# una-dinosauria/local-search-quantization

Hardware: AMD Instinct MI355X
Metric: vectors encoded/sec (ICM, m=8 h=256) (higher is better)
Workload: dtype f32

## Files before the change

local-search-quantization_amd/csrc/lsq_api.hip:

```cpp
#include <stdarg.h>
#include <stddef.h>
#include <stdio.h>
#include <string.h>

#include <algorithm>
#include <atomic>
#include <chrono>
#include <string>
#include <thread>
#include <vector>

#include "lsq_internal.h"

static thread_local char g_err[512] = "";

void lsq_set_error(const char *fmt, ...) {
    va_list ap;
    va_start(ap, fmt);
    vsnprintf(g_err, sizeof(g_err), fmt, ap);
    va_end(ap);
}

extern "C" const char *lsq_last_error(void) { return g_err; }
extern "C" int lsq_version(void) { return LSQ_VERSION; }

extern "C" int lsq_device_count(int *count) {
    if (!count) { lsq_set_error("lsq_device_count: null pointer"); return LSQ_EINVAL; }
    int c = 0;
    hipError_t e = hipGetDeviceCount(&c);
    if (e != hipSuccess) { *count = 0; lsq_set_error("hipGetDeviceCount: %s", hipGetErrorString(e)); return LSQ_ENODEV; }
    *count = c;
    return LSQ_OK;
}


enum { CAT_TABLES = 0, CAT_UNARIES, CAT_PERTURB, CAT_ICM, CAT_COST, CAT_OTHER, CAT_COUNT };

enum : size_t { SMALL_COUNTERS = 0, SMALL_OBJ = 8192, SMALL_BAD = 8704, SMALL_QP = 8832, SMALL_ACTIVE = 10240, SMALL_ROAD = 11008,
                SMALL_READ_END = 11072, SMALL_PROBE = 11264, SMALL_BYTES = 12288 };
static_assert(sizeof(lsq_q16_params) <= SMALL_ACTIVE - SMALL_QP && sizeof(unsigned long long) * LSQ_WALK_COUNTERS <= SMALL_ROAD - SMALL_ACTIVE &&
              sizeof(unsigned long long) * LSQ_WALK_COUNTERS <= SMALL_BYTES - SMALL_PROBE, "the per-call block's windows");

struct ChunkRoad {
    bool filtered = false;
    bool on_device = false;
    bool resident = false;
    int64_t cn = 0, row0 = 0;
    int m = 0;
};

struct lsq_ctx {
    int device = 0;
    hipStream_t own_stream = nullptr;
    hipStream_t stream = nullptr;
    int64_t chunk = 256 * 3968;
    int profile = 0;
    int schedule = 6;
    int64_t q16_min = 65536;
    int tables_changed = 1;
    std::vector<float> hostK;
    int hostK_d = 0, hostK_m = 0;
    bool tables_valid = false;
    int64_t table_reuses = 0;
    int per_node = 0;
    int ablation = 0;
    int light = -1;
    int wave_max = 64;
    int fallback = 1;
    int skip = 1;
    uint32_t auto_it = 0;
    DevBuf sci, T, Ts, U, vCur, vNew, active, recCur, recNew, prev, counters, obj, bad;
    DevBuf probe;
    int64_t probe_div = 8;
    DevBuf small;
    char *small_host = nullptr;
    bool small_packed = false;
    DevBuf Uq, Tq, qp, qscratch, qflag, qsigma;
    lsq_q16_work qw;
    ChunkRoad chunk_road;
    int64_t call_row0 = 0;
    int async_mode = 0;
    bool pending_fold = false;
    DevBuf road;
    int64_t fallback_div = 64;
    int64_t filter_fallback_chunks = 0;
    lsq_lsqr_state *lsqr = nullptr;
    lsq_kmeans_state *kmeans = nullptr;
    lsq_spgl1_state *spgl1 = nullptr;
    lsq_adc_state *adc = nullptr;
    lsq_linscan_stats adc_stats{};
    lsq_search_opts search;
    int knn_u8_int = 1;
    int64_t rerank_batch = 0;
    DevBuf sX, sX2, sK, sB16, sOut16, sTight, sF32;
    DevBuf sSample, sSigmaS;
    std::vector<float> sample_host;
    std::vector<hipEvent_t> panel_ev;
    int64_t panel_bytes = 48ll << 20;
    int64_t pipeline_min_bytes = 64ll << 20;
    hipStream_t copy_stream = nullptr;
    hipEvent_t copy_done = nullptr;
    double cat_ms[CAT_COUNT] = {0, 0, 0, 0, 0, 0};
    int64_t icm_launches = 0, icm_node_updates = 0, staged_blocks = 0, light_blocks = 0, filtered_blocks = 0, filter_refined = 0, filter_exact = 0, filter_f32 = 0;
    int64_t trace[LSQ_WALK_TRACE] = {0};
    struct Pending { hipEvent_t a, b; int cat; };
    std::vector<Pending> pending;
    std::vector<hipEvent_t> pool;
};

static int fold_pending(lsq_ctx *c);
struct AsyncOff {
    lsq_ctx *c; int saved;
    explicit AsyncOff(lsq_ctx *ctx) : c(ctx), saved(ctx ? ctx->async_mode : 0) { if (c) c->async_mode = 0; }
    ~AsyncOff() { if (c) c->async_mode = saved; }
};

static int use_device(lsq_ctx *ctx) {
    if (!ctx) { lsq_set_error("null lsq_ctx"); return LSQ_EINVAL; }
    LSQ_HIP(hipSetDevice(ctx->device));
    return LSQ_OK;
}

struct Timer {
    lsq_ctx *c; int cat; hipEvent_t a = nullptr, b = nullptr; bool on;
    Timer(lsq_ctx *ctx, int category) : c(ctx), cat(category), on(ctx->profile != 0) {
        if (!on) return;
        a = grab(); b = grab();
        if (!a || !b) { on = false; return; }
        (void)hipEventRecord(a, c->stream);
    }
    hipEvent_t grab() {
        if (!c->pool.empty()) { hipEvent_t e = c->pool.back(); c->pool.pop_back(); return e; }
        hipEvent_t e = nullptr;
        if (hipEventCreate(&e) != hipSuccess) return nullptr;
        return e;
    }
    ~Timer() {
        if (!on) return;
        (void)hipEventRecord(b, c->stream);
        c->pending.push_back({a, b, cat});
    }
};

static int resolve_timings(lsq_ctx *ctx) {
    for (auto &p : ctx->pending) {
        LSQ_HIP(hipEventSynchronize(p.b));
        float ms = 0.f;
        LSQ_HIP(hipEventElapsedTime(&ms, p.a, p.b));
        ctx->cat_ms[p.cat] += (double)ms;
        ctx->pool.push_back(p.a);
        ctx->pool.push_back(p.b);
    }
    ctx->pending.clear();
    return LSQ_OK;
}

extern "C" int lsq_create(lsq_ctx **out, int device) {
    if (!out) { lsq_set_error("lsq_create: null out pointer"); return LSQ_EINVAL; }
    *out = nullptr;
    int count = 0;
    LSQ_TRY(lsq_device_count(&count));
    if (count <= 0) { lsq_set_error("no HIP device visible (this library has no CPU fallback)"); return LSQ_ENODEV; }
    if (device < 0 || device >= count) { lsq_set_error("device %d out of range (0..%d)", device, count - 1); return LSQ_EINVAL; }
    LSQ_HIP(hipSetDevice(device));
    hipDeviceProp_t prop;
    LSQ_HIP(hipGetDeviceProperties(&prop, device));
    if (strncmp(prop.gcnArchName, "gfx950", 6) != 0) {
        lsq_set_error("device %d is %s; this library carries gfx950 (MI355X) code objects only", device, prop.gcnArchName);
        return LSQ_ENODEV;
    }
    lsq_ctx *c = new lsq_ctx();
    c->device = device;
    hipError_t e = hipStreamCreateWithFlags(&c->own_stream, hipStreamNonBlocking);
    if (e != hipSuccess) { delete c; lsq_set_error("hipStreamCreate: %s", hipGetErrorString(e)); return LSQ_EHIP; }
    c->stream = c->own_stream;
    if (hipMalloc(&c->small.p, SMALL_BYTES) != hipSuccess || hipHostMalloc(reinterpret_cast<void **>(&c->small_host), SMALL_BYTES, hipHostMallocDefault) != hipSuccess) {
        if (c->small.p) (void)hipFree(c->small.p);
        (void)hipStreamDestroy(c->own_stream);
        delete c;
        lsq_set_error("lsq_create: no memory for the per-call block");
        return LSQ_ENOMEM;
    }
    c->small.cap = SMALL_BYTES;
    {
        hipFuncAttributes fa;
        (void)hipFuncGetAttributes(&fa, lsq_probe_kernel_gemm());
        (void)hipFuncGetAttributes(&fa, lsq_probe_kernel_icm());
        (void)hipFuncGetAttributes(&fa, lsq_probe_kernel_icmq());
        (void)hipStreamCreateWithFlags(&c->copy_stream, hipStreamNonBlocking);
        (void)hipEventCreateWithFlags(&c->copy_done, hipEventDisableTiming);
        char warm[256] = {0};
        (void)hipMemcpyAsync(c->small.p, warm, sizeof(warm), hipMemcpyHostToDevice, c->own_stream);
        (void)hipMemcpyAsync(warm, c->small.p, sizeof(warm), hipMemcpyDeviceToHost, c->own_stream);
        (void)hipStreamSynchronize(c->own_stream);
        (void)hipGetLastError();
    }
    c->counters.window(c->small.p, SMALL_COUNTERS, SMALL_OBJ - SMALL_COUNTERS);
    c->obj.window(c->small.p, SMALL_OBJ, SMALL_BAD - SMALL_OBJ);
    c->bad.window(c->small.p, SMALL_BAD, 64);
    c->qp.window(c->small.p, SMALL_QP, SMALL_ACTIVE - SMALL_QP);
    c->active.window(c->small.p, SMALL_ACTIVE, SMALL_ROAD - SMALL_ACTIVE);
    c->road.window(c->small.p, SMALL_ROAD, SMALL_READ_END - SMALL_ROAD);
    c->probe.window(c->small.p, SMALL_PROBE, SMALL_BYTES - SMALL_PROBE);
    *out = c;
    return LSQ_OK;
}

extern "C" int lsq_destroy(lsq_ctx *c) {
    if (!c) return LSQ_OK;
    (void)hipSetDevice(c->device);
    (void)hipStreamSynchronize(c->stream);
    for (auto &p : c->pending) { (void)hipEventDestroy(p.a); (void)hipEventDestroy(p.b); }
    for (auto e : c->pool) (void)hipEventDestroy(e);
    DevBuf *bufs[] = {&c->road, &c->probe, &c->Uq, &c->Tq, &c->qp, &c->qscratch, &c->qflag, &c->qsigma, &c->sci, &c->T, &c->Ts, &c->U, &c->vCur, &c->vNew, &c->active, &c->recCur, &c->recNew, &c->prev, &c->counters, &c->obj, &c->bad,
                      &c->sX, &c->sX2, &c->sK, &c->sB16, &c->sOut16, &c->sTight, &c->sF32, &c->sSample, &c->sSigmaS};
    for (DevBuf *b : bufs) b->release();
    c->small.release();
    if (c->small_host) (void)hipHostFree(c->small_host);
    for (auto e : c->panel_ev) (void)hipEventDestroy(e);
    lsq_adc_free(c->adc);
    lsq_lsqr_free(c->lsqr);
    lsq_spgl1_free(c->spgl1);
    lsq_kmeans_free(c->kmeans);
    if (c->own_stream) (void)hipStreamDestroy(c->own_stream);
    if (c->copy_stream) (void)hipStreamDestroy(c->copy_stream);
    if (c->copy_done) (void)hipEventDestroy(c->copy_done);
    delete c;
    return LSQ_OK;
}

extern "C" int lsq_set_stream(lsq_ctx *c, void *hip_stream) {
    LSQ_TRY(use_device(c));
    if (c->stream != reinterpret_cast<hipStream_t>(hip_stream)) c->tables_valid = false;
    c->stream = reinterpret_cast<hipStream_t>(hip_stream);
    return LSQ_OK;
}

extern "C" int lsq_set_option(lsq_ctx *c, const char *key, int64_t value) {
    if (!c || !key) { lsq_set_error("lsq_set_option: null argument"); return LSQ_EINVAL; }
    if (!strcmp(key, "chunk")) {
        if (value < 1) { lsq_set_error("chunk must be >= 1"); return LSQ_EINVAL; }
        c->chunk = value;
    } else if (!strcmp(key, "profile")) c->profile = value != 0;
    else if (!strcmp(key, "own_stream")) { if (c->stream != c->own_stream) c->tables_valid = false; c->stream = c->own_stream; }
    else if (!strcmp(key, "skip")) c->skip = value != 0;
#ifdef LSQ_TUNING
    else if (!strcmp(key, "ablation")) c->ablation = (int)value;
#endif
    else if (!strcmp(key, "light")) c->light = (int)value;
    else if (!strcmp(key, "wave_max")) c->wave_max = (int)value;
    else if (!strcmp(key, "fallback")) c->fallback = (int)value;
    else if (!strcmp(key, "q16_min")) c->q16_min = value;
    else if (!strcmp(key, "async")) c->async_mode = value != 0;
    else if (!strcmp(key, "per_node")) c->per_node = value != 0;
    else if (!strcmp(key, "upload_panel_bytes")) {
        if (value < 1) { lsq_set_error("upload_panel_bytes must be >= 1"); return LSQ_EINVAL; }
        c->panel_bytes = value;
    }
    else if (!strcmp(key, "upload_pipeline_min_bytes")) {
        if (value < 0) { lsq_set_error("upload_pipeline_min_bytes must be >= 0"); return LSQ_EINVAL; }
        c->pipeline_min_bytes = value;
    }
    else if (!strcmp(key, "filter_probe_div")) {
        if (value < 0) { lsq_set_error("filter_probe_div must be >= 0"); return LSQ_EINVAL; }
        c->probe_div = value;
    }
    else if (!strcmp(key, "filter_fallback_div")) {
        if (value < 0) { lsq_set_error("filter_fallback_div must be >= 0"); return LSQ_EINVAL; }
        c->fallback_div = value;
    }
    else if (!strcmp(key, "linscan_exhaustive")) c->search.force_exhaustive = value != 0;
    else if (!strcmp(key, "linscan_rank")) {
        if (value < 0) { lsq_set_error("linscan_rank must be >= 0"); return LSQ_EINVAL; }
        c->search.rank_override = (int)value;
    }
    else if (!strcmp(key, "knn_u8_int")) c->knn_u8_int = value != 0;
    else if (!strcmp(key, "rerank_batch")) {
        if (value < 0) { lsq_set_error("rerank_batch must be >= 0"); return LSQ_EINVAL; }
        c->rerank_batch = value;
    }
    else if (!strcmp(key, "ils_counter")) {
        if (value < 0 || value >= (int64_t)LSQ_IT_AUTO) { lsq_set_error("ils_counter must lie in 0..2^32-2"); return LSQ_EINVAL; }
        c->auto_it = (uint32_t)value;
    }
    else if (!strcmp(key, "schedule")) {
        if (value != 3 && value != 4 && value != 6) { lsq_set_error("schedule must be 3, 4 or 6"); return LSQ_EINVAL; }
        c->schedule = (int)value;
    } else { lsq_set_error("unknown option '%s'", key); return LSQ_EINVAL; }
    return LSQ_OK;
}

static int fill_timings(lsq_ctx *c, lsq_timings *out);

extern "C" int lsq_get_timings(lsq_ctx *c, lsq_timings *out) {
    if (!out) { lsq_set_error("lsq_get_timings: null out"); return LSQ_EINVAL; }
    lsq_timings t;
    LSQ_TRY(fill_timings(c, &t));
    memcpy(out, &t, offsetof(lsq_timings, table_reuses));
    return LSQ_OK;
}

extern "C" int lsq_get_timings_sized(lsq_ctx *c, void *out, size_t bytes) {
    if (!out) { lsq_set_error("lsq_get_timings_sized: null out"); return LSQ_EINVAL; }
    lsq_timings t;
    LSQ_TRY(fill_timings(c, &t));
    memcpy(out, &t, bytes < sizeof(t) ? bytes : sizeof(t));
    return LSQ_OK;
}

static int fill_timings(lsq_ctx *c, lsq_timings *out) {
    LSQ_TRY(use_device(c));
    LSQ_TRY(fold_pending(c));
    LSQ_TRY(resolve_timings(c));
    out->tables_ms = c->cat_ms[CAT_TABLES];
    out->unaries_ms = c->cat_ms[CAT_UNARIES];
    out->perturb_ms = c->cat_ms[CAT_PERTURB];
    out->icm_ms = c->cat_ms[CAT_ICM];
    out->cost_ms = c->cat_ms[CAT_COST];
    out->other_ms = c->cat_ms[CAT_OTHER];
    out->icm_launches = c->icm_launches;
    out->icm_node_updates = c->icm_node_updates;
    out->staged_blocks = c->staged_blocks;
    out->light_blocks = c->light_blocks;
    out->filtered_blocks = c->filtered_blocks;
    out->filter_refined = c->filter_refined;
    out->filter_exact = c->filter_exact;
    out->filter_f32 = c->filter_f32;
    out->filter_fallback_chunks = c->filter_fallback_chunks;
    out->xs_launches = 0;
    out->xs_fallback_launches = 0;
    out->table_reuses = c->table_reuses;
    return LSQ_OK;
}

extern "C" int lsq_get_walk_trace(lsq_ctx *c, int64_t *out, int count) {
    if (!c || !out || count < 0) { lsq_set_error("lsq_get_walk_trace: bad arguments"); return LSQ_EINVAL; }
    for (int q = 0; q < count; ++q) out[q] = q < LSQ_WALK_TRACE ? c->trace[q] : 0;
    return LSQ_OK;
}

static_assert(sizeof(lsq_q16_snapshot_params) == sizeof(lsq_q16_params) && sizeof(lsq_q16_snapshot_node) == sizeof(lsq_q16_node) &&
              offsetof(lsq_q16_snapshot_params, node) == offsetof(lsq_q16_params, node) && offsetof(lsq_q16_snapshot_node, window) == offsetof(lsq_q16_node, window) &&
              offsetof(lsq_q16_snapshot_node, slack) == offsetof(lsq_q16_node, slack) && offsetof(lsq_q16_snapshot_node, hiq) == offsetof(lsq_q16_node, hiq),
              "the public snapshot structure restates lsq_q16_params");
extern "C" int lsq_get_q16_snapshot(lsq_ctx *c, int what, void *dst, size_t bytes, int64_t *info) {
    LSQ_TRY(use_device(c));
    if (!c->chunk_road.resident) {
        lsq_set_error("lsq_get_q16_snapshot: no filtered chunk is resident (the last chunk whose unaries were built did not take the 16-bit filtered walk)");
        return LSQ_EINVAL;
    }
    const size_t cn = (size_t)c->chunk_road.cn, m = (size_t)c->chunk_road.m;
    const DevBuf *src = nullptr;
    size_t need = 0;
    switch (what) {
    case LSQ_SNAP_PARAMS: src = &c->qp; need = sizeof(lsq_q16_params); break;
    case LSQ_SNAP_UQ: src = &c->Uq; need = sizeof(uint16_t) * m * cn * LSQ_H; break;
    case LSQ_SNAP_TQ: src = &c->Tq; need = sizeof(uint16_t) * m * (m - 1) * LSQ_H * LSQ_H; break;
    case LSQ_SNAP_QFLAG: src = &c->qflag; need = sizeof(unsigned short) * cn; break;
    case LSQ_SNAP_U: src = &c->U; need = sizeof(float) * m * cn * LSQ_H; break;
    case LSQ_SNAP_T: src = &c->T; need = sizeof(float) * m * m * LSQ_H * LSQ_H; break;
    default: lsq_set_error("lsq_get_q16_snapshot: unknown item %d", what); return LSQ_EINVAL;
    }
    if (need > 0 && (!dst || bytes < need || src->cap < need)) {
        lsq_set_error("lsq_get_q16_snapshot: item %d takes %zu bytes, the buffer has %zu", what, need, dst ? bytes : (size_t)0);
        return LSQ_EINVAL;
    }
    if (info) {
        info[0] = c->chunk_road.cn; info[1] = c->chunk_road.row0; info[2] = c->chunk_road.m;
        info[3] = lsq_q16_slice_width(c->chunk_road.m); info[4] = lsq_walk_slice_width(c->chunk_road.m); info[5] = c->chunk_road.filtered ? 1 : 0;
    }
    if (need > 0) LSQ_HIP(hipMemcpyAsync(dst, src->p, need, hipMemcpyDefault, c->stream));
    return LSQ_OK;
}

extern "C" int lsq_reset_timings(lsq_ctx *c) {
    LSQ_TRY(use_device(c));
    LSQ_TRY(fold_pending(c));
    LSQ_TRY(resolve_timings(c));
    for (double &v : c->cat_ms) v = 0.0;
    c->icm_launches = c->icm_node_updates = c->staged_blocks = c->light_blocks = c->filtered_blocks = c->filter_refined = c->filter_exact = c->filter_f32 = 0;
    c->filter_fallback_chunks = 0;
    c->table_reuses = 0;
    for (int64_t &v : c->trace) v = 0;
    c->adc_stats = lsq_linscan_stats{};
    return LSQ_OK;
}

static int linscan_check(const char *fn, const void *a, const void *b, const void *c0, const void *d0, const void *e, const void *f, int nq, int n,
                         int m, int h, int d, int nn) {
    if (nq < 0 || n < 0 || d < 1 || nn < 1) { lsq_set_error("%s: bad shape nq=%d n=%d d=%d nn=%d", fn, nq, n, d, nn); return LSQ_EINVAL; }
    if (h != LSQ_H || m < 1 || m > LSQ_MAX_M) { lsq_set_error("%s: needs h == 256 and 1 <= m <= 16 (got h=%d m=%d)", fn, h, m); return LSQ_EINVAL; }
    if (nn > n) { lsq_set_error("%s: nn=%d exceeds the database size %d", fn, nn, n); return LSQ_EINVAL; }
    if (nq > 0 && (!a || !b || !c0 || !d0 || !e || !f)) { lsq_set_error("%s: null pointer", fn); return LSQ_EINVAL; }
    return LSQ_OK;
}

static lsq_search_opts search_opts(const lsq_ctx *c, lsq_linscan_stats *stats) {
    lsq_search_opts o = c->search;
    o.stats = stats;
    o.timed = c->profile;
    return o;
}

static lsq_search_input lsq_input(const uint8_t *codes, const float *Q, const float *K, const float *dbnorms, int n, int m, int d) {
    lsq_search_input in{};
    in.kind = LSQ_SEARCH_LSQ; in.codes = codes; in.cstride = m; in.Q = Q; in.qstride = d; in.K = K; in.dbnorms = dbnorms; in.n = n; in.m = m; in.d = d;
    return in;
}
static lsq_search_input pq_input(const uint8_t *codes, int cstride, const float *centers, const float *Q, int qstride, int n, int m, int subdim) {
    lsq_search_input in{};
    in.kind = LSQ_SEARCH_PQ; in.codes = codes; in.cstride = cstride; in.Q = Q; in.qstride = qstride; in.K = centers; in.n = n; in.m = m; in.d = subdim;
    return in;
}
static lsq_search_input exact_input(const void *base, int base_u8, int ldb, const void *Q, int q_u8, int ldq, int n, int d) {
    lsq_search_input in{};
    in.kind = LSQ_SEARCH_EXACT; in.Q = Q; in.qstride = ldq; in.n = n; in.d = d; in.base = base; in.bstride = ldb; in.base_u8 = base_u8; in.q_u8 = q_u8;
    return in;
}

extern "C" int lsq_linscan_dev(lsq_ctx *c, float *d_dists, int *d_idx, const uint8_t *d_codes, const float *d_queries, const float *d_codebooks,
                               const float *d_dbnorms, int nqueries, int ncodes, int m, int h, int d, int nn) {
    if (!c) { lsq_set_error("lsq_linscan_dev: null context"); return LSQ_EINVAL; }
    LSQ_TRY(linscan_check("lsq_linscan_dev", d_dists, d_idx, d_codes, d_queries, d_codebooks, d_dbnorms, nqueries, ncodes, m, h, d, nn));
    if (nqueries == 0) return LSQ_OK;
    LSQ_TRY(use_device(c));
    return lsq_adc_search(c->stream, &c->adc, d_dists, d_idx, lsq_input(d_codes, d_queries, d_codebooks, d_dbnorms, ncodes, m, d), nqueries, nn,
                          search_opts(c, &c->adc_stats));
}

extern "C" int lsq_linscan(lsq_ctx *c, float *dists, int *idx, const unsigned char *codes, const float *queries, const float *codebooks,
                           const float *dbnorms, int nqueries, int ncodes, int m, int h, int d, int nn) {
    if (!c) { lsq_set_error("lsq_linscan: null context"); return LSQ_EINVAL; }
    LSQ_TRY(linscan_check("lsq_linscan", dists, idx, codes, queries, codebooks, dbnorms, nqueries, ncodes, m, h, d, nn));
    if (nqueries == 0) return LSQ_OK;
    LSQ_TRY(use_device(c));
    return lsq_adc_search_host(c->stream, &c->adc, dists, idx, lsq_input(codes, queries, codebooks, dbnorms, ncodes, m, d), nqueries, nn,
                               search_opts(c, &c->adc_stats));
}

static int linscan_pq_check(const char *fn, const void *a, const void *b, const void *c0, const void *d0, const void *e, int N, uint32_t NQ, int B,
                            int K, int dim1codes, int dim1queries, int subdim) {
    LSQ_TRY(lsq_linscan_pq_check(fn, a, b, c0, d0, e, N, NQ, B, K, dim1codes, dim1queries, subdim));
    if (B / 8 > LSQ_MAX_M) { lsq_set_error("%s: the device scan needs B/8 <= 16 (got B=%d: %d sub-spaces)", fn, B, B / 8); return LSQ_EINVAL; }
    if (NQ > (uint32_t)INT32_MAX) { lsq_set_error("%s: NQ=%u exceeds the device scan's limit of 2^31 - 1 queries", fn, NQ); return LSQ_EINVAL; }
    return LSQ_OK;
}

extern "C" int lsq_linscan_pq_dev(lsq_ctx *c, float *d_dists, uint32_t *d_res, const uint8_t *d_codes, const float *d_centers, const float *d_queries,
                                  int N, uint32_t NQ, int B, int K, int dim1codes, int dim1queries, int subdim) {
    if (!c) { lsq_set_error("lsq_linscan_pq_dev: null context"); return LSQ_EINVAL; }
    LSQ_TRY(linscan_pq_check("lsq_linscan_pq_dev", d_dists, d_res, d_codes, d_centers, d_queries, N, NQ, B, K, dim1codes, dim1queries, subdim));
    if (NQ == 0) return LSQ_OK;
    LSQ_TRY(use_device(c));
    return lsq_adc_search(c->stream, &c->adc, d_dists, reinterpret_cast<int *>(d_res),
                          pq_input(d_codes, dim1codes, d_centers, d_queries, dim1queries, N, B / 8, subdim), (int)NQ, K, search_opts(c, &c->adc_stats));
}

extern "C" int lsq_linscan_pq(lsq_ctx *c, float *dists, uint32_t *res, const uint8_t *codes, const float *centers, const float *queries, int N,
                              uint32_t NQ, int B, int K, int dim1codes, int dim1queries, int subdim) {
    if (!c) { lsq_set_error("lsq_linscan_pq: null context"); return LSQ_EINVAL; }
    LSQ_TRY(linscan_pq_check("lsq_linscan_pq", dists, res, codes, centers, queries, N, NQ, B, K, dim1codes, dim1queries, subdim));
    if (NQ == 0) return LSQ_OK;
    LSQ_TRY(use_device(c));
    return lsq_adc_search_host(c->stream, &c->adc, dists, reinterpret_cast<int *>(res), pq_input(codes, dim1codes, centers, queries, dim1queries, N, B / 8, subdim),
                               (int)NQ, K, search_opts(c, &c->adc_stats));
}

extern "C" int lsq_knn_exact_dev(lsq_ctx *c, float *d_dists, uint32_t *d_ids, const float *d_base, const float *d_queries, int n, int nq, int d, int ldb,
                                 int ldq, int nn) {
    if (!c) { lsq_set_error("lsq_knn_exact_dev: null context"); return LSQ_EINVAL; }
    LSQ_TRY(lsq_knn_exact_check("lsq_knn_exact_dev", d_dists, d_ids, d_base, d_queries, n, nq, d, ldb, ldq, nn));
    LSQ_TRY(use_device(c));
    return lsq_adc_search(c->stream, &c->adc, d_dists, reinterpret_cast<int *>(d_ids), exact_input(d_base, 0, ldb, d_queries, 0, ldq, n, d), nq, nn,
                          search_opts(c, &c->adc_stats));
}

extern "C" int lsq_knn_exact(lsq_ctx *c, float *dists, uint32_t *ids, const float *base, const float *queries, int n, int nq, int d, int ldb, int ldq,
                             int nn) {
    if (!c) { lsq_set_error("lsq_knn_exact: null context"); return LSQ_EINVAL; }
    LSQ_TRY(lsq_knn_exact_check("lsq_knn_exact", dists, ids, base, queries, n, nq, d, ldb, ldq, nn));
    LSQ_TRY(use_device(c));
    return lsq_adc_search_host(c->stream, &c->adc, dists, reinterpret_cast<int *>(ids), exact_input(base, 0, ldb, queries, 0, ldq, n, d), nq, nn,
                               search_opts(c, &c->adc_stats));
}

extern "C" int lsq_get_linscan_stats(lsq_ctx *c, lsq_linscan_stats *out) {
    if (!c || !out) { lsq_set_error("lsq_get_linscan_stats: null argument"); return LSQ_EINVAL; }
    *out = c->adc_stats;
    return LSQ_OK;
}

struct lsq_index {
    lsq_ctx *ctx = nullptr;
    int64_t n = 0;
    int d = 0, m = 0, base_u8 = 0;
    int64_t ldb = 0;
    const uint8_t *codes = nullptr;
    const float *K = nullptr, *norms = nullptr;
    const void *base = nullptr;
    DevBuf own_codes, own_K, own_norms, own_base;
    lsq_adc_state *adc = nullptr;
    DevBuf rec_a, rec_b, seg, counter;
    DevBuf short_d, short_i;
    DevBuf s_qscan, s_qexact, s_cand, s_dists, s_ids;
    DevBuf nrm_x, nrm_q;
    hipEvent_t ev[3] = {nullptr, nullptr, nullptr};
    lsq_index_stats stats{};
    lsq_index_knn_info knn{};
};

extern "C" int lsq_index_destroy(lsq_index *ix) {
    if (!ix) return LSQ_OK;
    (void)hipSetDevice(ix->ctx->device);
    (void)hipStreamSynchronize(ix->ctx->stream);
    DevBuf *bufs[] = {&ix->own_codes, &ix->own_K, &ix->own_norms, &ix->own_base, &ix->rec_a, &ix->rec_b, &ix->seg, &ix->counter, &ix->short_d, &ix->short_i,
                      &ix->s_qscan, &ix->s_qexact, &ix->s_cand, &ix->s_dists, &ix->s_ids, &ix->nrm_x, &ix->nrm_q};
    for (DevBuf *b : bufs) b->release();
    lsq_adc_free(ix->adc);
    for (hipEvent_t e : ix->ev) if (e) (void)hipEventDestroy(e);
    delete ix;
    return LSQ_OK;
}

static int index_adopt(lsq_index *ix, DevBuf &own, const void *src, size_t bytes, int on_device, const void **dst) {
    if (on_device) { *dst = src; return LSQ_OK; }
    LSQ_TRY(own.ensure(bytes));
    LSQ_HIP(hipMemcpyAsync(own.p, src, bytes, hipMemcpyHostToDevice, ix->ctx->stream));
    *dst = own.p;
    return LSQ_OK;
}

extern "C" int lsq_index_create(lsq_index **out, lsq_ctx *c, const lsq_index_desc *desc) {
    if (!out) { lsq_set_error("lsq_index_create: null out pointer"); return LSQ_EINVAL; }
    *out = nullptr;
    if (!c || !desc) { lsq_set_error("lsq_index_create: null %s", c ? "description" : "context"); return LSQ_EINVAL; }
    if (!desc->codes && !desc->base) { lsq_set_error("lsq_index_create: neither codes nor base rows"); return LSQ_EINVAL; }
    if (desc->n < 1 || desc->n > (int64_t)INT32_MAX - 1 || desc->d < 1) {
        lsq_set_error("lsq_index_create: needs 1 <= n <= 2^31 - 2 and d >= 1 (got n=%lld d=%d)", (long long)desc->n, desc->d);
        return LSQ_EINVAL;
    }
    if (desc->codes) {
        if (desc->h != LSQ_H || desc->m < 1 || desc->m > LSQ_MAX_M) {
            lsq_set_error("lsq_index_create: needs h == 256 and 1 <= m <= 16 (got h=%d m=%d)", desc->h, desc->m);
            return LSQ_EINVAL;
        }
        if (!desc->codebooks || !desc->dbnorms) { lsq_set_error("lsq_index_create: codes without codebooks or dbnorms"); return LSQ_EINVAL; }
    }
    if (desc->base && desc->ldb < desc->d) { lsq_set_error("lsq_index_create: needs ldb >= d (got ldb=%d d=%d)", desc->ldb, desc->d); return LSQ_EINVAL; }
    if (desc->base && !desc->base_u8 && ((uintptr_t)desc->base & 3) != 0) { lsq_set_error("lsq_index_create: the f32 base is not 4-byte aligned"); return LSQ_EINVAL; }
    LSQ_TRY(use_device(c));
    lsq_index *ix = new lsq_index();
    ix->ctx = c;
    ix->n = desc->n; ix->d = desc->d; ix->m = desc->codes ? desc->m : 0; ix->base_u8 = desc->base_u8 != 0; ix->ldb = desc->ldb;
    const size_t n = (size_t)desc->n, d = (size_t)desc->d;
    int rc = LSQ_OK;
    if (desc->codes) {
        rc = index_adopt(ix, ix->own_codes, desc->codes, n * (size_t)desc->m, desc->on_device, reinterpret_cast<const void **>(&ix->codes));
        if (rc == LSQ_OK) rc = index_adopt(ix, ix->own_K, desc->codebooks, sizeof(float) * (size_t)desc->m * LSQ_H * d, desc->on_device, reinterpret_cast<const void **>(&ix->K));
        if (rc == LSQ_OK) rc = index_adopt(ix, ix->own_norms, desc->dbnorms, sizeof(float) * n, desc->on_device, reinterpret_cast<const void **>(&ix->norms));
    }
    if (rc == LSQ_OK && desc->base)
        rc = index_adopt(ix, ix->own_base, desc->base, ((n - 1) * (size_t)desc->ldb + d) * (desc->base_u8 ? 1 : sizeof(float)), desc->on_device, &ix->base);
    if (rc == LSQ_OK) rc = ix->counter.ensure(sizeof(unsigned long long));
    if (rc == LSQ_OK && hipStreamSynchronize(c->stream) != hipSuccess) { lsq_set_error("lsq_index_create: the upload failed"); rc = LSQ_EHIP; }
    if (rc != LSQ_OK) { (void)lsq_index_destroy(ix); return rc; }
    *out = ix;
    return LSQ_OK;
}

static int index_rerank_dev(lsq_index *ix, float *d_dists, int *d_ids, const float *d_q, int64_t ldq, const int *d_cand, int nq, int L, int nn, int id_base) {
    lsq_ctx *c = ix->ctx;
    hipStream_t s = c->stream;
    const bool timed = c->profile != 0;
    if (timed) for (hipEvent_t &e : ix->ev) if (!e) LSQ_HIP(hipEventCreate(&e));
    int64_t qb = c->rerank_batch > 0 ? c->rerank_batch : (int64_t)(1u << 28) / L;
    if (qb > (int64_t)(1u << 28) / L) qb = (int64_t)(1u << 28) / L;
    if (qb > 16384) qb = 16384;
    if (qb < 1) qb = 1;
    if (qb > nq) qb = nq;
    LSQ_TRY(ix->rec_a.ensure(sizeof(uint64_t) * (size_t)qb * L));
    LSQ_TRY(ix->rec_b.ensure(sizeof(uint64_t) * (size_t)qb * L));
    LSQ_TRY(ix->seg.ensure(sizeof(int) * 2 * (size_t)qb));
    LSQ_HIP(hipMemsetAsync(ix->counter.p, 0, sizeof(unsigned long long), s));
    const int idbits = lsq_adc_idbits(ix->n);
    for (int q0 = 0; q0 < nq; q0 += (int)qb) {
        const int nqb = (int)std::min<int64_t>(qb, nq - q0);
        if (timed) LSQ_HIP(hipEventRecord(ix->ev[0], s));
        LSQ_TRY(lsq_rerank_launch(s, ix->base, ix->base_u8, ix->ldb, ix->n, d_q, ldq, d_cand, q0, nqb, L, ix->d, id_base, ix->rec_a.as<uint64_t>(), idbits,
                                  ix->counter.as<unsigned long long>()));
        if (timed) LSQ_HIP(hipEventRecord(ix->ev[1], s));
        LSQ_TRY(lsq_adc_select(&ix->adc, s, ix->rec_a.as<uint64_t>(), ix->rec_b.as<uint64_t>(), ix->seg.as<int>(), nullptr, nullptr, nullptr, q0, nqb, L, nn,
                               d_dists, d_ids, idbits, 33 + idbits, 1 - id_base));
        if (timed) {
            LSQ_HIP(hipEventRecord(ix->ev[2], s));
            LSQ_HIP(hipEventSynchronize(ix->ev[2]));
            float a = 0, b = 0;
            LSQ_HIP(hipEventElapsedTime(&a, ix->ev[0], ix->ev[1]));
            LSQ_HIP(hipEventElapsedTime(&b, ix->ev[1], ix->ev[2]));
            ix->stats.gather_ms += a; ix->stats.select_ms += b;
        }
        ix->stats.batches += 1;
    }
    unsigned long long bad = 0;
    LSQ_HIP(hipMemcpyAsync(&bad, ix->counter.p, sizeof(bad), hipMemcpyDeviceToHost, s));
    LSQ_HIP(hipStreamSynchronize(s));
    ix->stats.invalid += (int64_t)bad;
    ix->stats.rows += (int64_t)nq * L - (int64_t)bad;
    return LSQ_OK;
}

static int index_stage_rows(lsq_index *ix, DevBuf &buf, const float *src, int rows, int64_t ld, int width, bool pack, const float **dst, int64_t *ld_out) {
    hipStream_t s = ix->ctx->stream;
    if (pack && ld != width) {
        LSQ_TRY(buf.ensure(sizeof(float) * (size_t)rows * width));
        LSQ_HIP(hipMemcpy2DAsync(buf.p, sizeof(float) * (size_t)width, src, sizeof(float) * (size_t)ld, sizeof(float) * (size_t)width, (size_t)rows,
                                 hipMemcpyDefault, s));
        *ld_out = width;
    } else {
        const size_t floats = (size_t)(rows - 1) * (size_t)ld + (size_t)width;
        LSQ_TRY(buf.ensure(sizeof(float) * floats));
        LSQ_HIP(hipMemcpyAsync(buf.p, src, sizeof(float) * floats, hipMemcpyDefault, s));
        *ld_out = ld;
    }
    *dst = buf.as<float>();
    return LSQ_OK;
}

static int index_call_check(const char *fn, lsq_index *ix, const void *dists, const void *ids, int nq, int64_t ldq, int nn) {
    if (!ix) { lsq_set_error("%s: null index", fn); return LSQ_EINVAL; }
    if (nq < 0 || nn < 1 || ldq < ix->d) { lsq_set_error("%s: needs nq >= 0, nn >= 1, ldq >= d (got nq=%d nn=%d ldq=%lld d=%d)", fn, nq, nn, (long long)ldq, ix->d); return LSQ_EINVAL; }
    if (!dists || !ids) { lsq_set_error("%s: null pointer", fn); return LSQ_EINVAL; }
    return LSQ_OK;
}

extern "C" int lsq_index_rerank(lsq_index *ix, float *dists, int *ids, const float *queries, const int *cand, int nq, int ldq, int L, int nn, int id_base,
                                int on_device) {
    LSQ_TRY(index_call_check("lsq_index_rerank", ix, dists, ids, nq, ldq, nn));
    if (!ix->base) { lsq_set_error("lsq_index_rerank: the index holds no base rows"); return LSQ_EINVAL; }
    LSQ_TRY(lsq_rerank_check("lsq_index_rerank", dists, ids, ix->base, queries, cand, ix->n, nq, ix->d, ix->ldb, ldq, L, nn, id_base));
    if (L > (1 << 28)) { lsq_set_error("lsq_index_rerank: needs L <= 2^28 candidates per query (got %d)", L); return LSQ_EINVAL; }
    if (nq == 0) return LSQ_OK;
    LSQ_TRY(use_device(ix->ctx));
    hipStream_t s = ix->ctx->stream;
    if (on_device) {
        LSQ_TRY(index_rerank_dev(ix, dists, ids, queries, ldq, cand, nq, L, nn, id_base));
    } else {
        const float *dq = nullptr;
        int64_t ld = 0;
        LSQ_TRY(index_stage_rows(ix, ix->s_qexact, queries, nq, ldq, ix->d, false, &dq, &ld));
        LSQ_TRY(ix->s_cand.ensure(sizeof(int) * (size_t)nq * L));
        LSQ_TRY(ix->s_dists.ensure(sizeof(float) * (size_t)nq * nn));
        LSQ_TRY(ix->s_ids.ensure(sizeof(int) * (size_t)nq * nn));
        LSQ_HIP(hipMemcpyAsync(ix->s_cand.p, cand, sizeof(int) * (size_t)nq * L, hipMemcpyHostToDevice, s));
        LSQ_TRY(index_rerank_dev(ix, ix->s_dists.as<float>(), ix->s_ids.as<int>(), dq, ld, ix->s_cand.as<int>(), nq, L, nn, id_base));
        LSQ_HIP(hipMemcpyAsync(dists, ix->s_dists.p, sizeof(float) * (size_t)nq * nn, hipMemcpyDeviceToHost, s));
        LSQ_HIP(hipMemcpyAsync(ids, ix->s_ids.p, sizeof(int) * (size_t)nq * nn, hipMemcpyDeviceToHost, s));
        LSQ_HIP(hipStreamSynchronize(s));
    }
    ix->stats.queries += nq;
    return LSQ_OK;
}

extern "C" int lsq_index_search(lsq_index *ix, float *dists, int *ids, const float *q_scan, const float *q_exact, int nq, int ldq, int shortlist, int nn,
                                int on_device) {
    LSQ_TRY(index_call_check("lsq_index_search", ix, dists, ids, nq, ldq, nn));
    if (!ix->codes) { lsq_set_error("lsq_index_search: the index holds no codes"); return LSQ_EINVAL; }
    if (shortlist < 0 || (shortlist > 0 && shortlist < nn)) { lsq_set_error("lsq_index_search: needs shortlist == 0 or shortlist >= nn (got shortlist=%d nn=%d)", shortlist, nn); return LSQ_EINVAL; }
    const int L = shortlist > 0 ? shortlist : nn;
    if (L > ix->n) { lsq_set_error("lsq_index_search: %s=%d exceeds the database size %lld", shortlist > 0 ? "shortlist" : "nn", L, (long long)ix->n); return LSQ_EINVAL; }
    if (shortlist > (1 << 28)) { lsq_set_error("lsq_index_search: needs shortlist <= 2^28 (got %d)", shortlist); return LSQ_EINVAL; }
    if (shortlist > 0 && !ix->base) { lsq_set_error("lsq_index_search: a shortlist needs base rows, the index holds none"); return LSQ_EINVAL; }
    if (!q_scan || (shortlist > 0 && !q_exact)) { lsq_set_error("lsq_index_search: null pointer"); return LSQ_EINVAL; }
    if (nq == 0) return LSQ_OK;
    lsq_ctx *c = ix->ctx;
    LSQ_TRY(use_device(c));
    hipStream_t s = c->stream;
    const int d = ix->d;
    const float *dqs = q_scan;
    int64_t ld = ldq;
    if (!on_device || ldq != d) LSQ_TRY(index_stage_rows(ix, ix->s_qscan, q_scan, nq, ldq, d, true, &dqs, &ld));
    const float *dqe = q_exact;
    int64_t lde = ldq;
    if (shortlist > 0 && !on_device) LSQ_TRY(index_stage_rows(ix, ix->s_qexact, q_exact, nq, ldq, d, false, &dqe, &lde));
    float *out_d = dists;
    int *out_i = ids;
    if (!on_device) {
        LSQ_TRY(ix->s_dists.ensure(sizeof(float) * (size_t)nq * nn));
        LSQ_TRY(ix->s_ids.ensure(sizeof(int) * (size_t)nq * nn));
        out_d = ix->s_dists.as<float>();
        out_i = ix->s_ids.as<int>();
    }
    float *scan_d = out_d;
    int *scan_i = out_i;
    if (shortlist > 0) {
        LSQ_TRY(ix->short_d.ensure(sizeof(float) * (size_t)nq * L));
        LSQ_TRY(ix->short_i.ensure(sizeof(int) * (size_t)nq * L));
        scan_d = ix->short_d.as<float>();
        scan_i = ix->short_i.as<int>();
    }
    lsq_linscan_stats st{};
    LSQ_TRY(lsq_adc_search(s, &ix->adc, scan_d, scan_i, lsq_input(ix->codes, dqs, ix->K, ix->norms, (int)ix->n, ix->m, d), nq, L, search_opts(c, &st)));
    ix->stats.scan_ms += st.lut_ms + st.sample_ms + st.scan_ms + st.select_ms;
    if (shortlist > 0) LSQ_TRY(index_rerank_dev(ix, out_d, out_i, dqe, lde, scan_i, nq, L, nn, 1));
    if (!on_device) {
        LSQ_HIP(hipMemcpyAsync(dists, out_d, sizeof(float) * (size_t)nq * nn, hipMemcpyDeviceToHost, s));
        LSQ_HIP(hipMemcpyAsync(ids, out_i, sizeof(int) * (size_t)nq * nn, hipMemcpyDeviceToHost, s));
        LSQ_HIP(hipStreamSynchronize(s));
    }
    ix->stats.queries += nq;
    return LSQ_OK;
}

extern "C" int lsq_index_knn(lsq_index *ix, float *dists, int *ids, const void *queries, int queries_u8, int nq, int ldq, int nn, int id_base,
                             int on_device) {
    if (!ix) { lsq_set_error("lsq_index_knn: null index"); return LSQ_EINVAL; }
    if (!ix->base) { lsq_set_error("lsq_index_knn: the index holds no base rows"); return LSQ_EINVAL; }
    if (!dists || !ids || !queries) { lsq_set_error("lsq_index_knn: null pointer"); return LSQ_EINVAL; }
    if (nq < 1 || ldq < ix->d) { lsq_set_error("lsq_index_knn: needs nq >= 1 and ldq >= d (got nq=%d ldq=%d d=%d)", nq, ldq, ix->d); return LSQ_EINVAL; }
    if (nn < 1 || nn > ix->n) { lsq_set_error("lsq_index_knn: needs 1 <= nn <= n (got nn=%d n=%lld)", nn, (long long)ix->n); return LSQ_EINVAL; }
    if (id_base != 0 && id_base != 1) { lsq_set_error("lsq_index_knn: id_base must be 0 or 1 (got %d)", id_base); return LSQ_EINVAL; }
    const int q_u8 = queries_u8 != 0;
    if (!q_u8 && ((uintptr_t)queries & 3) != 0) { lsq_set_error("lsq_index_knn: the f32 queries are not 4-byte aligned"); return LSQ_EINVAL; }
    if (ix->ldb > (int64_t)INT32_MAX) { lsq_set_error("lsq_index_knn: needs ldb <= 2^31 - 1"); return LSQ_EINVAL; }
    lsq_ctx *c = ix->ctx;
    LSQ_TRY(use_device(c));
    hipStream_t s = c->stream;
    const int n = (int)ix->n, d = ix->d;
    const size_t qe = q_u8 ? 1 : sizeof(float), out_items = (size_t)nq * (size_t)nn;
    const void *dq = queries;
    float *out_d = dists;
    int *out_i = ids;
    if (!on_device) {
        const size_t q_bytes = qe * ((size_t)(nq - 1) * (size_t)ldq + (size_t)d);
        LSQ_TRY(ix->s_qexact.ensure(q_bytes));
        LSQ_TRY(ix->s_dists.ensure(sizeof(float) * out_items));
        LSQ_TRY(ix->s_ids.ensure(sizeof(int) * out_items));
        LSQ_HIP(hipMemcpyAsync(ix->s_qexact.p, queries, q_bytes, hipMemcpyHostToDevice, s));
        dq = ix->s_qexact.p;
        out_d = ix->s_dists.as<float>();
        out_i = ix->s_ids.as<int>();
    }
    lsq_search_input in = exact_input(ix->base, ix->base_u8, (int)ix->ldb, dq, q_u8, ldq, n, d);
    in.id_base = id_base;
    const bool int_road = ix->base_u8 && q_u8 && d <= 258 && c->knn_u8_int;
    lsq_index_knn_info info{};
    if (int_road) {
        const bool timed = c->profile != 0;
        if (timed) for (hipEvent_t &e : ix->ev) if (!e) LSQ_HIP(hipEventCreate(&e));
        LSQ_TRY(ix->nrm_x.ensure(sizeof(uint32_t) * (size_t)n));
        LSQ_TRY(ix->nrm_q.ensure(sizeof(uint32_t) * (size_t)nq));
        if (timed) LSQ_HIP(hipEventRecord(ix->ev[0], s));
        LSQ_TRY(lsq_knn_launch_norms_u8(s, static_cast<const uint8_t *>(ix->base), ix->ldb, n, d, ix->nrm_x.as<uint32_t>()));
        LSQ_TRY(lsq_knn_launch_norms_u8(s, static_cast<const uint8_t *>(dq), ldq, nq, d, ix->nrm_q.as<uint32_t>()));
        if (timed) {
            LSQ_HIP(hipEventRecord(ix->ev[1], s));
            LSQ_HIP(hipEventSynchronize(ix->ev[1]));
            float ms = 0;
            LSQ_HIP(hipEventElapsedTime(&ms, ix->ev[0], ix->ev[1]));
            info.norms_ms = ms;
        }
        in.xnorms = ix->nrm_x.as<uint32_t>();
        in.qnorms = ix->nrm_q.as<uint32_t>();
    }
    lsq_linscan_stats st{};
    LSQ_TRY(lsq_adc_search(s, &ix->adc, out_d, out_i, in, nq, nn, search_opts(c, &st)));
    if (!on_device) {
        LSQ_HIP(hipMemcpyAsync(dists, out_d, sizeof(float) * out_items, hipMemcpyDeviceToHost, s));
        LSQ_HIP(hipMemcpyAsync(ids, out_i, sizeof(int) * out_items, hipMemcpyDeviceToHost, s));
        LSQ_HIP(hipStreamSynchronize(s));
    }
    info.queries = nq; info.rows = n; info.batches = st.batches; info.fallback_queries = st.fallback_queries; info.exhaustive = st.exhaustive;
    info.int_road = int_road ? 1 : 0;
    info.scan_ms = st.sample_ms + st.scan_ms; info.select_ms = st.select_ms;
    ix->knn = info;
    ix->stats.queries += nq;
    return LSQ_OK;
}

extern "C" int lsq_index_get_knn_info(lsq_index *ix, lsq_index_knn_info *out) {
    if (!ix || !out) { lsq_set_error("lsq_index_get_knn_info: null argument"); return LSQ_EINVAL; }
    *out = ix->knn;
    return LSQ_OK;
}

extern "C" int lsq_index_get_stats(lsq_index *ix, lsq_index_stats *out) {
    if (!ix || !out) { lsq_set_error("lsq_index_get_stats: null argument"); return LSQ_EINVAL; }
    *out = ix->stats;
    return LSQ_OK;
}

extern "C" int lsq_synchronize(lsq_ctx *c) {
    LSQ_TRY(use_device(c));
    LSQ_HIP(hipStreamSynchronize(c->stream));
    return LSQ_OK;
}

extern "C" int lsq_node_order(uint64_t seed, uint32_t it, int m, int randord, int32_t *order) {
    if (!order || m < 1 || m > LSQ_MAX_M) { lsq_set_error("lsq_node_order: bad arguments"); return LSQ_EINVAL; }
    for (int p = 0; p < m; ++p) order[p] = p;
    if (!randord) return LSQ_OK;
    for (int p = m - 1; p >= 1; --p) {
        const uint32_t r = lsq_rng_word(seed, 0, it, LSQ_DOM_PERM, (uint32_t)(m - 1 - p));
        const int q = (int)lsq_mulhi32(r, (uint32_t)(p + 1));
        std::swap(order[p], order[q]);
    }
    return LSQ_OK;
}

extern "C" int lsq_splitarray(int64_t n, int nparts, int part, int64_t *start, int64_t *len) {
    if (n < 0 || nparts < 1 || part < 0 || part >= nparts || !start || !len) { lsq_set_error("lsq_splitarray: bad arguments"); return LSQ_EINVAL; }
    const int64_t per = n / nparts, xtra = n % nparts;
    *start = part < xtra ? part * (per + 1) : xtra * (per + 1) + (part - xtra) * per;
    *len = part < xtra ? per + 1 : per;
    return LSQ_OK;
}

extern "C" int lsq_randinit(uint64_t seed, uint64_t global_offset, int64_t n, int m, int h, int16_t *B) {
    if (n < 0 || m < 1 || h < 1 || h > 32767 || (!B && n > 0)) { lsq_set_error("lsq_randinit: bad arguments"); return LSQ_EINVAL; }
    for (int64_t i = 0; i < n; ++i)
        for (int j = 0; j < m; ++j)
            B[i * m + j] = (int16_t)(1 + lsq_mulhi32(lsq_rng_word(seed, global_offset + (uint64_t)i, 0, LSQ_DOM_INIT, (uint32_t)j), (uint32_t)h));
    return LSQ_OK;
}

static int check_shape(const char *fn, int d, int64_t n, int m, int h) {
    if (d < 1 || n < 0 || m < 1 || m > LSQ_MAX_M) { lsq_set_error("%s: bad shape d=%d n=%lld m=%d (need d>=1, n>=0, 1<=m<=16)", fn, d, (long long)n, m); return LSQ_EINVAL; }
    if (h != LSQ_H) { lsq_set_error("%s: h=%d unsupported; this engine (like the reference GPU path) needs h == 256", fn, h); return LSQ_EINVAL; }
    return LSQ_OK;
}

static int check_codes_host(const char *fn, const int16_t *B, int64_t n, int m, int h) {
    const int64_t total = n * (int64_t)m;
    unsigned bad = 0;
    for (int64_t q = 0; q < total; ++q) bad |= (unsigned)((unsigned)(uint16_t)(B[q] - 1) >= (unsigned)h);
    if (bad) { lsq_set_error("%s: input codes must lie in 1..%d", fn, h); return LSQ_ECODE; }
    return LSQ_OK;
}

static int prepare_tables(lsq_ctx *c, const float *dK, int d, int m) {
    Timer t(c, CAT_TABLES);
    c->tables_changed = 1;
    c->chunk_road.resident = false;
    c->tables_valid = false;
    const int mh = m * LSQ_H;
    LSQ_TRY(c->sci.ensure(sizeof(float) * (size_t)mh));
    LSQ_TRY(c->T.ensure(sizeof(float) * (size_t)mh * mh));
    LSQ_TRY(lsq_launch_sqnorms(c->stream, dK, mh, d, c->sci.as<float>()));
    LSQ_TRY(lsq_launch_chain_gemm(c->stream, dK, dK, nullptr, 2.0f, mh, mh, d, LSQ_H, (int64_t)m * LSQ_H * LSQ_H, LSQ_H, c->T.as<float>(), 0, mh, 0));
    if (c->schedule >= 3 && m > 1) {
        LSQ_TRY(c->Ts.ensure(sizeof(float) * (size_t)m * (m - 1) * LSQ_H * LSQ_H));
        LSQ_TRY(lsq_launch_tables_to_slices(c->stream, c->T.as<float>(), c->Ts.as<float>(), m, lsq_walk_slice_width(m)));
    }
    return LSQ_OK;
}

static bool use_q16(const lsq_ctx *c, int64_t cn) { return c->schedule >= 6 && cn >= c->q16_min; }
static bool start_chunk(lsq_ctx *c, int64_t cn, int slice) {
    c->chunk_road = ChunkRoad{};
    return slice > 0 && use_q16(c, cn);
}

static int q16_map(lsq_ctx *c, int d, int64_t cn, int m, int64_t nsample_rows) {
    LSQ_TRY(c->Uq.ensure(sizeof(uint16_t) * (size_t)m * (size_t)cn * LSQ_H));
    LSQ_TRY(c->Tq.ensure(sizeof(uint16_t) * (size_t)m * (size_t)(m > 1 ? m - 1 : 1) * LSQ_H * LSQ_H));
    const size_t off_bad = 16, off_qrange = 64, off_trange = 256;
    static_assert(off_qrange + sizeof(unsigned) * lsq_q16_work::Q_WORDS <= off_trange, "the range words end before the table ranges");
    const size_t off_rowmin = (off_trange + sizeof(float) * 3 * (size_t)m * m + 255) & ~(size_t)255;
    const size_t off_colmean = off_rowmin + sizeof(float) * (size_t)m * m * LSQ_H;
    const size_t off_colshift = off_colmean + sizeof(float) * (size_t)m * m * LSQ_H;
    const size_t off_means = off_colshift + sizeof(float) * (size_t)m * LSQ_H;
    LSQ_TRY(c->qscratch.ensure(off_means + sizeof(float) * (size_t)m * d));
    LSQ_TRY(c->qsigma.ensure(sizeof(float) * (size_t)cn * m));
    LSQ_TRY(c->qflag.ensure(sizeof(unsigned short) * (size_t)(cn + 2)));
    LSQ_TRY(c->qp.ensure(sizeof(lsq_q16_params)));
    if (nsample_rows > 0) LSQ_TRY(c->sSigmaS.ensure(sizeof(float) * (size_t)nsample_rows * m));
    char *sc = c->qscratch.as<char>();
    lsq_q16_work &w = c->qw;
    w = lsq_q16_work{};
    w.Tq = c->Tq.as<uint16_t>(); w.Uq = c->Uq.as<uint16_t>();
    w.bad = reinterpret_cast<int *>(sc + off_bad);
    w.qrange = reinterpret_cast<unsigned *>(sc + off_qrange);
    w.trange = reinterpret_cast<float *>(sc + off_trange);
    w.rowmin = reinterpret_cast<float *>(sc + off_rowmin);
    w.colmean = reinterpret_cast<float *>(sc + off_colmean);
    w.colshift = reinterpret_cast<float *>(sc + off_colshift);
    w.means = reinterpret_cast<float *>(sc + off_means);
    w.sigma = c->qsigma.as<float>();
    w.qflag = c->qflag.as<unsigned short>();
    w.P = c->qp.as<lsq_q16_params>();
    return LSQ_OK;
}

template <class XT>
static int q16_prepare_chunk(lsq_ctx *c, const XT *dX, const float *dK, int d, int64_t cn, int m, const XT *Xsample = nullptr, int64_t nsample_rows = 0) {
    Timer t(c, CAT_TABLES);
    LSQ_TRY(q16_map(c, d, cn, m, Xsample ? nsample_rows : 0));
    if (Xsample) { c->qw.Xsample = Xsample; c->qw.nsample_rows = nsample_rows; c->qw.sigma_sample = c->sSigmaS.as<float>(); }
    LSQ_TRY(lsq_launch_q16_prepare(c->stream, dX, cn, d, dK, c->sci.as<float>(), c->T.as<float>(), m, c->qw, c->tables_changed));
    c->tables_changed = 0;
    return LSQ_OK;
}

template <class XT>
static int unary_gemm(lsq_ctx *c, const XT *dXc, const float *dK, int d, int64_t cn, int m, int slice, int64_t r0, int64_t rows, bool q16) {
    lsq_gemm_q16 levels;
    if (q16) {
        const lsq_q16_work &w = c->qw;
        levels.Dq = w.Uq; levels.slice_q = lsq_q16_slice_width(m); levels.qp = w.P; levels.qflag = w.qflag; levels.sigma = w.sigma; levels.colshift = w.colshift;
    }
    return lsq_launch_chain_gemm(c->stream, dXc + (size_t)r0 * d, dK, c->sci.as<float>(), -2.0f, rows, m * LSQ_H, d, LSQ_H, cn * (int64_t)LSQ_H, LSQ_H,
                                 c->U.as<float>(), slice, cn, r0, q16 ? &levels : nullptr);
}

static int q16_verdict(lsq_ctx *c, bool q16, int64_t cn, int m);

template <class XT>
static int build_unaries(lsq_ctx *c, const XT *dX, const float *dK, int d, int64_t cn, int m, int slice, int64_t r0, int64_t rows) {
    const bool q16 = start_chunk(c, cn, slice) && r0 == 0 && rows == cn;
    if (q16) LSQ_TRY(q16_prepare_chunk(c, dX, dK, d, cn, m));
    {
        Timer t(c, CAT_UNARIES);
        LSQ_TRY(c->U.ensure(sizeof(float) * (size_t)m * (size_t)cn * LSQ_H));
        LSQ_TRY(unary_gemm(c, dX, dK, d, cn, m, slice, r0, rows, q16));
    }
    return q16_verdict(c, q16, cn, m);
}

static int q16_verdict(lsq_ctx *c, bool q16, int64_t cn, int m) {
    if (q16 && c->async_mode) {
        LSQ_TRY(c->road.ensure(2 * sizeof(unsigned)));
        LSQ_TRY(lsq_launch_q16_road(c->stream, c->qp.as<lsq_q16_params>(), c->road.as<unsigned>(), cn * (int64_t)m, c->fallback_div));
        c->chunk_road.filtered = true;
        c->chunk_road.on_device = true;
    } else if (q16) {
        int verdict[3] = {0, 0, 0};
        LSQ_HIP(hipMemcpyAsync(verdict, c->qp.p, sizeof(verdict), hipMemcpyDeviceToHost, c->stream));
        LSQ_HIP(hipStreamSynchronize(c->stream));
        if (verdict[0] == 1 && (int64_t)verdict[2] * c->fallback_div <= cn * (int64_t)m) c->chunk_road.filtered = true;
        else c->filter_fallback_chunks += 1;
        c->chunk_road.resident = c->chunk_road.filtered;
        c->chunk_road.cn = cn; c->chunk_road.m = m; c->chunk_road.row0 = c->call_row0;
    }
    return LSQ_OK;
}

template <class XT>
static int build_unaries_from_host(lsq_ctx *c, const XT *Xh, XT *dXc, const float *dK, int d, int64_t cn, int m, int slice) {
    const bool q16 = start_chunk(c, cn, slice);
    const size_t row_bytes = sizeof(XT) * (size_t)d;
    int64_t prow = (int64_t)((uint64_t)c->panel_bytes / row_bytes) / 128 * 128;
    if (prow < 128) prow = 128;
    const int npan = (int)((cn + prow - 1) / prow);
    if (!c->copy_stream) LSQ_HIP(hipStreamCreateWithFlags(&c->copy_stream, hipStreamNonBlocking));
    while ((int)c->panel_ev.size() < npan) {
        hipEvent_t e = nullptr;
        LSQ_HIP(hipEventCreateWithFlags(&e, hipEventDisableTiming));
        c->panel_ev.push_back(e);
    }
    if (q16) {
        int64_t rts = 1;
        const int spanels = lsq_q16_sample_rows(cn, d, &rts);
        int64_t ns = 0;
        for (int sp = 0; sp < spanels; ++sp) ns += std::min<int64_t>(128, cn - (int64_t)sp * rts * 128);
        c->sample_host.resize(((size_t)ns * row_bytes + sizeof(float) - 1) / sizeof(float));
        XT *sample = reinterpret_cast<XT *>(c->sample_host.data());
        int64_t at = 0;
        for (int sp = 0; sp < spanels; ++sp) {
            const int64_t r0 = (int64_t)sp * rts * 128, rows = std::min<int64_t>(128, cn - r0);
            memcpy(sample + (size_t)at * d, Xh + (size_t)r0 * d, (size_t)rows * row_bytes);
            at += rows;
        }
        LSQ_TRY(c->sSample.ensure((size_t)ns * row_bytes));
        LSQ_HIP(hipMemcpyAsync(c->sSample.p, sample, (size_t)ns * row_bytes, hipMemcpyHostToDevice, c->stream));
        LSQ_TRY(q16_prepare_chunk<XT>(c, dXc, dK, d, cn, m, c->sSample.as<XT>(), ns));
    }
    LSQ_TRY(c->U.ensure(sizeof(float) * (size_t)m * (size_t)cn * LSQ_H));
    std::atomic<int> landed{0};
    hipError_t herr = hipSuccess;
    std::thread feeder;
    try {
    feeder = std::thread([&]() {
        hipError_t e = hipSetDevice(c->device);
        for (int p = 0; p < npan && e == hipSuccess; ++p) {
            const int64_t r0 = (int64_t)p * prow, rows = std::min<int64_t>(prow, cn - r0);
            e = hipMemcpyAsync(dXc + (size_t)r0 * d, Xh + (size_t)r0 * d, (size_t)rows * row_bytes, hipMemcpyHostToDevice, c->copy_stream);
            if (e == hipSuccess) e = hipEventRecord(c->panel_ev[(size_t)p], c->copy_stream);
            if (e == hipSuccess) landed.store(p + 1, std::memory_order_release);
        }
        herr = e;
        if (e != hipSuccess) landed.store(npan + 1, std::memory_order_release);
    });
    } catch (...) {
        LSQ_HIP(hipMemcpyAsync(dXc, Xh, (size_t)cn * row_bytes, hipMemcpyHostToDevice, c->stream));
        if (q16) c->tables_changed = 1;
        return build_unaries(c, dXc, dK, d, cn, m, slice, 0, cn);
    }
    int rc = LSQ_OK;
    for (int p = 0; p < npan && rc == LSQ_OK; ++p) {
        for (int spins = 0; landed.load(std::memory_order_acquire) <= p; ++spins) {
            if (spins < 64) std::this_thread::yield();
            else std::this_thread::sleep_for(std::chrono::microseconds(50));
        }
        if (landed.load(std::memory_order_acquire) > npan) break;
        const int64_t r0 = (int64_t)p * prow, rows = std::min<int64_t>(prow, cn - r0);
        if (hipStreamWaitEvent(c->stream, c->panel_ev[(size_t)p], 0) != hipSuccess) { lsq_set_error("hipStreamWaitEvent failed"); rc = LSQ_EHIP; break; }
        Timer t(c, CAT_UNARIES);
        if (q16) rc = lsq_launch_unary_shift_panel(c->stream, dXc + (size_t)r0 * d, rows, d, m, c->qw, r0);
        if (rc == LSQ_OK) rc = unary_gemm(c, dXc, dK, d, cn, m, slice, r0, rows, q16);
    }
    feeder.join();
    if (herr != hipSuccess) { lsq_set_error("upload of X failed: %s", hipGetErrorString(herr)); return herr == hipErrorOutOfMemory ? LSQ_ENOMEM : LSQ_EHIP; }
    LSQ_TRY(rc);
    return q16_verdict(c, q16, cn, m);
}

static int run_sweeps(lsq_ctx *c, uint8_t *rec, unsigned short *valid, int64_t cn, int m, const int32_t *order, int nsweeps, unsigned long long *stats,
                      const uint8_t *ref_rec = nullptr, const unsigned short *ref_valid = nullptr, int first_sweep = 0) {
    if (nsweeps <= 0) return LSQ_OK;
    const int pos_base = first_sweep * m;
    Timer t(c, CAT_ICM);
    if (!c->fallback) { ref_rec = nullptr; ref_valid = nullptr; }
    std::vector<int32_t> seq((size_t)nsweeps * m);
    for (int sw = 0; sw < nsweeps; ++sw)
        for (int q = 0; q < m; ++q) seq[(size_t)sw * m + q] = order[q];
    enum { F32, WAVE, FILTERED } road = F32;
    int per_launch = 64;
    if (c->schedule < 4) per_launch = 1;
    else if (c->chunk_road.filtered && valid) {
        road = FILTERED;
        if (c->per_node) per_launch = 1;
    } else {
        int per_pass = 0, npass = 0;
        lsq_walk_geometry(cn, lsq_walk_pp(m, lsq_walk_slice_width(m)), &per_pass, &npass);
        const int light_max = c->light >= 0 ? c->light : 256;
        if (c->ablation == 0 && per_pass <= light_max && per_pass <= c->wave_max) road = WAVE;
    }
    const bool both = road == FILTERED && c->chunk_road.on_device;
    const float *U = c->U.as<float>(), *T = c->T.as<float>();
    int launched = 0;
    if (road == FILTERED)
        LSQ_TRY(lsq_launch_icm_walkq(c->stream, U, c->Uq.as<uint16_t>(), c->Tq.as<uint16_t>(), T, rec, valid, cn, m, seq.data(), (int)seq.size(), pos_base, per_launch,
                                     c->skip, stats, c->light, ref_rec, ref_valid, c->qp.as<lsq_q16_params>(), c->qflag.as<unsigned short>(),
                                     both ? c->road.as<unsigned>() : nullptr, &launched));
    if (road == WAVE)
        LSQ_TRY(lsq_launch_icm_wave(c->stream, U, T, rec, valid, cn, m, seq.data(), (int)seq.size(), pos_base, 64, c->skip, stats, ref_rec, ref_valid, &launched));
    if (road == F32 || both)
        LSQ_TRY(lsq_launch_icm_walk(c->stream, U, c->Ts.as<float>(), T, rec, valid, cn, m, seq.data(), (int)seq.size(), pos_base, both ? 64 : per_launch, c->skip, stats,
                                    c->ablation, c->light, ref_rec, ref_valid, both ? reinterpret_cast<const int *>(c->road.as<unsigned>()) : nullptr, &launched));
    c->icm_launches += launched;
    return LSQ_OK;
}

static void fold_walk_counters(lsq_ctx *c, const unsigned long long *act);
static int fold_pending(lsq_ctx *c);

struct EncodeParams {
    int d, m;
    const int64_t *ilsiters; int nr;
    int icmiter, npert, randord;
    uint64_t seed; uint32_t it0;
};

template <class Snap, class XT>
static int encode_chunk(lsq_ctx *c, const XT *dXc, const float *dK, int64_t cn, uint64_t goff, const EncodeParams &P, int64_t I, Snap snap,
                        bool unaries_ready = false) {
    const int cs = lsq_code_stride(P.m);
    if (!unaries_ready) LSQ_TRY(build_unaries(c, dXc, dK, P.d, cn, P.m, lsq_walk_slice_width(P.m), 0, cn));
    LSQ_TRY(c->recNew.ensure((size_t)cn * cs));
    LSQ_TRY(c->prev.ensure(sizeof(float) * (size_t)cn));
    LSQ_TRY(c->vCur.ensure(sizeof(unsigned short) * (size_t)(cn + 8)));
    LSQ_TRY(c->vNew.ensure(sizeof(unsigned short) * (size_t)(cn + 8)));
    LSQ_HIP(hipMemsetAsync(c->vCur.p, 0, sizeof(unsigned short) * (size_t)cn, c->stream));
    unsigned short *vcur = c->vCur.as<unsigned short>(), *vnew = c->vNew.as<unsigned short>();
    uint8_t *cur = c->recCur.as<uint8_t>(), *nw = c->recNew.as<uint8_t>();
    float *prev = c->prev.as<float>();
    unsigned long long *counters = c->counters.as<unsigned long long>();
    unsigned long long *totals = c->active.as<unsigned long long>(), *probed = nullptr;
    lsq_perturb_next pn;
    pn.on = 1; pn.m = P.m; pn.npert = P.npert; pn.seed = P.seed; pn.goff = goff; pn.dst = nw; pn.vdst = vnew;
    {
        Timer t(c, CAT_COST);
        pn.it = P.it0;
        LSQ_TRY(lsq_launch_cost(c->stream, dXc, dK, cur, cur, prev, counters, cn, P.d, P.m, 0, nullptr, vcur, I > 0 ? &pn : nullptr));
    }
    for (int64_t it = 0; it < I; ++it) {
        int32_t order[LSQ_MAX_M];
        LSQ_TRY(lsq_node_order(P.seed, P.it0 + (uint32_t)it, P.m, P.randord, order));
        const bool probing = it == 0 && c->chunk_road.filtered && c->probe_div > 0 && (I > 1 || P.icmiter > 1);
        const int probe_sweeps = I > 1 ? P.icmiter : (P.icmiter >= 3 ? 2 : 1);
        if (probing) {
            LSQ_TRY(c->probe.ensure(sizeof(unsigned long long) * LSQ_WALK_COUNTERS));
            LSQ_HIP(hipMemsetAsync(c->probe.p, 0, sizeof(unsigned long long) * LSQ_WALK_COUNTERS, c->stream));
            probed = c->probe.as<unsigned long long>();
        }
        LSQ_TRY(run_sweeps(c, nw, vnew, cn, P.m, order, probing ? probe_sweeps : P.icmiter, probing ? probed : totals, cur, vcur, 0));
        if (probing && c->chunk_road.on_device) {
            LSQ_TRY(lsq_launch_q16_probe(c->stream, probed, totals, c->road.as<unsigned>(), c->probe_div));
            LSQ_TRY(run_sweeps(c, nw, vnew, cn, P.m, order, P.icmiter - probe_sweeps, totals, cur, vcur, probe_sweeps));
        } else if (probing) {
            unsigned long long act[LSQ_WALK_COUNTERS] = {0};
            LSQ_HIP(hipMemcpyAsync(act, c->probe.p, sizeof(act), hipMemcpyDeviceToHost, c->stream));
            LSQ_HIP(hipStreamSynchronize(c->stream));
            fold_walk_counters(c, act);
            const unsigned long long hard = act[4 + LSQ_WALK_TRACE] + act[4 + LSQ_WALK_TRACE + 2];
            if ((double)hard * (double)c->probe_div > (double)act[0]) {
                c->chunk_road.filtered = false;
                c->filter_fallback_chunks += 1;
            }
            LSQ_TRY(run_sweeps(c, nw, vnew, cn, P.m, order, P.icmiter - probe_sweeps, totals, cur, vcur, probe_sweeps));
        }
        {
            Timer t(c, CAT_COST);
            pn.it = P.it0 + (uint32_t)it + 1u;
            LSQ_TRY(lsq_launch_cost(c->stream, dXc, dK, nw, cur, prev, counters + 2 * it, cn, P.d, P.m, 1, vnew, vcur, it + 1 < I ? &pn : nullptr));
        }
        for (int r = 0; r < P.nr; ++r)
            if (P.ilsiters[r] == it + 1) {
                Timer t(c, CAT_OTHER);
                LSQ_TRY(lsq_launch_sum_f64(c->stream, prev, cn, c->obj.as<double>() + r));
                LSQ_TRY(snap(r, cur));
            }
    }
    return LSQ_OK;
}

static int validate_encode(const char *fn, int d, int64_t n, int m, int h, const int64_t *ilsiters, int nr, int icmiter, int npert, int64_t *I) {
    LSQ_TRY(check_shape(fn, d, n, m, h));
    if (!ilsiters || nr < 1) { lsq_set_error("%s: ilsiters must hold at least one entry", fn); return LSQ_EINVAL; }
    if (icmiter < 0 || npert < 0) { lsq_set_error("%s: icmiter and npert must be >= 0", fn); return LSQ_EINVAL; }
    *I = 0;
    for (int r = 0; r < nr; ++r) {
        if (ilsiters[r] < 1) { lsq_set_error("%s: ilsiters[%d] = %lld must be >= 1", fn, r, (long long)ilsiters[r]); return LSQ_EINVAL; }
        *I = std::max<int64_t>(*I, ilsiters[r]);
    }
    return LSQ_OK;
}

static int begin_call(lsq_ctx *c, int64_t I, int nr) {
    c->call_row0 = 0;
    c->chunk_road.resident = false;
    LSQ_TRY(c->counters.ensure(sizeof(unsigned long long) * 2 * (size_t)std::max<int64_t>(I, 1)));
    LSQ_TRY(c->obj.ensure(sizeof(double) * (size_t)std::max(nr, 1)));
    LSQ_TRY(c->bad.ensure(sizeof(int)));
    LSQ_TRY(c->active.ensure(sizeof(unsigned long long) * LSQ_WALK_COUNTERS));
    LSQ_TRY(c->road.ensure(2 * sizeof(unsigned)));
    LSQ_TRY(c->qp.ensure(sizeof(lsq_q16_params)));
    if (!c->async_mode) LSQ_TRY(fold_pending(c));
    c->small_packed = c->counters.view && c->obj.view && c->bad.view && c->qp.view && c->active.view && c->road.view;
    if (c->small_packed) {
        LSQ_HIP(hipMemsetAsync(c->small.p, 0, c->pending_fold ? SMALL_ACTIVE : SMALL_READ_END, c->stream));
        return LSQ_OK;
    }
    if (!c->pending_fold) {
        LSQ_HIP(hipMemsetAsync(c->active.p, 0, sizeof(unsigned long long) * LSQ_WALK_COUNTERS, c->stream));
        LSQ_HIP(hipMemsetAsync(c->road.p, 0, 2 * sizeof(unsigned), c->stream));
    }
    LSQ_HIP(hipMemsetAsync(c->counters.p, 0, sizeof(unsigned long long) * 2 * (size_t)std::max<int64_t>(I, 1), c->stream));
    LSQ_HIP(hipMemsetAsync(c->obj.p, 0, sizeof(double) * (size_t)std::max(nr, 1), c->stream));
    LSQ_HIP(hipMemsetAsync(c->bad.p, 0, sizeof(int), c->stream));
    LSQ_HIP(hipMemsetAsync(c->qp.p, 0, sizeof(lsq_q16_params), c->stream));
    return LSQ_OK;
}

static void fold_walk_counters(lsq_ctx *c, const unsigned long long *act) {
    c->icm_node_updates += (int64_t)act[0];
    c->staged_blocks += (int64_t)act[1];
    c->light_blocks += (int64_t)act[2];
    c->filtered_blocks += (int64_t)act[3];
    c->filter_refined += (int64_t)act[4 + LSQ_WALK_TRACE];
    c->filter_exact += (int64_t)act[4 + LSQ_WALK_TRACE + 1];
    c->filter_f32 += (int64_t)act[4 + LSQ_WALK_TRACE + 2];
    for (int q = 0; q < LSQ_WALK_TRACE; ++q) c->trace[q] += (int64_t)act[4 + q];
}

static int fold_pending(lsq_ctx *c) {
    if (!c->pending_fold) return LSQ_OK;
    c->pending_fold = false;
    unsigned long long act[LSQ_WALK_COUNTERS] = {0};
    unsigned road[2] = {0u, 0u};
    LSQ_HIP(hipMemcpyAsync(act, c->active.p, sizeof(act), hipMemcpyDeviceToHost, c->stream));
    LSQ_HIP(hipMemcpyAsync(road, c->road.p, sizeof(road), hipMemcpyDeviceToHost, c->stream));
    LSQ_HIP(hipMemsetAsync(c->active.p, 0, sizeof(act), c->stream));
    LSQ_HIP(hipMemsetAsync(c->road.as<unsigned>() + 1, 0, sizeof(unsigned), c->stream));
    LSQ_HIP(hipStreamSynchronize(c->stream));
    fold_walk_counters(c, act);
    c->filter_fallback_chunks += (int64_t)road[1];
    return LSQ_OK;
}

static int finish_call(lsq_ctx *c, int64_t I, int nr, double *obj_sums, int64_t *stats) {
    if (c->async_mode) {
        LSQ_HIP(hipMemcpyAsync(obj_sums, c->obj.p, sizeof(double) * (size_t)nr, hipMemcpyDefault, c->stream));
        if (stats) LSQ_HIP(hipMemcpyAsync(stats, c->counters.p, sizeof(unsigned long long) * 2 * (size_t)I, hipMemcpyDefault, c->stream));
        c->pending_fold = true;
        return LSQ_OK;
    }
    if (c->small_packed) {
        LSQ_HIP(hipMemcpyAsync(c->small_host, c->small.p, SMALL_READ_END, hipMemcpyDeviceToHost, c->stream));
        LSQ_HIP(hipStreamSynchronize(c->stream));
        memcpy(obj_sums, c->small_host + SMALL_OBJ, sizeof(double) * (size_t)nr);
        unsigned long long act[LSQ_WALK_COUNTERS];
        memcpy(act, c->small_host + SMALL_ACTIVE, sizeof(act));
        fold_walk_counters(c, act);
        if (stats) {
            const unsigned long long *cnt = reinterpret_cast<const unsigned long long *>(c->small_host + SMALL_COUNTERS);
            for (int64_t q = 0; q < 2 * I; ++q) stats[q] = (int64_t)cnt[q];
        }
        return LSQ_OK;
    }
    std::vector<unsigned long long> cnt(2 * (size_t)std::max<int64_t>(I, 1));
    LSQ_HIP(hipMemcpyAsync(obj_sums, c->obj.p, sizeof(double) * (size_t)nr, hipMemcpyDeviceToHost, c->stream));
    LSQ_HIP(hipMemcpyAsync(cnt.data(), c->counters.p, sizeof(unsigned long long) * cnt.size(), hipMemcpyDeviceToHost, c->stream));
    unsigned long long act[LSQ_WALK_COUNTERS] = {0};
    LSQ_HIP(hipMemcpyAsync(act, c->active.p, sizeof(act), hipMemcpyDeviceToHost, c->stream));
    LSQ_HIP(hipStreamSynchronize(c->stream));
    fold_walk_counters(c, act);
    if (stats) for (int64_t q = 0; q < 2 * I; ++q) stats[q] = (int64_t)cnt[(size_t)q];
    return LSQ_OK;
}

template <class XT>
static int encode_dev(lsq_ctx *c, const char *fn, const XT *dX, const uint8_t *dB0, const float *dK, int d, int64_t n, int m, int h,
                      const int64_t *ilsiters, int nr, int icmiter, int npert, int randord, uint64_t seed,
                      uint64_t global_offset, uint8_t *dBs, double *obj_sums, int64_t *stats) {
    LSQ_TRY(use_device(c));
    int64_t I = 0;
    LSQ_TRY(validate_encode(fn, d, n, m, h, ilsiters, nr, icmiter, npert, &I));
    if (!dK || !obj_sums || (n > 0 && (!dX || !dB0 || !dBs))) { lsq_set_error("%s: null pointer", fn); return LSQ_EINVAL; }
    LSQ_TRY(begin_call(c, I, nr));
    LSQ_TRY(prepare_tables(c, dK, d, m));
    const EncodeParams P{d, m, ilsiters, nr, icmiter, npert, randord, seed, 0u};
    const int cs = lsq_code_stride(m);
    for (int64_t off = 0; off < n; off += c->chunk) {
        const int64_t cn = std::min<int64_t>(c->chunk, n - off);
        c->call_row0 = off;
        LSQ_TRY(c->recCur.ensure((size_t)cn * cs));
        {
            Timer t(c, CAT_OTHER);
            LSQ_TRY(lsq_launch_codes_expand(c->stream, dB0 + off * m, cn, m, c->recCur.as<uint8_t>()));
        }
        auto snap = [&](int r, const uint8_t *cur) {
            return lsq_launch_codes_compact(c->stream, cur, cn, m, dBs + ((int64_t)r * n + off) * m);
        };
        LSQ_TRY(encode_chunk(c, dX + off * d, dK, cn, global_offset + (uint64_t)off, P, I, snap));
    }
    return finish_call(c, I, nr, obj_sums, stats);
}

extern "C" int lsq_encode_icm_dev(lsq_ctx *c, const float *dX, const uint8_t *dB0, const float *dK, int d, int64_t n, int m, int h,
                                  const int64_t *ilsiters, int nr, int icmiter, int npert, int randord, uint64_t seed,
                                  uint64_t global_offset, uint8_t *dBs, double *obj_sums, int64_t *stats) {
    return encode_dev(c, "lsq_encode_icm_dev", dX, dB0, dK, d, n, m, h, ilsiters, nr, icmiter, npert, randord, seed, global_offset, dBs, obj_sums, stats);
}

extern "C" int lsq_encode_icm_u8_dev(lsq_ctx *c, const uint8_t *dX8, const uint8_t *dB0, const float *dK, int d, int64_t n, int m, int h,
                                     const int64_t *ilsiters, int nr, int icmiter, int npert, int randord, uint64_t seed,
                                     uint64_t global_offset, uint8_t *dBs, double *obj_sums, int64_t *stats) {
    return encode_dev(c, "lsq_encode_icm_u8_dev", dX8, dB0, dK, d, n, m, h, ilsiters, nr, icmiter, npert, randord, seed, global_offset, dBs, obj_sums, stats);
}

static size_t codebook_bytes(int d, int m) { return sizeof(float) * (size_t)m * LSQ_H * d; }
static int claim_sK(lsq_ctx *c, int d, int m, const float *K = nullptr) {
    c->tables_valid = false;
    LSQ_TRY(c->sK.ensure(codebook_bytes(d, m)));
    if (K) LSQ_HIP(hipMemcpyAsync(c->sK.p, K, codebook_bytes(d, m), hipMemcpyHostToDevice, c->stream));
    return LSQ_OK;
}

static int host_codebooks(lsq_ctx *c, const float *K, int d, int m) {
    const size_t count = (size_t)m * LSQ_H * d, kbytes = sizeof(float) * count;
    if (c->tables_valid && c->hostK_d == d && c->hostK_m == m && c->hostK.size() == count && memcmp(c->hostK.data(), K, kbytes) == 0) {
        c->table_reuses += 1;
        return LSQ_OK;
    }
    LSQ_TRY(claim_sK(c, d, m, K));
    LSQ_TRY(prepare_tables(c, c->sK.as<float>(), d, m));
    c->hostK.assign(K, K + count);
    c->hostK_d = d; c->hostK_m = m;
    c->tables_valid = true;
    return LSQ_OK;
}

struct HostPlacement { int64_t ntot, row0; double *sums; int64_t *stats; };

template <class XT>
static int encode_host(lsq_ctx *c, const char *fn, const XT *X, const int16_t *B, const float *K, int d, int64_t n, int m, int h,
                       const int64_t *ilsiters, int nr, int icmiter, int npert, int randord, uint64_t seed, uint32_t it0,
                       uint64_t global_offset, int verbose, int16_t *Bs, float *objs, const HostPlacement *place = nullptr) {
    LSQ_TRY(use_device(c));
    const AsyncOff sync_here(c);
    int64_t I = 0;
    LSQ_TRY(validate_encode(fn, d, n, m, h, ilsiters, nr, icmiter, npert, &I));
    if (!K || (!objs && !place) || (n > 0 && (!X || !B || !Bs))) { lsq_set_error("%s: null pointer", fn); return LSQ_EINVAL; }
    const int64_t ntot = place ? place->ntot : n, row0 = place ? place->row0 : 0;
    LSQ_TRY(begin_call(c, I, nr));
    LSQ_TRY(host_codebooks(c, K, d, m));
    const float *dK = c->sK.as<float>();
    {
        const int rc = check_codes_host(fn, B, n, m, h);
        if (rc != LSQ_OK) {
            (void)hipStreamSynchronize(c->stream);
            return rc;
        }
    }
    const EncodeParams P{d, m, ilsiters, nr, icmiter, npert, randord, seed, it0};
    const int cs = lsq_code_stride(m);
    if (n > c->chunk) {
        if (!c->copy_stream) LSQ_HIP(hipStreamCreateWithFlags(&c->copy_stream, hipStreamNonBlocking));
        if (!c->copy_done) LSQ_HIP(hipEventCreateWithFlags(&c->copy_done, hipEventDisableTiming));
    }
    DevBuf *xb[2] = {&c->sX, &c->sX2};
    int which = 0;
    for (int64_t off = 0; off < n; off += c->chunk, which ^= 1) {
        const int64_t cn = std::min<int64_t>(c->chunk, n - off);
        c->call_row0 = off;
        LSQ_TRY(xb[which]->ensure(sizeof(XT) * (size_t)cn * d));
        LSQ_TRY(c->sB16.ensure(sizeof(int16_t) * (size_t)cn * m));
        LSQ_TRY(c->sOut16.ensure(sizeof(int16_t) * (size_t)cn * m * nr));
        LSQ_TRY(c->recCur.ensure((size_t)cn * cs));
        XT *dXc = xb[which]->as<XT>();
        const bool piped = off == 0 && c->pipeline_min_bytes > 0 && (int64_t)sizeof(XT) * cn * d >= c->pipeline_min_bytes;
        if (piped) {}
        else if (off == 0) LSQ_HIP(hipMemcpyAsync(dXc, X, sizeof(XT) * (size_t)cn * d, hipMemcpyHostToDevice, c->stream));
        else LSQ_HIP(hipStreamWaitEvent(c->stream, c->copy_done, 0));
        LSQ_HIP(hipMemcpyAsync(c->sB16.p, B + off * m, sizeof(int16_t) * (size_t)cn * m, hipMemcpyHostToDevice, c->stream));
        LSQ_TRY(lsq_launch_codes_from_i16(c->stream, c->sB16.as<int16_t>(), cn, m, h, c->recCur.as<uint8_t>(), c->bad.as<int>()));
        auto snap = [&](int r, const uint8_t *cur) {
            return lsq_launch_codes_to_i16(c->stream, cur, cn, m, c->sOut16.as<int16_t>() + (int64_t)r * cn * m);
        };
        if (piped) LSQ_TRY(build_unaries_from_host(c, X, dXc, dK, d, cn, m, lsq_walk_slice_width(m)));
        LSQ_TRY(encode_chunk(c, dXc, dK, cn, global_offset + (uint64_t)off, P, I, snap, piped));
        const int64_t noff = off + c->chunk;
        if (noff < n) {
            const int64_t ncn = std::min<int64_t>(c->chunk, n - noff);
            LSQ_TRY(xb[which ^ 1]->ensure(sizeof(XT) * (size_t)ncn * d));
            LSQ_HIP(hipMemcpyAsync(xb[which ^ 1]->p, X + noff * d, sizeof(XT) * (size_t)ncn * d, hipMemcpyHostToDevice, c->copy_stream));
            LSQ_HIP(hipEventRecord(c->copy_done, c->copy_stream));
        }
        for (int r = 0; r < nr; ++r)
            LSQ_HIP(hipMemcpyAsync(Bs + ((int64_t)r * ntot + row0 + off) * m, c->sOut16.as<int16_t>() + (int64_t)r * cn * m,
                                   sizeof(int16_t) * (size_t)cn * m, hipMemcpyDeviceToHost, c->stream));
        LSQ_HIP(hipStreamSynchronize(c->stream));
    }
    std::vector<double> sums((size_t)nr, 0.0);
    std::vector<int64_t> stats(2 * (size_t)I, 0);
    LSQ_TRY(finish_call(c, I, nr, sums.data(), stats.data()));
    if (place) {
        for (int r = 0; r < nr; ++r) place->sums[r] = sums[(size_t)r];
        if (place->stats) for (size_t q = 0; q < stats.size(); ++q) place->stats[q] = stats[q];
        return LSQ_OK;
    }
    for (int r = 0; r < nr; ++r) objs[r] = (float)(n > 0 ? sums[(size_t)r] / (double)n : 0.0);
    if (verbose)
        for (int64_t it = 0; it < I; ++it)
            printf(" ILS iteration %lld/%lld done. %5.2f%% new codes are equal. %5.2f%% new codes are better.\n", (long long)(it + 1),
                   (long long)I, n ? 100.0 * (double)stats[2 * it] / (double)n : 0.0, n ? 100.0 * (double)stats[2 * it + 1] / (double)n : 0.0);
    return LSQ_OK;
}

extern "C" int lsq_encode_icm(lsq_ctx *c, const float *RX, const int16_t *B, const float *K, int d, int64_t n, int m, int h,
                              const int64_t *ilsiters, int nr, int icmiter, int npert, int randord, int nsplits, uint64_t seed,
                              uint64_t global_offset, int verbose, int16_t *Bs, float *objs) {
    if (nsplits < 1) { lsq_set_error("lsq_encode_icm: nsplits must be >= 1"); return LSQ_EINVAL; }
    return encode_host(c, "lsq_encode_icm", RX, B, K, d, n, m, h, ilsiters, nr, icmiter, npert, randord, seed, 0u, global_offset, verbose, Bs, objs);
}

extern "C" int lsq_encode_icm_u8(lsq_ctx *c, const uint8_t *RX8, const int16_t *B, const float *K, int d, int64_t n, int m, int h,
                                 const int64_t *ilsiters, int nr, int icmiter, int npert, int randord, int nsplits, uint64_t seed,
                                 uint64_t global_offset, int verbose, int16_t *Bs, float *objs) {
    if (nsplits < 1) { lsq_set_error("lsq_encode_icm_u8: nsplits must be >= 1"); return LSQ_EINVAL; }
    return encode_host(c, "lsq_encode_icm_u8", RX8, B, K, d, n, m, h, ilsiters, nr, icmiter, npert, randord, seed, 0u, global_offset, verbose, Bs, objs);
}

struct lsq_multi { std::vector<lsq_ctx *> ctx; };

extern "C" int lsq_multi_create(lsq_multi **out, const int *devices, int ndev) {
    if (!out || !devices || ndev < 1) { lsq_set_error("lsq_multi_create: need an output pointer and at least one device"); return LSQ_EINVAL; }
    *out = nullptr;
    lsq_multi *mg = new lsq_multi();
    for (int p = 0; p < ndev; ++p) {
        lsq_ctx *c = nullptr;
        const int rc = lsq_create(&c, devices[p]);
        if (rc != LSQ_OK) {
            for (lsq_ctx *q : mg->ctx) (void)lsq_destroy(q);
            delete mg;
            return rc;
        }
        mg->ctx.push_back(c);
    }
    *out = mg;
    return LSQ_OK;
}

extern "C" int lsq_multi_destroy(lsq_multi *mg) {
    if (!mg) return LSQ_OK;
    for (lsq_ctx *q : mg->ctx) (void)lsq_destroy(q);
    delete mg;
    return LSQ_OK;
}

extern "C" int lsq_multi_set_option(lsq_multi *mg, const char *key, int64_t value) {
    if (!mg) { lsq_set_error("null lsq_multi"); return LSQ_EINVAL; }
    for (lsq_ctx *q : mg->ctx) LSQ_TRY(lsq_set_option(q, key, value));
    return LSQ_OK;
}

template <class XT>
static int multi_encode(lsq_multi *mg, const char *fn, const XT *RX, const int16_t *B, const float *K, int d, int64_t n, int m, int h,
                        const int64_t *ilsiters, int nr, int icmiter, int npert, int randord, uint64_t seed,
                        uint64_t global_offset, int verbose, int16_t *Bs, float *objs) {
    if (!mg || mg->ctx.empty()) { lsq_set_error("null lsq_multi"); return LSQ_EINVAL; }
    int64_t I = 0;
    LSQ_TRY(validate_encode(fn, d, n, m, h, ilsiters, nr, icmiter, npert, &I));
    if (!K || !objs || (n > 0 && (!RX || !B || !Bs))) { lsq_set_error("%s: null pointer", fn); return LSQ_EINVAL; }
    const int G = (int)mg->ctx.size();
    std::vector<std::vector<double>> sums((size_t)G, std::vector<double>((size_t)nr, 0.0));
    std::vector<std::vector<int64_t>> stats((size_t)G, std::vector<int64_t>(2 * (size_t)I, 0));
    std::vector<int> rc((size_t)G, LSQ_OK);
    std::vector<std::string> err((size_t)G);
    std::vector<std::thread> th;
    for (int p = 0; p < G; ++p) {
        th.emplace_back([&, p]() {
            int64_t s0 = 0, len = 0;
            rc[(size_t)p] = lsq_splitarray(n, G, p, &s0, &len);
            if (rc[(size_t)p] == LSQ_OK && len > 0) {
                const HostPlacement place{n, s0, sums[(size_t)p].data(), stats[(size_t)p].data()};
                rc[(size_t)p] = encode_host(mg->ctx[(size_t)p], fn, RX + s0 * d, B + s0 * m, K, d, len, m, h, ilsiters, nr,
                                            icmiter, npert, randord, seed, 0u, global_offset + (uint64_t)s0, 0, Bs, nullptr, &place);
            }
            if (rc[(size_t)p] != LSQ_OK) err[(size_t)p] = lsq_last_error();
        });
    }
    for (auto &t : th) t.join();
    for (int p = 0; p < G; ++p)
        if (rc[(size_t)p] != LSQ_OK) { lsq_set_error("device shard %d: %s", p, err[(size_t)p].c_str()); return rc[(size_t)p]; }
    for (int r = 0; r < nr; ++r) {
        double tot = 0.0;
        for (int p = 0; p < G; ++p) tot += sums[(size_t)p][(size_t)r];
        objs[r] = (float)(n > 0 ? tot / (double)n : 0.0);
    }
    if (verbose)
        for (int64_t it = 0; it < I; ++it) {
            int64_t eq = 0, better = 0;
            for (int p = 0; p < G; ++p) { eq += stats[(size_t)p][2 * (size_t)it]; better += stats[(size_t)p][2 * (size_t)it + 1]; }
            printf(" ILS iteration %lld/%lld done. %5.2f%% new codes are equal. %5.2f%% new codes are better.\n", (long long)(it + 1),
                   (long long)I, n ? 100.0 * (double)eq / (double)n : 0.0, n ? 100.0 * (double)better / (double)n : 0.0);
        }
    return LSQ_OK;
}

extern "C" int lsq_multi_encode_icm(lsq_multi *mg, const float *RX, const int16_t *B, const float *K, int d, int64_t n, int m, int h,
                                    const int64_t *ilsiters, int nr, int icmiter, int npert, int randord, uint64_t seed,
                                    uint64_t global_offset, int verbose, int16_t *Bs, float *objs) {
    return multi_encode(mg, "lsq_multi_encode_icm", RX, B, K, d, n, m, h, ilsiters, nr, icmiter, npert, randord, seed, global_offset, verbose, Bs, objs);
}

extern "C" int lsq_multi_encode_icm_u8(lsq_multi *mg, const uint8_t *RX8, const int16_t *B, const float *K, int d, int64_t n, int m, int h,
                                       const int64_t *ilsiters, int nr, int icmiter, int npert, int randord, uint64_t seed,
                                       uint64_t global_offset, int verbose, int16_t *Bs, float *objs) {
    return multi_encode(mg, "lsq_multi_encode_icm_u8", RX8, B, K, d, n, m, h, ilsiters, nr, icmiter, npert, randord, seed, global_offset, verbose, Bs, objs);
}

extern "C" int lsq_multi_linscan(lsq_multi *mg, float *dists, int *idx, const unsigned char *codes, const float *queries, const float *codebooks,
                                 const float *dbnorms, int nqueries, int ncodes, int m, int h, int d, int nn) {
    if (!mg || mg->ctx.empty()) { lsq_set_error("null lsq_multi"); return LSQ_EINVAL; }
    LSQ_TRY(linscan_check("lsq_multi_linscan", dists, idx, codes, queries, codebooks, dbnorms, nqueries, ncodes, m, h, d, nn));
    if (nqueries == 0) return LSQ_OK;
    const int G = (int)mg->ctx.size();
    std::vector<std::vector<float>> pd((size_t)G);
    std::vector<std::vector<int>> pi((size_t)G);
    std::vector<int> klen((size_t)G, 0), rc((size_t)G, LSQ_OK);
    std::vector<int64_t> start((size_t)G, 0);
    std::vector<std::string> err((size_t)G);
    std::vector<std::thread> th;
    for (int p = 0; p < G; ++p) {
        th.emplace_back([&, p]() {
            int64_t s0 = 0, len = 0;
            rc[(size_t)p] = lsq_splitarray(ncodes, G, p, &s0, &len);
            start[(size_t)p] = s0;
            if (rc[(size_t)p] != LSQ_OK || len == 0) return;
            const int k = (int)std::min<int64_t>(nn, len);
            klen[(size_t)p] = k;
            pd[(size_t)p].resize((size_t)nqueries * k);
            pi[(size_t)p].resize((size_t)nqueries * k);
            rc[(size_t)p] = lsq_linscan(mg->ctx[(size_t)p], pd[(size_t)p].data(), pi[(size_t)p].data(), codes + s0 * m, queries, codebooks, dbnorms + s0,
                                        nqueries, (int)len, m, h, d, k);
            if (rc[(size_t)p] != LSQ_OK) err[(size_t)p] = lsq_last_error();
        });
    }
    for (auto &t : th) t.join();
    for (int p = 0; p < G; ++p)
        if (rc[(size_t)p] != LSQ_OK) { lsq_set_error("device shard %d: %s", p, err[(size_t)p].c_str()); return rc[(size_t)p]; }
    auto less = [](float da, int ia, float db, int ib) {
        const bool na = da != da, nb = db != db;
        if (na != nb) return nb;
        if (!na && da != db) return da < db;
        return ia < ib;
    };
    const int nt = std::max(1, std::min<int>((int)std::thread::hardware_concurrency(), nqueries));
    std::vector<std::thread> mt;
    for (int t = 0; t < nt; ++t) {
        mt.emplace_back([&, t]() {
            std::vector<int> pos((size_t)G);
            for (int q = (int)((int64_t)nqueries * t / nt); q < (int)((int64_t)nqueries * (t + 1) / nt); ++q) {
                std::fill(pos.begin(), pos.end(), 0);
                for (int r = 0; r < nn; ++r) {
                    int best = -1;
                    float bd = 0.0f;
                    int bi = 0;
                    for (int p = 0; p < G; ++p) {
                        if (pos[(size_t)p] >= klen[(size_t)p]) continue;
                        const size_t e = (size_t)q * klen[(size_t)p] + (size_t)pos[(size_t)p];
                        const float dd = pd[(size_t)p][e];
                        const int ii = pi[(size_t)p][e] + (int)start[(size_t)p];
                        if (best < 0 || less(dd, ii, bd, bi)) { best = p; bd = dd; bi = ii; }
                    }
                    dists[(size_t)q * nn + r] = bd;
                    idx[(size_t)q * nn + r] = bi;
                    pos[(size_t)best] += 1;
                }
            }
        });
    }
    for (auto &t : mt) t.join();
    return LSQ_OK;
}

extern "C" int lsq_encoding_icm(lsq_ctx *c, const float *X, const int16_t *oldB, const float *K, int d, int64_t n, int m, int h,
                                int niter, int randord, int npert, uint64_t seed, uint32_t it, uint64_t global_offset, int16_t *outB) {
    const int64_t one = 1;
    float obj = 0.f;
    if (!c) { lsq_set_error("null lsq_ctx"); return LSQ_EINVAL; }
    const bool autoit = it == LSQ_IT_AUTO;
    const int rc = encode_host(c, "lsq_encoding_icm", X, oldB, K, d, n, m, h, &one, 1, niter, npert, randord, seed, autoit ? c->auto_it : it,
                               global_offset, 0, outB, &obj);
    if (rc == LSQ_OK && autoit && c->auto_it < LSQ_IT_AUTO - 1u) ++c->auto_it;
    return rc;
}


static int entry_args(const char *fn, lsq_ctx *c, int d, int64_t n, int m, int h, bool ok, const char *what = "null pointer") {
    LSQ_TRY(use_device(c));
    LSQ_TRY(check_shape(fn, d, n, m, h));
    if (!ok) { lsq_set_error("%s: %s", fn, what); return LSQ_EINVAL; }
    return LSQ_OK;
}

static int stage_X(lsq_ctx *c, const float *X, int d, int64_t n) {
    LSQ_TRY(c->sX.ensure(sizeof(float) * (size_t)std::max<int64_t>(n, 1) * d));
    if (n > 0) LSQ_HIP(hipMemcpyAsync(c->sX.p, X, sizeof(float) * (size_t)n * d, hipMemcpyHostToDevice, c->stream));
    return LSQ_OK;
}

static int stage_codes(lsq_ctx *c, const int16_t *B, int64_t n, int m, int h, bool tight = false) {
    LSQ_TRY(c->sB16.ensure(sizeof(int16_t) * (size_t)std::max<int64_t>(n, 1) * m));
    LSQ_TRY(c->recCur.ensure((size_t)std::max<int64_t>(n, 1) * lsq_code_stride(m)));
    LSQ_TRY(c->bad.ensure(sizeof(int)));
    LSQ_HIP(hipMemsetAsync(c->bad.p, 0, sizeof(int), c->stream));
    if (n > 0) {
        LSQ_HIP(hipMemcpyAsync(c->sB16.p, B, sizeof(int16_t) * (size_t)n * m, hipMemcpyHostToDevice, c->stream));
        LSQ_TRY(lsq_launch_codes_from_i16(c->stream, c->sB16.as<int16_t>(), n, m, h, c->recCur.as<uint8_t>(), c->bad.as<int>()));
    }
    int bad = 0;
    LSQ_HIP(hipMemcpyAsync(&bad, c->bad.p, sizeof(int), hipMemcpyDeviceToHost, c->stream));
    LSQ_HIP(hipStreamSynchronize(c->stream));
    if (bad) { lsq_set_error("input codes must lie in 1..%d", h); return LSQ_ECODE; }
    if (tight) LSQ_TRY(c->sTight.ensure((size_t)std::max<int64_t>(n, 1) * m));
    if (tight && n > 0) LSQ_TRY(lsq_launch_codes_compact(c->stream, c->recCur.as<uint8_t>(), n, m, c->sTight.as<uint8_t>()));
    return LSQ_OK;
}

struct Slice { size_t bytes; void *p = nullptr; template <class T> T *as() const { return static_cast<T *>(p); } };
static int carve_f32(lsq_ctx *c, std::initializer_list<Slice *> slices) {
    size_t total = 0;
    for (Slice *s : slices) total += (s->bytes + 15) & ~(size_t)15;
    LSQ_TRY(c->sF32.ensure(total));
    char *p = c->sF32.as<char>();
    for (Slice *s : slices) { s->p = p; p += (s->bytes + 15) & ~(size_t)15; }
    return LSQ_OK;
}

static int stage(lsq_ctx *c, void *dst, const void *src, size_t bytes) { LSQ_HIP(hipMemcpyAsync(dst, src, bytes, hipMemcpyHostToDevice, c->stream)); return LSQ_OK; }
static int fetch(lsq_ctx *c, void *dst, const void *src, size_t bytes) { if (dst) LSQ_HIP(hipMemcpyAsync(dst, src, bytes, hipMemcpyDeviceToHost, c->stream)); return LSQ_OK; }
static int finish(lsq_ctx *c) { LSQ_HIP(hipStreamSynchronize(c->stream)); return LSQ_OK; }

static int fetch_codes(lsq_ctx *c, int16_t *B, int64_t n, int m, bool from_tight = false) {
    LSQ_TRY(c->sB16.ensure(sizeof(int16_t) * (size_t)n * m));
    if (from_tight) LSQ_TRY(c->recNew.ensure((size_t)n * lsq_code_stride(m)));
    if (from_tight) LSQ_TRY(lsq_launch_codes_expand(c->stream, c->sTight.as<uint8_t>(), n, m, c->recNew.as<uint8_t>()));
    LSQ_TRY(lsq_launch_codes_to_i16(c->stream, c->recNew.as<uint8_t>(), n, m, c->sB16.as<int16_t>()));
    return fetch(c, B, c->sB16.p, sizeof(int16_t) * (size_t)n * m);
}

extern "C" int lsq_encode_icm_fully(lsq_ctx *c, int16_t *B, const float *X, const float *K, int d, int64_t n, int m, int h, int niter,
                                    int randord, int npert, int64_t idx_first, uint64_t seed, uint32_t it) {
    LSQ_TRY(use_device(c));
    const AsyncOff sync_here(c);
    LSQ_TRY(check_shape("lsq_encode_icm_fully", d, n, m, h));
    if (!K || niter < 0 || npert < 0 || idx_first < 1 || (n > 0 && (!B || !X))) { lsq_set_error("lsq_encode_icm_fully: bad arguments"); return LSQ_EINVAL; }
    const bool autoit = it == LSQ_IT_AUTO;
    if (autoit) it = c->auto_it;
    if (n == 0) return LSQ_OK;
    if (n > c->chunk) { lsq_set_error("lsq_encode_icm_fully: n = %lld exceeds the resident chunk (%lld); raise option \"chunk\"", (long long)n, (long long)c->chunk); return LSQ_EINVAL; }
// ... 334 lines not shown
```

local-search-quantization_amd/csrc/lsq_icmq.hip:

```cpp
#include <stdlib.h>

#include <type_traits>

#include <atomic>

#include "lsq_q16.h"
#include "lsq_xload.h"
#ifdef LSQ_TUNING
__device__ unsigned long long *g_walkq_dbg = nullptr;
__device__ unsigned int g_walkq_dbg_slot = 0;
__device__ unsigned long long *g_walkq_dbg_cur = nullptr;
__device__ unsigned long long *g_walkq_blk = nullptr;
#define LSQ_WALKQ_DBG_WORDS (24 + 2 * 65)
#define DBG_STAMP(k) do { if (dbgp && threadIdx.x == 0) dbgp[k] = wall_clock64(); } while (0)
#else
#define DBG_STAMP(k) do {} while (0)
#endif

namespace {

__global__ __launch_bounds__(256) void table_colmean_kernel(const float *__restrict__ T, int m, float *__restrict__ colmean) {
    const int jk = blockIdx.x, j = jk / m, k = jk % m, a = threadIdx.x;
    if (j == k) { colmean[(int64_t)jk * LSQ_H + a] = 0.0f; return; }
    const float *p = T + (int64_t)jk * LSQ_H * LSQ_H;
    double acc = 0.0;
    for (int b = 0; b < LSQ_H; ++b) acc += (double)p[(int64_t)b * LSQ_H + a];
    colmean[(int64_t)jk * LSQ_H + a] = (float)(acc * (1.0 / LSQ_H));
}
__global__ __launch_bounds__(256) void unary_colshift_kernel(const float *__restrict__ colmean, int m, float *__restrict__ colshift) {
    const int j = blockIdx.x, a = threadIdx.x;
    double acc = 0.0;
    for (int k = 0; k < m; ++k)
        if (k != j) acc += (double)colmean[((int64_t)j * m + k) * LSQ_H + a];
    colshift[j * LSQ_H + a] = (float)acc;
}
__global__ __launch_bounds__(256) void table_range_kernel(const float *__restrict__ T, int m, const float *__restrict__ colmean, float *__restrict__ range,
                                                          float *__restrict__ rowmin, int *__restrict__ bad) {
    const int jk = blockIdx.x, j = jk / m, k = jk % m;
    if (j == k) return;
    const float *p = T + (int64_t)jk * LSQ_H * LSQ_H;
    const int lane = threadIdx.x & 63, wave = threadIdx.x >> 6;
    const f32x4 g = *reinterpret_cast<const f32x4 *>(colmean + (int64_t)jk * LSQ_H + 4 * lane);
    float rng = 0.0f, mag = 0.0f;
    float gmag = fmaxf(fmaxf(fabsf(g.x), fabsf(g.y)), fmaxf(fabsf(g.z), fabsf(g.w)));
    bool nonfinite = false;
    for (int b = wave; b < LSQ_H; b += 4) {
        const f32x4 v = *reinterpret_cast<const f32x4 *>(p + (int64_t)b * LSQ_H + 4 * lane);
        nonfinite = nonfinite || !(fabsf(v.x) <= 3.0e38f) || !(fabsf(v.y) <= 3.0e38f) || !(fabsf(v.z) <= 3.0e38f) || !(fabsf(v.w) <= 3.0e38f);
        const f32x4 c = v - g;
        float lo = fminf(fminf(c.x, c.y), fminf(c.z, c.w)), hi = fmaxf(fmaxf(c.x, c.y), fmaxf(c.z, c.w));
        float am = fmaxf(fmaxf(fabsf(v.x), fabsf(v.y)), fmaxf(fabsf(v.z), fabsf(v.w)));
#pragma unroll
        for (int off = 32; off > 0; off >>= 1) {
            lo = fminf(lo, __shfl_xor(lo, off, 64)); hi = fmaxf(hi, __shfl_xor(hi, off, 64)); am = fmaxf(am, __shfl_xor(am, off, 64));
        }
        if (lane == 0) rowmin[(int64_t)jk * LSQ_H + b] = lo;
        rng = fmaxf(rng, hi - lo);
        mag = fmaxf(mag, am);
    }
#pragma unroll
    for (int off = 32; off > 0; off >>= 1) gmag = fmaxf(gmag, __shfl_xor(gmag, off, 64));
    __shared__ float srng[4], smag[4];
    if (__ballot(nonfinite) != 0ull && lane == 0) atomicExch(bad, 1);
    if (lane == 0) { srng[wave] = rng; smag[wave] = mag; }
    __syncthreads();
    if (threadIdx.x == 0) {
        range[jk * 3 + 0] = fmaxf(fmaxf(srng[0], srng[1]), fmaxf(srng[2], srng[3]));
        range[jk * 3 + 1] = fmaxf(fmaxf(smag[0], smag[1]), fmaxf(smag[2], smag[3]));
        range[jk * 3 + 2] = gmag;
    }
}

__global__ __launch_bounds__(256) void codebook_means_kernel(const float *__restrict__ K, int m, int d, float *__restrict__ R) {
    const int j = blockIdx.y, t = blockIdx.x * 64 + (threadIdx.x & 63), wave = threadIdx.x >> 6;
    __shared__ float part[4][64];
    float acc = 0.0f;
    if (t < d)
        for (int a = wave; a < LSQ_H; a += 4) acc += K[((int64_t)j * LSQ_H + a) * d + t];
    part[wave][threadIdx.x & 63] = acc;
    __syncthreads();
    if (wave == 0 && t < d) R[(int64_t)j * d + t] = ((part[0][threadIdx.x] + part[1][threadIdx.x]) + (part[2][threadIdx.x] + part[3][threadIdx.x])) * (1.0f / LSQ_H);
}

template <bool LONGV, class XT = float>
__global__ __launch_bounds__(256) void unary_shift_kernel(const XT *__restrict__ X, const float *__restrict__ R, int64_t n, int d, int m,
                                                          float *__restrict__ sigma, unsigned *__restrict__ sigmax,
                                                          const unsigned *__restrict__ bound, unsigned short *__restrict__ qflag,
                                                          int64_t flag_row0, lsq_q16_params *__restrict__ P) {
    const int lane = threadIdx.x & 63, lp = lane & 15;
    const int64_t nrows = (int64_t)gridDim.x * 16;
    const bool vec = std::is_same<XT, float>::value ? (d & 3) == 0 && ((((uintptr_t)X | (uintptr_t)R) & 15) == 0)
                                                    : (d & 3) == 0 && (((uintptr_t)X & 3) == 0) && (((uintptr_t)R & 15) == 0);
    float amax = 0.0f;
    const int64_t first = ((int64_t)blockIdx.x * 256 + (threadIdx.x & ~63)) >> 4;
    const float bnd = bound ? __uint_as_float(*bound) : __builtin_inff();
    auto flag_row = [&](int64_t i, bool live, float rmax, bool rnan) {
        if (!qflag || !live || lp != 0 || (!(rmax > bnd) && !rnan)) return;
        const int64_t gi = flag_row0 + i;
        const unsigned bits = ((1u << m) - 1u) << (16 * (int)(gi & 1));
        const unsigned old = atomicOr(reinterpret_cast<unsigned *>(qflag + (gi & ~(int64_t)1)), bits);
        const int fresh = __popc(bits & ~old);
        if (P && fresh) atomicAdd(&P->nflag, fresh);
    };
    for (int64_t base = first; base < n; base += nrows) {
        const int64_t i = base + (lane >> 4);
        const bool live = i < n;
        float rmax = 0.0f;
        bool rnan = false;
        const XT *x = X + (live ? i : 0) * (int64_t)d;
        if (!LONGV && vec && d <= 256) {
            f32x4 xr[4];
#pragma unroll
            for (int t = 0; t < 4; ++t)
                xr[t] = 4 * lp + 64 * t < d ? lsq_ld4(x + 4 * lp + 64 * t) : (f32x4){0.0f, 0.0f, 0.0f, 0.0f};
            for (int j = 0; j < m; ++j) {
                const float *r = R + (int64_t)j * d + 4 * lp;
                float acc = 0.0f;
#pragma unroll
                for (int t = 0; t < 4; ++t)
                    if (4 * lp + 64 * t < d) {
                        const f32x4 rv = *reinterpret_cast<const f32x4 *>(r + 64 * t);
                        acc = fmaf(xr[t].w, rv.w, fmaf(xr[t].z, rv.z, fmaf(xr[t].y, rv.y, fmaf(xr[t].x, rv.x, acc))));
                    }
                acc = acc + dpp_self<DPP_XOR1, 0xf>(acc);
                acc = acc + dpp_self<DPP_XOR2, 0xf>(acc);
                acc = acc + dpp_self<DPP_HALF_MIRROR, 0xf>(acc);
                acc = acc + dpp_self<DPP_MIRROR, 0xf>(acc);
                const float sg = 2.0f * acc;
                if (live && lp == 0) sigma[i * m + j] = sg;
                if (live) { amax = fmaxf(amax, fabsf(sg)); rmax = fmaxf(rmax, fabsf(sg)); if (!(sg == sg)) rnan = true; }
            }
            flag_row(i, live, rmax, rnan);
            continue;
        }
        if (LONGV && vec) {
            float accj[LSQ_MAX_M];
#pragma unroll
            for (int j = 0; j < LSQ_MAX_M; ++j) accj[j] = 0.0f;
            for (int c0 = 0; c0 < d; c0 += 256) {
                f32x4 xr[4];
#pragma unroll
                for (int t = 0; t < 4; ++t)
                    xr[t] = c0 + 4 * lp + 64 * t < d ? lsq_ld4_nt(x + c0 + 4 * lp + 64 * t) : (f32x4){0.0f, 0.0f, 0.0f, 0.0f};
#pragma unroll
                for (int j = 0; j < LSQ_MAX_M; ++j) {
                    if (j < m) {
                        const float *r = R + (int64_t)j * d + c0 + 4 * lp;
#pragma unroll
                        for (int t = 0; t < 4; ++t)
                            if (c0 + 4 * lp + 64 * t < d) {
                                const f32x4 rv = *reinterpret_cast<const f32x4 *>(r + 64 * t);
                                accj[j] = fmaf(xr[t].w, rv.w, fmaf(xr[t].z, rv.z, fmaf(xr[t].y, rv.y, fmaf(xr[t].x, rv.x, accj[j]))));
                            }
                    }
                }
            }
#pragma unroll
            for (int j = 0; j < LSQ_MAX_M; ++j) {
                if (j < m) {
                    float acc = accj[j];
                    acc = acc + dpp_self<DPP_XOR1, 0xf>(acc);
                    acc = acc + dpp_self<DPP_XOR2, 0xf>(acc);
                    acc = acc + dpp_self<DPP_HALF_MIRROR, 0xf>(acc);
                    acc = acc + dpp_self<DPP_MIRROR, 0xf>(acc);
                    const float sg = 2.0f * acc;
                    if (live && lp == 0) sigma[i * m + j] = sg;
                    if (live) { amax = fmaxf(amax, fabsf(sg)); rmax = fmaxf(rmax, fabsf(sg)); if (!(sg == sg)) rnan = true; }
                }
            }
            flag_row(i, live, rmax, rnan);
            continue;
        }
        for (int j = 0; j < m; ++j) {
            const float *r = R + (int64_t)j * d;
            float acc = 0.0f;
            if (vec) {
                for (int t = 4 * lp; t < d; t += 64) {
                    const f32x4 xv = lsq_ld4(x + t), rv = *reinterpret_cast<const f32x4 *>(r + t);
                    acc += xv.x * rv.x + xv.y * rv.y + xv.z * rv.z + xv.w * rv.w;
                }
            } else {
                for (int t = lp; t < d; t += 16) acc += (float)x[t] * r[t];
            }
            acc = acc + dpp_self<DPP_XOR1, 0xf>(acc);
            acc = acc + dpp_self<DPP_XOR2, 0xf>(acc);
            acc = acc + dpp_self<DPP_HALF_MIRROR, 0xf>(acc);
            acc = acc + dpp_self<DPP_MIRROR, 0xf>(acc);
            const float sg = 2.0f * acc;
            if (live && lp == 0) sigma[i * m + j] = sg;
            if (live) { amax = fmaxf(amax, fabsf(sg)); rmax = fmaxf(rmax, fabsf(sg)); if (!(sg == sg)) rnan = true; }
        }
        flag_row(i, live, rmax, rnan);
    }
#pragma unroll
    for (int off = 32; off > 0; off >>= 1) amax = fmaxf(amax, __shfl_xor(amax, off, 64));
    if (lane == 0 && __float_as_uint(amax) > __hip_atomic_load(sigmax, __ATOMIC_RELAXED, __HIP_MEMORY_SCOPE_AGENT)) atomicMax(sigmax, __float_as_uint(amax));
}

__global__ __launch_bounds__(64) void q16_range_init_kernel(unsigned *__restrict__ qrange, int m) {
    const int t = threadIdx.x;
    if (t < 2 * LSQ_MAX_M + 4) qrange[t] = (t < 2 * m && !(t & 1)) ? 0xffffffffu : 0u;
}

template <class XT>
static void launch_unary_shift(dim3 grid, hipStream_t s, const XT *X, const float *R, int64_t n, int d, int m, float *sigma, unsigned *sigmax,
                               const unsigned *bound = nullptr, unsigned short *qflag = nullptr, int64_t flag_row0 = 0, lsq_q16_params *P = nullptr) {
    if (d > 256) hipLaunchKernelGGL((unary_shift_kernel<true, XT>), grid, dim3(256), 0, s, X, R, n, d, m, sigma, sigmax, bound, qflag, flag_row0, P);
    else hipLaunchKernelGGL((unary_shift_kernel<false, XT>), grid, dim3(256), 0, s, X, R, n, d, m, sigma, sigmax, bound, qflag, flag_row0, P);
}
#define LSQ_SHIFT_LAUNCH(D_, GRID_, S_, ...) launch_unary_shift(GRID_, S_, __VA_ARGS__)

__global__ __launch_bounds__(64) void q16_params_kernel(const float *__restrict__ trange, const int *__restrict__ bad, const unsigned *__restrict__ qrange,
                                                        int m, lsq_q16_params *__restrict__ P, unsigned *__restrict__ sigrange, float sig_scale) {
    if (threadIdx.x != 0) return;
    const float sigb = sigrange ? __uint_as_float(sigrange[0]) * sig_scale + (sig_scale > 1.0f ? 1e-30f : 0.0f) : 0.0f;
    if (sigrange) sigrange[1] = __float_as_uint(sigb);
    const double sigmax = (double)sigb;
    bool ok = (bad[0] == 0) && (qrange[2 * LSQ_MAX_M] == 0);
    for (int j = 0; j < m; ++j) {
        const unsigned kl = qrange[2 * j], kh = qrange[2 * j + 1];
        lsq_q16_node nd;
        nd.loU = 0.0f; nd.invD = 0.0f; nd.D = 0.0f; nd.hiq = 0.0f; nd.window = 65535; nd.slack = 0.0;
        if (kl > kh) { ok = false; P->node[j] = nd; continue; }
        const double sl = (double)__uint_as_float((kl & 0x80000000u) ? (kl ^ 0x80000000u) : ~kl);
        const double sh = (double)__uint_as_float((kh & 0x80000000u) ? (kh ^ 0x80000000u) : ~kh);
        const double mg = 0.125 * (sh - sl) + 1e-30 + fmax(fabs(sl), fabs(sh)) / 1048576.0;
        double loU = sl - mg;
        const double hiU = sh + mg;
        nd.loU = (float)loU;
        if ((double)nd.loU > loU) nd.loU = nextafterf(nd.loU, -__builtin_inff());
        loU = (double)nd.loU;
        const double W = fmax(fabs(loU), fabs(hiU));
        double Gmax = 0.0;
        double rsum = hiU - loU, tsum = 0.0, sub = 0.0;
        for (int k = 0; k < m; ++k) {
            if (k == j) continue;
            const double tr = (double)trange[(j * m + k) * 3] * (1.0 + 1e-6), tm = (double)trange[(j * m + k) * 3 + 1], gm = (double)trange[(j * m + k) * 3 + 2];
            rsum += tr;
            tsum += tm;
            Gmax += gm;
            sub += 2.0 * (tm + gm) + tr;
        }
        const double smax = W + sigmax + Gmax + tsum;
        sub += (W + Gmax + sigmax) * 3.0 + 2.0 * Gmax;
        const double D = rsum / 65500.0;
        const double eps = (double)(m + 1) * smax * 5.9604644775390625e-8 * 2.0 + sub * 5.9604644775390625e-8 * 2.0;
        const double slack = (double)m * (0.5 + 1.0 / 32.0) * D + eps + 65535.0 * D * 2.384185791015625e-7;
        nd.D = (float)D;
        nd.invD = (float)(1.0 / D);
        nd.hiq = (float)fmin(floor((hiU - loU) / D), 65535.0);
        nd.slack = slack;
        const double w = 2.0 * slack / D;
        nd.window = (w < 30000.0) ? (int)w + 1 : 65535;
        if (!(D > 1e-30 && D < 1e30 && rsum == rsum && smax < 1e30)) ok = false;
        if (!(nd.invD > 1e-30f && nd.invD < 1e30f)) ok = false;
        P->node[j] = nd;
    }
    P->ok = ok ? 1 : 0;
    P->nflag = 0;
}

template <int SLQ>
__global__ __launch_bounds__(256) void tables_to_q16_slices_kernel(const float *__restrict__ T, uint16_t *__restrict__ Tq, int m,
                                                                   const lsq_q16_params *__restrict__ P, const float *__restrict__ rowmin,
                                                                   const float *__restrict__ colmean) {
    constexpr int NS = LSQ_H / SLQ, LPV = SLQ / 8;
    const int64_t total = (int64_t)m * NS * (m - 1) * LSQ_H * LPV;
    const int64_t e = (int64_t)blockIdx.x * 256 + threadIdx.x;
    if (e >= total) return;
    const int qq = (int)(e % LPV);
    int64_t r = e / LPV;
    const int b = (int)(r % LSQ_H); r /= LSQ_H;
    const int kk = (int)(r % (m - 1)); r /= (m - 1);
    const int slice = (int)(r % NS);
    const int j = (int)(r / NS);
    const int k = kk + (kk >= j ? 1 : 0);
    const float lo = rowmin[((int64_t)j * m + k) * LSQ_H + b], inv = P->node[j].invD;
    const float *src = T + (((int64_t)j * m + k) * LSQ_H + b) * LSQ_H + slice * SLQ + qq * 8;
    const float *gs = colmean + ((int64_t)j * m + k) * LSQ_H + slice * SLQ + qq * 8;
    uint32_t w[4];
#pragma unroll
    for (int t = 0; t < 4; ++t) {
        const float q0 = fminf(fmaxf(rintf(((src[2 * t] - gs[2 * t]) - lo) * inv), 0.0f), 65535.0f);
        const float q1 = fminf(fmaxf(rintf(((src[2 * t + 1] - gs[2 * t + 1]) - lo) * inv), 0.0f), 65535.0f);
        w[t] = (uint32_t)q0 | ((uint32_t)q1 << 16);
    }
    const int64_t dst = (((int64_t)j * NS + slice) * (m - 1) * LSQ_H + q16_row_index<SLQ>(m, kk, b)) * LPV + qq;
    reinterpret_cast<u32x4 *>(Tq)[dst] = (u32x4){w[0], w[1], w[2], w[3]};
}

template <int M>
__device__ inline int q16_refine(const float *__restrict__ U, const uint16_t *__restrict__ Uq, const uint16_t *__restrict__ Tq,
                                 const float *__restrict__ T, uint8_t *__restrict__ rec, unsigned short *__restrict__ valid,
                                 const uint8_t *__restrict__ ref_rec, const unsigned short *__restrict__ ref_valid, int64_t n, int j,
                                 int64_t lo, const unsigned short *list, const uint32_t *arec, int namb, int SLF, int abl, unsigned short *vmir) {
    using RT = WalkqRot<M>;
    constexpr int CS = (M <= 8) ? 8 : 16;
    constexpr int RW = CS / 4;
    constexpr int AREC = 2 + RW;
    if (abl & 4) return 0;
    constexpr int NS = LSQ_H / RT::SLQ;
    constexpr int TAB = (M - 1) * LSQ_H * (RT::SLQ / 8);
    constexpr int NW = RT::NT / 64;
    const int lane = threadIdx.x & 63, wave = threadIdx.x >> 6;
    const int grp = lane >> 4, t16 = lane & 15;
    const int sl = (16 * t16) / RT::SLQ, off = (16 * t16) % RT::SLQ;
    const uint16_t *__restrict__ Uqj = Uq + (int64_t)j * n * LSQ_H;
    const uint16_t *__restrict__ Tqj = Tq + ((int64_t)j * NS + sl) * TAB * 8 + off;
    const float *__restrict__ Tj = T + (int64_t)j * M * LSQ_H * LSQ_H;
    const bool have_ref = ref_rec && ref_valid;
    int nexact = 0;
    for (int r0 = wave * 4; r0 < namb; r0 += NW * 4) {
        const int r = r0 + grp;
        const bool act = r < namb;
        const uint32_t *ar = arec + (act ? r : r0) * AREC;
        const uint32_t key = ar[0], limit = ar[1];
        uint32_t rw[RW];
#pragma unroll
        for (int w2 = 0; w2 < RW; ++w2) rw[w2] = ar[2 + w2];
        const int ci = (int)(key & 0xffffu), a1 = (int)((key >> 16) & 0xffu), a2 = (int)(key >> 24);
        const int64_t i = lo + (RT::LHOLE ? list[((ci >> 4) << 7) + (ci & 15)] : list[ci]);
        const u32x4 *up = reinterpret_cast<const u32x4 *>(Uqj + ((int64_t)sl * n + ((abl & 2) ? (int64_t)0 : i)) * RT::SLQ + off);
        u32x4 s0 = (u32x4){0xffffffffu, 0xffffffffu, 0xffffffffu, 0xffffffffu}, s1 = s0;
        if (!(abl & 8)) { s0 = up[0]; s1 = up[1]; }
        unsigned short vo = 0, rv = 0;
        uint32_t rr[RW];
#pragma unroll
        for (int w2 = 0; w2 < RW; ++w2) rr[w2] = 0;
        if (t16 == 0) {
            if (valid) vo = valid[i];
            if (have_ref) {
#pragma unroll
                for (int w2 = 0; w2 < RW; ++w2) rr[w2] = reinterpret_cast<const uint32_t *>(ref_rec + i * CS)[w2];
                rv = ref_valid[i];
            }
        }
        float term = 0.0f;
        if (M <= 8) {
            const int cand = (t16 < 8) ? a1 : a2, tt = t16 & 7;
            if (abl & 1) term = 1.0f;
            else if (tt == 0) term = U[(int64_t)j * n * LSQ_H + ((int64_t)(cand / SLF) * n + ((abl & 16) ? lo : i)) * SLF + (cand % SLF)];
            else if (tt < M) {
                const int k = (tt - 1) + ((tt - 1) >= j ? 1 : 0);
                const uint32_t bk = (rw[k >> 2] >> (8 * (k & 3))) & 0xffu;
                term = Tj[((int64_t)(k * LSQ_H) + bk) * LSQ_H + cand];
            }
        }
#pragma unroll
        for (int kk = 0; kk < M - 1; ++kk) {
            if (abl & 8) break;
            const int k = kk + (kk >= j ? 1 : 0);
            const uint32_t bk = (rw[k >> 2] >> (8 * (k & 3))) & 0xffu;
            const u32x4 *tp = reinterpret_cast<const u32x4 *>(Tqj + (int64_t)q16_row_index<RT::SLQ>(M, kk, (int)bk) * RT::SLQ);
            const u32x4 b0 = tp[0], b1 = tp[1];
            s0.x = pk_add_u16(s0.x, b0.x); s0.y = pk_add_u16(s0.y, b0.y); s0.z = pk_add_u16(s0.z, b0.z); s0.w = pk_add_u16(s0.w, b0.w);
            s1.x = pk_add_u16(s1.x, b1.x); s1.y = pk_add_u16(s1.y, b1.y); s1.z = pk_add_u16(s1.z, b1.z); s1.w = pk_add_u16(s1.w, b1.w);
        }
        uint32_t mask = 0;
#define LSQ_SURV(W, B) mask |= (((W) & 0xffffu) <= limit ? 1u : 0u) << (B); mask |= (((W) >> 16) <= limit ? 1u : 0u) << ((B) + 1);
        LSQ_SURV(s0.x, 0) LSQ_SURV(s0.y, 2) LSQ_SURV(s0.z, 4) LSQ_SURV(s0.w, 6) LSQ_SURV(s1.x, 8) LSQ_SURV(s1.y, 10) LSQ_SURV(s1.z, 12) LSQ_SURV(s1.w, 14)
#undef LSQ_SURV
        if (!act) mask = 0;
        float bv = __builtin_inff();
        int bi = 0x7fffffff;
        if (M <= 8) {
            float e = __shfl(term, (lane & ~7), 64);
#pragma unroll
            for (int q = 1; q < M; ++q) e = e + __shfl(term, (lane & ~7) + q, 64);
            const float e1 = __shfl(e, lane & ~15, 64), e2 = __shfl(e, (lane & ~15) + 8, 64);
            if (a1 / 16 == t16) mask &= ~(1u << (a1 % 16));
            if (a2 / 16 == t16) mask &= ~(1u << (a2 % 16));
            bv = e1; bi = a1;
            if (e2 < bv || (e2 == bv && a2 < bi)) { bv = e2; bi = a2; }
            if (act && t16 == 0) nexact += 2;
        }
        while (mask) {
            const int a = 16 * t16 + __builtin_ctz(mask);
            mask &= mask - 1;
            const float ev = q16_exact_value<M, RW>(U, T, n, SLF, j, i, rw, a);
            ++nexact;
            if (ev < bv || (ev == bv && a < bi)) { bv = ev; bi = a; }
        }
#pragma unroll
        for (int o = 8; o > 0; o >>= 1) {
            const float ov = __shfl_xor(bv, o, 16);
            const int oi = __shfl_xor(bi, o, 16);
            if (ov < bv || (ov == bv && oi < bi)) { bv = ov; bi = oi; }
        }
        if (act && t16 == 0) {
            const uint8_t c8 = (uint8_t)bi;
            const uint8_t old = (uint8_t)(rw[j >> 2] >> (8 * (j & 3)));
            if (c8 != old) store_code<CS>(rec, i, j, c8, rw);
            if (valid) {
                unsigned short vm = (c8 != old) ? (unsigned short)(1u << j) : (unsigned short)(vo | (1u << j));
                if (have_ref) {
                    bool same = true;
#pragma unroll
                    for (int w2 = 0; w2 < RW; ++w2) {
                        uint32_t mine = rw[w2];
                        if (w2 == (j >> 2)) mine = (mine & ~(0xffu << (8 * (j & 3)))) | ((uint32_t)c8 << (8 * (j & 3)));
                        same = same && (mine == rr[w2]);
                    }
                    if (same) vm = (unsigned short)(vm | rv);
                }
                valid[i] = vm;
                if (vmir) vmir[i - lo] = vm;
            }
        }
    }
    return nexact;
}

constexpr int WALKQ_MISC_BYTES = (20 + LSQ_WALK_COUNTERS) * 4;

template <int M>
__global__ __launch_bounds__(WalkqRot<M>::NT) __attribute__((amdgpu_waves_per_eu(4, 4))) void icm_walkq_kernel(const float *__restrict__ U, const uint16_t *__restrict__ Uq, const uint16_t *__restrict__ Tq,
                                                       const float *__restrict__ T, uint8_t *__restrict__ rec, unsigned short *__restrict__ valid,
                                                       int64_t n, const WalkNodes nodes, int per_pass, int use_skip, int direct_max,
                                                       unsigned long long *__restrict__ active_total,
                                                       const uint8_t *__restrict__ ref_rec, const unsigned short *__restrict__ ref_valid,
                                                       const lsq_q16_params *__restrict__ P, int SLF, const unsigned short *__restrict__ qflag, int abl,
                                                       const unsigned *__restrict__ gate) {
    using RT = WalkqRot<M>;
    constexpr int CS = (M <= 8) ? 8 : 16;
    constexpr int NS = LSQ_H / RT::SLQ;
    constexpr int LPV = RT::SLQ / 8;
    constexpr int VPW = 64 / LPV;
    constexpr int CW = (M - 1 + 3) / 4;
    constexpr int RW = CS / 4;
    constexpr int TAB = (M - 1) * LSQ_H * LPV;
    constexpr int PP = RT::pp();
    if (P->ok == 0) return;
    if (gate && *gate != 2u) return;
    extern __shared__ u32x4 lds_walkq[];
    constexpr int MAIN_BYTES = RT::lds_bytes();
    int *misc = reinterpret_cast<int *>(reinterpret_cast<char *>(lds_walkq) + MAIN_BYTES);
#ifdef LSQ_TUNING
    unsigned long long *dbgp = nullptr;
    if (g_walkq_dbg) {
        unsigned &dbg_slot_s = reinterpret_cast<unsigned *>(misc)[19];
        if (threadIdx.x == 0) dbg_slot_s = (blockIdx.x == 0) ? atomicAdd(&g_walkq_dbg_slot, 1u) : 0u;
        __syncthreads();
        if (blockIdx.x == 0 && dbg_slot_s < 4096) dbgp = g_walkq_dbg + (size_t)dbg_slot_s * LSQ_WALKQ_DBG_WORDS;
    }
    DBG_STAMP(0);
    if (blockIdx.x == 0 && threadIdx.x == 0) g_walkq_dbg_cur = dbgp;
    if (g_walkq_blk && threadIdx.x == 0) g_walkq_blk[2 * blockIdx.x] = wall_clock64();
#endif
    if ((uint32_t)(uintptr_t)(lds_char *)lds_walkq != 0u) __builtin_trap();
    u32x4 *tab = lds_walkq;
    constexpr bool HOLE = RT::HOLE;
    constexpr bool LHOLE = RT::LHOLE;
    constexpr bool ROT8 = M <= 8, ROT16 = M > 8;
    constexpr int TABE = RT::TAB_BYTES / 16;
    uint32_t *bestA = HOLE ? reinterpret_cast<uint32_t *>(reinterpret_cast<char *>(lds_walkq) + RT::HOLE_BYTE0)
                           : reinterpret_cast<uint32_t *>(lds_walkq + TABE);
    uint32_t *bestB = HOLE ? reinterpret_cast<uint32_t *>(lds_walkq + TABE) : bestA + PP;
    unsigned short *list = LHOLE ? reinterpret_cast<unsigned short *>(reinterpret_cast<char *>(lds_walkq) + RT::HOLE_BYTE0)
                                 : reinterpret_cast<unsigned short *>(bestB + PP);
    auto listp = [&](int i) -> unsigned short * { return LHOLE ? list + ((i >> 4) << 7) + (i & 15) : list + i; };
    constexpr bool MIRROR = RT::mirror();
    auto keyA = [&](int ci) -> uint32_t * { return HOLE ? bestA + ((ci >> 4) << 6) + (ci & 15) : bestA + ci; };
    auto f32slot = [&](int i) -> unsigned short * { return reinterpret_cast<unsigned short *>(keyA(i >> 1)) + (i & 1); };
    unsigned short *vmir = (MIRROR && valid) ? list + PP : nullptr;
    int *wave_tot = misc;
    int &nact_s = misc[16];
    int &redo_s = misc[17];
    int &f32_s = misc[18];
    unsigned *stat_s = reinterpret_cast<unsigned *>(misc) + 20;
    for (int e = threadIdx.x; e < LSQ_WALK_COUNTERS; e += RT::NT) stat_s[e] = 0u;
    __syncthreads();

    const int lane = threadIdx.x & 63;
    const int wave = __builtin_amdgcn_readfirstlane((int)(threadIdx.x >> 6));
    const int v = lane / LPV, q = lane % LPV;
    constexpr int NW = RT::NT / 64;
    constexpr int EPT = 4096 / RT::NT;
    constexpr int step = NW * VPW;

    struct Item { u32x4 u; uint32_t r[RW]; };

    auto walk_slices = [&](const int j, const int64_t lo, const int nact, const bool dense) {
#ifndef LSQ_TUNING
        unsigned long long *dbgp = nullptr; (void)dbgp;
#endif
        const uint16_t *__restrict__ Uqj = Uq + (int64_t)j * n * LSQ_H;
        const uint16_t *__restrict__ Tqj = Tq + (int64_t)j * NS * TAB * 8;
        uint32_t sel[CW > 0 ? CW : 1];
#pragma unroll
        for (int w = 0; w < CW; ++w) {
            uint32_t sv = 0;
#pragma unroll
            for (int t = 0; t < 4; ++t) {
                const int kk = 4 * w + t;
                const int k = kk + (kk >= j ? 1 : 0);
                sv |= (uint32_t)((kk < M - 1 ? k - 4 * w : 0) & 7) << (8 * t);
            }
            sel[w] = sv;
        }
        constexpr int NST = (TAB + RT::NT - 1) / RT::NT;
        u32x4 nxt[NST > 0 ? NST : 1];
        uint32_t selC0 = 0x0c0c0c0cu, selC1 = 0x0c0c0c0cu, base0 = 0u, base1 = 0x01000000u;
        uint32_t rotA = 0x0c0c0c0cu, rotB = 0x0c0c0c0cu, rot1A = 0x0c0c0c0cu, rot1B = 0x0c0c0c0cu, b0a = 0u, b0b = 0u, b1a = 0u, b1b = 0u;
        if constexpr (ROT16) {
#pragma unroll
            for (int t = 0; t < 8; ++t) {
                if (t < RT::NT0) {
                    const uint32_t slot = (uint32_t)(t + v) % (uint32_t)RT::NT0;
                    const uint32_t ab = ((slot << 5) | ((uint32_t)q << 4)) << (8 * (t & 3));
// ... 207 lines not shown
                    if (t < ipw) {
                        compute(buf[(PH + e) % RT::DEPTH], slice, c0); load_next(buf[(PH + e) % RT::DEPTH]); c0 += step;
                        ++t; phase = (PH + e + 1) % RT::DEPTH;
                    }
            };
            bool ran = false;
            auto try_phase = [&](auto P_) {
                if constexpr (decltype(P_)::value < RT::DEPTH) {
                    if (!ran && phase == decltype(P_)::value) { run(P_); ran = true; }
                }
            };
            try_phase(std::integral_constant<int, 0>{}); try_phase(std::integral_constant<int, 1>{});
            try_phase(std::integral_constant<int, 2>{}); try_phase(std::integral_constant<int, 3>{});
#ifdef LSQ_TUNING
            if (slice == 4) DBG_STAMP(22);
#endif
        }
        __syncthreads();
    };

    constexpr int LB = LSQ_LIGHT_LB(M);
    int64_t lo_cur = 0;
    auto light_list = [&](const int j, const int count, auto pick) {
        const float *__restrict__ Usj = U + (int64_t)j * n * LSQ_H;
        const float *__restrict__ Tj = T + (int64_t)j * M * LSQ_H * LSQ_H;
        for (int r0 = wave; r0 < count; r0 += NW * LB) {
            int64_t vi[LB];
            bool on[LB];
#pragma unroll
            for (int e = 0; e < LB; ++e) {
                const int r = r0 + e * NW;
                on[e] = r < count;
                vi[e] = lo_cur + __builtin_amdgcn_readfirstlane((int)pick(on[e] ? r : r0));
            }
            light_update<M, CS, LB>(rec, valid, ref_rec, ref_valid, Usj, Tj, n, SLF, j, vi, on, lane, vmir, lo_cur);
        }
    };

    const int64_t npass = (n + per_pass - 1) / per_pass;
    for (int64_t pass = blockIdx.x; pass < npass; pass += gridDim.x) {
        const int64_t lo = pass * per_pass;
        const int64_t hi = (lo + per_pass < n) ? lo + per_pass : n;
        const int cnt = (int)(hi - lo);
        lo_cur = lo;
        if (vmir) {
            __syncthreads();
            for (int idx = (int)threadIdx.x; idx < cnt; idx += RT::NT) vmir[idx] = valid[lo + idx];
            __syncthreads();
        }
        for (int nu = 0; nu < nodes.count; ++nu) {
            const int j = nodes.j[nu];
            int tix = (int)threadIdx.x;
            asm volatile("" : "+v"(tix));
#ifdef LSQ_TUNING
            if (dbgp && threadIdx.x == 0 && pass == (int64_t)blockIdx.x && nu < 64) dbgp[24 + nu] = wall_clock64();
#endif
            {
                const int base = tix * EPT;
                int f[EPT], c = 0;
#pragma unroll
                for (int e = 0; e < EPT; ++e) {
                    const int idx = base + e;
                    f[e] = 0;
                    if (idx < cnt) f[e] = (!use_skip) || !(((vmir ? vmir[idx] : valid[lo + idx]) >> j) & 1);
                    c += f[e];
                }
                int inc = c;
#pragma unroll
                for (int off = 1; off < 64; off <<= 1) {
                    const int t = __shfl_up(inc, off, 64);
                    if (lane >= off) inc += t;
                }
                if (lane == 63) wave_tot[wave] = inc;
                DBG_STAMP(16);
                __syncthreads();
                DBG_STAMP(17);
                int wbase = 0;
                for (int w2 = 0; w2 < wave; ++w2) wbase += wave_tot[w2];
                int pos = wbase + inc - c;
#pragma unroll
                for (int e = 0; e < EPT; ++e)
                    if (f[e]) *listp(pos++) = (unsigned short)(base + e);
                if (threadIdx.x == RT::NT - 1) { nact_s = wbase + inc; redo_s = 0; f32_s = 0; }
                DBG_STAMP(18);
                __syncthreads();
            }
            const int nact = nact_s;
            DBG_STAMP(1);
#ifdef LSQ_TUNING
            if (dbgp && threadIdx.x == 0 && pass == (int64_t)blockIdx.x && nu < 64) dbgp[24 + 65 + nu] = (unsigned long long)nact;
#endif
            if (nact == 0) { __syncthreads(); continue; }
            if (threadIdx.x == 0) {
                stat_s[0] += (unsigned)nact;
                stat_s[nact <= direct_max ? 2 : 3] += 1u;
                stat_s[4 + ((nodes.pos0 + nu) & (LSQ_WALK_TRACE - 1))] += (unsigned)nact;
            }
            if (nact <= direct_max) {
                light_list(j, nact, [&](int r) { return *listp(r); });
                __syncthreads();
                continue;
            }
            for (int ci = tix; ci < nact; ci += RT::NT) { *keyA(ci) = 0xffffffffu; bestB[ci] = 0xffffffffu; }
            DBG_STAMP(2);
            walk_slices(j, lo, nact, nact == cnt);
            DBG_STAMP(11);
            const lsq_q16_node &nd = P->node[j];
            const int window = nd.window;
            constexpr int EPD = (PP + RT::NT - 1) / RT::NT;
            constexpr int AREC = 2 + RW;
            constexpr int ACAP = (PP * 4) / (AREC * 4);
            {
                int64_t vi[EPD];
                uint32_t vcode[EPD], vkey[EPD], vlim[EPD];
                bool von[EPD], vamb[EPD], vf32[EPD];
                constexpr bool ONE_TRIP = (M <= 8);
                uint32_t rw[EPD][RW], rr[EPD][RW];
                unsigned short vo[EPD], rv[EPD], fl[EPD];
                uint32_t kA[EPD], kB[EPD];
                const bool have_ref = ref_rec && ref_valid;
#pragma unroll
                for (int e = 0; e < EPD; ++e) {
                    const int ci = tix + e * RT::NT;
                    vi[e] = lo; kA[e] = 0; kB[e] = 0; vo[e] = 0; rv[e] = 0; fl[e] = 0;
#pragma unroll
                    for (int w2 = 0; w2 < RW; ++w2) { rw[e][w2] = 0; rr[e][w2] = 0; }
                    if (ci < nact) {
                        kA[e] = *keyA(ci); kB[e] = bestB[ci];
                        vi[e] = lo + *listp(ci);
                        fl[e] = qflag[vi[e]];
                        if constexpr (ONE_TRIP) {
#pragma unroll
                            for (int w2 = 0; w2 < RW; ++w2) rw[e][w2] = reinterpret_cast<const uint32_t *>(rec + vi[e] * CS)[w2];
                            if (valid) vo[e] = valid[vi[e]];
                            if (have_ref) {
#pragma unroll
                                for (int w2 = 0; w2 < RW; ++w2) rr[e][w2] = reinterpret_cast<const uint32_t *>(ref_rec + vi[e] * CS)[w2];
                                rv[e] = ref_valid[vi[e]];
                            }
                        }
                    }
                }
#pragma unroll
                for (int e = 0; e < EPD; ++e) {
                    const int ci = tix + e * RT::NT;
                    von[e] = false; vamb[e] = false; vf32[e] = false; vcode[e] = 0; vkey[e] = 0; vlim[e] = 0;
                    if (ci < nact) {
                        vcode[e] = kA[e] & 0xffffu;
                        vkey[e] = (uint32_t)ci | ((kA[e] & 0xffu) << 16) | ((kB[e] & 0xffu) << 24);
                        vlim[e] = (kA[e] >> 16) + (uint32_t)window;
                        vf32[e] = (fl[e] >> j) & 1;
                        vamb[e] = !vf32[e] && ((int)(kB[e] >> 16) - (int)(kA[e] >> 16) <= window);
                        von[e] = !vamb[e] && !vf32[e];
                    }
                    if constexpr (!ONE_TRIP) {
                        if (von[e] || vamb[e]) {
#pragma unroll
                            for (int w2 = 0; w2 < RW; ++w2) rw[e][w2] = reinterpret_cast<const uint32_t *>(rec + vi[e] * CS)[w2];
                        }
                        if (von[e]) {
                            if (valid) vo[e] = valid[vi[e]];
                            if (have_ref) {
#pragma unroll
                                for (int w2 = 0; w2 < RW; ++w2) rr[e][w2] = reinterpret_cast<const uint32_t *>(ref_rec + vi[e] * CS)[w2];
                                rv[e] = ref_valid[vi[e]];
                            }
                        }
                    }
                }
                __syncthreads();
                uint32_t *arec = bestB;
#pragma unroll
                for (int e = 0; e < EPD; ++e) {
                    if (von[e]) {
                        const uint8_t c8 = (uint8_t)vcode[e];
                        const uint8_t old = (uint8_t)(rw[e][j >> 2] >> (8 * (j & 3)));
                        if (c8 != old) store_code<CS>(rec, vi[e], j, c8, rw[e]);
                        if (valid) {
                            unsigned short vm = (c8 != old) ? (unsigned short)(1u << j) : (unsigned short)(vo[e] | (1u << j));
                            if (have_ref) {
                                bool same = true;
#pragma unroll
                                for (int w2 = 0; w2 < RW; ++w2) {
                                    uint32_t mine = rw[e][w2];
                                    if (w2 == (j >> 2)) mine = (mine & ~(0xffu << (8 * (j & 3)))) | ((uint32_t)c8 << (8 * (j & 3)));
                                    same = same && (mine == rr[e][w2]);
                                }
                                if (same) vm = (unsigned short)(vm | rv[e]);
                            }
                            valid[vi[e]] = vm;
                            if (vmir) vmir[vi[e] - lo] = vm;
                        }
                    }
                    bool tof32 = vf32[e];
                    if (vamb[e]) {
                        const int slot = atomicAdd(&redo_s, 1);
                        if (slot < ACAP) {
                            arec[slot * AREC] = vkey[e];
                            arec[slot * AREC + 1] = vlim[e];
#pragma unroll
                            for (int w2 = 0; w2 < RW; ++w2) arec[slot * AREC + 2 + w2] = rw[e][w2];
                        } else tof32 = true;
                    }
                    if (tof32) *f32slot(atomicAdd(&f32_s, 1)) = (unsigned short)(vkey[e] & 0xffffu);
                }
            }
            __syncthreads();
            DBG_STAMP(12);
            const int namb = redo_s < ACAP ? redo_s : ACAP;
            int nexact = q16_refine<M>(U, Uq, Tq, T, rec, valid, ref_rec, ref_valid, n, j, lo, list, bestB, namb, SLF, abl, vmir);
            {
                const int nf32 = f32_s;
                light_list(j, nf32, [&](int r) { return *listp(*f32slot(r)); });
                if (threadIdx.x == 0 && nf32) atomicAdd(&stat_s[4 + LSQ_WALK_TRACE + 2], (unsigned)nf32);
            }
            {
#pragma unroll
                for (int o = 32; o > 0; o >>= 1) nexact += __shfl_xor(nexact, o, 64);
                if (lane == 0 && nexact) atomicAdd(&stat_s[4 + LSQ_WALK_TRACE + 1], (unsigned)nexact);
                if (threadIdx.x == 0 && namb) atomicAdd(&stat_s[4 + LSQ_WALK_TRACE], (unsigned)namb);
            }
            __syncthreads();
            DBG_STAMP(13);
#ifdef LSQ_TUNING
            if (dbgp && threadIdx.x == 0) { dbgp[14] = (unsigned long long)nact; dbgp[15] = (unsigned long long)namb; }
#endif
        }
    }
    __syncthreads();
#ifdef LSQ_TUNING
    if (dbgp && threadIdx.x == 0) dbgp[24 + 64] = wall_clock64();
    if (g_walkq_blk && threadIdx.x == 0) g_walkq_blk[2 * blockIdx.x + 1] = wall_clock64();
#endif
    if (active_total)
        for (int e = threadIdx.x; e < LSQ_WALK_COUNTERS; e += RT::NT)
            if (stat_s[e]) atomicAdd(active_total + e, (unsigned long long)stat_s[e]);
}

}

#ifdef LSQ_TUNING
extern "C" __attribute__((visibility("default"))) int lsq_tuning_set_walkq_debug(void *buf) {
    unsigned zero = 0;
    LSQ_HIP(hipMemcpyToSymbol(HIP_SYMBOL(g_walkq_dbg), &buf, sizeof(buf)));
    LSQ_HIP(hipMemcpyToSymbol(HIP_SYMBOL(g_walkq_dbg_slot), &zero, sizeof(zero)));
    return LSQ_OK;
}
extern "C" __attribute__((visibility("default"))) int lsq_tuning_set_walkq_block_clock(void *buf) {
    LSQ_HIP(hipMemcpyToSymbol(HIP_SYMBOL(g_walkq_blk), &buf, sizeof(buf)));
    return LSQ_OK;
}
#endif

__global__ void q16_road_kernel(const lsq_q16_params *__restrict__ P, unsigned *__restrict__ road, long long pairs, long long fallback_div) {
    if (threadIdx.x != 0) return;
    const bool filtered = P->ok == 1 && (long long)P->nflag * fallback_div <= pairs;
    road[0] = filtered ? 2u : 0u;
    if (!filtered) road[1] += 1u;
}
__global__ void q16_probe_kernel(const unsigned long long *__restrict__ probe, unsigned long long *__restrict__ totals, unsigned *__restrict__ road,
                                 unsigned long long probe_div) {
    const int e = threadIdx.x;
    if (e < LSQ_WALK_COUNTERS && totals) totals[e] += probe[e];
    if (e == 0 && road[0] == 2u && probe_div > 0) {
        const unsigned long long hard = probe[4 + LSQ_WALK_TRACE] + probe[4 + LSQ_WALK_TRACE + 2];
        if ((double)hard * (double)probe_div > (double)probe[0]) { road[0] = 0u; road[1] += 1u; }
    }
}
int lsq_launch_q16_road(hipStream_t s, const lsq_q16_params *P, unsigned *road, int64_t pairs, int64_t fallback_div) {
    hipLaunchKernelGGL(q16_road_kernel, dim3(1), dim3(64), 0, s, P, road, (long long)pairs, (long long)fallback_div);
    LSQ_HIP(hipGetLastError());
    return LSQ_OK;
}
int lsq_launch_q16_probe(hipStream_t s, const unsigned long long *probe, unsigned long long *totals, unsigned *road, int64_t probe_div) {
    hipLaunchKernelGGL(q16_probe_kernel, dim3(1), dim3(128), 0, s, probe, totals, road, (unsigned long long)probe_div);
    LSQ_HIP(hipGetLastError());
    return LSQ_OK;
}

const void *lsq_probe_kernel_icmq() { return reinterpret_cast<const void *>(&q16_range_init_kernel); }

template <class XT>
int lsq_launch_unary_shift_panel(hipStream_t s, const XT *Xp, int64_t rows, int d, int m, const lsq_q16_work &w, int64_t row0) {
    if (rows <= 0) return LSQ_OK;
    const int64_t shift_blocks = (rows * 16 + 255) / 256;
    LSQ_SHIFT_LAUNCH(d, dim3((unsigned)(shift_blocks < 2048 ? shift_blocks : 2048)), s, Xp, w.means, rows, d, m, w.sigma + (size_t)row0 * m,
                       &w.qrange[lsq_q16_work::Q_PANEL_SINK], &w.qrange[lsq_q16_work::Q_SIGBOUND], w.qflag, row0, w.P);
    LSQ_HIP(hipGetLastError());
    return LSQ_OK;
}

template int lsq_launch_unary_shift_panel(hipStream_t, const float *, int64_t, int, int, const lsq_q16_work &, int64_t);
template int lsq_launch_unary_shift_panel(hipStream_t, const uint8_t *, int64_t, int, int, const lsq_q16_work &, int64_t);

int lsq_q16_sample_rows(int64_t n, int d, int64_t *rts_out) {
    const int64_t nsample = d <= 128 ? 16384 : (d <= 512 ? 8192 : 4096);
    const int64_t rts = n > nsample ? n / nsample : 1;
    if (rts_out) *rts_out = rts;
    return (int)((n + 128 * rts - 1) / (128 * rts));
}

template <class XT>
int lsq_launch_q16_prepare(hipStream_t s, const XT *X, int64_t n, int d, const float *K, const float *sci, const float *T, int m, const lsq_q16_work &w,
                           int tables_changed) {
    using W = lsq_q16_work;
    const XT *Xsample = static_cast<const XT *>(w.Xsample);
    unsigned *sigmax = &w.qrange[W::Q_SIGMAX];
    static_assert(W::Q_SIGBOUND == W::Q_SIGMAX + 1 && W::Q_WORDS == 2 * LSQ_MAX_M + 4, "q16_params_kernel's sigrange[0 .. 1], q16_range_init_kernel's fill");
    if (tables_changed) {
        LSQ_HIP(hipMemsetAsync(w.bad, 0, sizeof(int), s));
        hipLaunchKernelGGL(table_colmean_kernel, dim3((unsigned)(m * m)), dim3(256), 0, s, T, m, w.colmean);
        hipLaunchKernelGGL(unary_colshift_kernel, dim3((unsigned)m), dim3(256), 0, s, w.colmean, m, w.colshift);
        if (m > 1) hipLaunchKernelGGL(table_range_kernel, dim3((unsigned)(m * m)), dim3(256), 0, s, T, m, w.colmean, w.trange, w.rowmin, w.bad);
        hipLaunchKernelGGL(codebook_means_kernel, dim3((unsigned)((d + 63) / 64), (unsigned)m), dim3(256), 0, s, K, m, d, w.means);
    }
    hipLaunchKernelGGL(q16_range_init_kernel, dim3(1), dim3(64), 0, s, w.qrange, m);
    lsq_gemm_q16 range;
    range.qrange = w.qrange; range.colshift = w.colshift;
    if (Xsample) {
        const int64_t shift_blocks = (w.nsample_rows * 16 + 255) / 256;
        LSQ_SHIFT_LAUNCH(d, dim3((unsigned)(shift_blocks < 2048 ? shift_blocks : 2048)), s, Xsample, w.means, w.nsample_rows, d, m, w.sigma_sample, sigmax);
        range.sigma = w.sigma_sample;
        LSQ_TRY(lsq_launch_chain_gemm(s, Xsample, K, sci, -2.0f, w.nsample_rows, m * LSQ_H, d, LSQ_H, 0, 0, nullptr, 0, w.nsample_rows, 0, &range));
        LSQ_HIP(hipMemsetAsync(w.qflag, 0, sizeof(unsigned short) * (size_t)((n + 1) & ~(int64_t)1), s));
    } else if (n > 0) {
        const int64_t shift_blocks = (n * 16 + 255) / 256;
        LSQ_SHIFT_LAUNCH(d, dim3((unsigned)(shift_blocks < 2048 ? shift_blocks : 2048)), s, X, w.means, n, d, m, w.sigma, sigmax);
        int64_t rts64 = 1;
        (void)lsq_q16_sample_rows(n, d, &rts64);
        range.rts = (int)rts64; range.sigma = w.sigma;
        LSQ_TRY(lsq_launch_chain_gemm(s, X, K, sci, -2.0f, n, m * LSQ_H, d, LSQ_H, 0, 0, nullptr, 0, n, 0, &range));
        LSQ_HIP(hipMemsetAsync(w.qflag, 0, sizeof(unsigned short) * (size_t)((n + 1) & ~(int64_t)1), s));
    }
    hipLaunchKernelGGL(q16_params_kernel, dim3(1), dim3(64), 0, s, w.trange, w.bad, w.qrange, m, w.P, sigmax, Xsample ? 2.0f : 1.0f);
    if (m > 1) {
        const int slq = lsq_q16_slice_width(m);
        const int64_t total = (int64_t)m * (LSQ_H / slq) * (m - 1) * LSQ_H * (slq / 8);
        const unsigned grid = (unsigned)((total + 255) / 256);
        if (slq == 32) hipLaunchKernelGGL(tables_to_q16_slices_kernel<32>, dim3(grid), dim3(256), 0, s, T, w.Tq, m, w.P, w.rowmin, w.colmean);
        else hipLaunchKernelGGL(tables_to_q16_slices_kernel<16>, dim3(grid), dim3(256), 0, s, T, w.Tq, m, w.P, w.rowmin, w.colmean);
    }
    LSQ_HIP(hipGetLastError());
    return LSQ_OK;
}

template int lsq_launch_q16_prepare(hipStream_t, const float *, int64_t, int, const float *, const float *, const float *, int, const lsq_q16_work &, int);
template int lsq_launch_q16_prepare(hipStream_t, const uint8_t *, int64_t, int, const float *, const float *, const float *, int, const lsq_q16_work &, int);

template <int M>
static int launch_walkq_t(hipStream_t s, const float *U, const uint16_t *Uq, const uint16_t *Tq, const float *T, uint8_t *rec, unsigned short *valid,
                          int64_t n, const WalkNodes &nodes, int use_skip, unsigned long long *active_total, int light,
                          const uint8_t *ref_rec, const unsigned short *ref_valid, const lsq_q16_params *P, const unsigned short *qflag, const unsigned *gate) {
    using RT = WalkqRot<M>;
    constexpr int PP = RT::pp();
    constexpr int LDS_BYTES = RT::lds_bytes() + WALKQ_MISC_BYTES;
    static_assert(LDS_BYTES <= 160 * 1024 && WALKQ_MISC_BYTES <= 768, "slice table + keys must fit the 160 KiB LDS");
    constexpr int NBLK = 256;
    int per_pass = 1, npass = 1;
    lsq_walk_geometry(n, PP, &per_pass, &npass);
    const int direct_max = light >= 0 ? light : LSQ_KNOB("LSQ_WALK_DIRECT", 160);
    const int skip = (use_skip && valid) ? 1 : 0;
    static LdsOptIn optin;
    LSQ_TRY(optin_lds(optin, &icm_walkq_kernel<M>, LDS_BYTES));
    static std::atomic<int> static_lds_known{-1};
    int static_lds = static_lds_known.load(std::memory_order_relaxed);
    if (static_lds < 0) {
        hipFuncAttributes fa;
        LSQ_HIP(hipFuncGetAttributes(&fa, reinterpret_cast<const void *>(&icm_walkq_kernel<M>)));
        static_lds = (int)fa.sharedSizeBytes;
        static_lds_known.store(static_lds, std::memory_order_relaxed);
    }
    if (static_lds != 0) { lsq_set_error("icm_walkq_kernel<%d>: %d bytes of static LDS in a kernel that addresses LDS from 0", M, static_lds); return LSQ_EHIP; }
    const unsigned grid = (unsigned)(npass < NBLK ? npass : NBLK);
    hipLaunchKernelGGL((icm_walkq_kernel<M>), dim3(grid), dim3(RT::NT), LDS_BYTES, s, U, Uq, Tq, T, rec, valid, n, nodes, per_pass, skip,
                       direct_max, active_total, skip ? ref_rec : nullptr, skip ? ref_valid : nullptr, P, lsq_walk_slice_width(M), qflag, LSQ_KNOB("LSQ_Q16_ABL", 0), gate);
    LSQ_HIP(hipGetLastError());
    return LSQ_OK;
}

int lsq_launch_icm_walkq(hipStream_t s, const float *U, const uint16_t *Uq, const uint16_t *Tq, const float *T, uint8_t *rec, unsigned short *valid,
                         int64_t n, int m, const int32_t *order, int nnodes, int pos0, int max_per, int use_skip, unsigned long long *active_total, int light,
                         const uint8_t *ref_rec, const unsigned short *ref_valid, const lsq_q16_params *P, const unsigned short *qflag, const unsigned *gate,
                         int *launched) {
    if (n <= 0 || nnodes <= 0) return LSQ_OK;
    return for_walk_launches(order, nnodes, pos0, m, max_per, launched, [&](const WalkNodes &nodes) -> int {
        LSQ_DISPATCH_M(m, LSQ_TRY((launch_walkq_t<M_>(s, U, Uq, Tq, T, rec, valid, n, nodes, use_skip, active_total, light, ref_rec, ref_valid, P, qflag, gate))));
        return LSQ_OK;
    });
}
```

local-search-quantization_amd/csrc/lsq_internal.h:

```cpp
#pragma once

#include <hip/hip_runtime.h>
#include <stdint.h>
#include <stddef.h>
#include <stdlib.h>

#include "../../include/lsq_mi355x.h"

#define LSQ_H 256
#define LSQ_MAX_M 16
#define LSQ_WALK_TRACE 64
#define LSQ_WALK_COUNTERS (4 + LSQ_WALK_TRACE + 3)

#ifdef LSQ_TUNING
#define LSQ_KNOB(name, def) ([] { static const int v_ = [] { const char *e_ = getenv(name); return e_ ? atoi(e_) : (def); }(); return v_; }())
#else
#define LSQ_KNOB(name, def) (def)
#endif

void lsq_set_error(const char *fmt, ...);

#define LSQ_HIP(call)                                                                          \
    do {                                                                                       \
        hipError_t e_ = (call);                                                                \
        if (e_ != hipSuccess) {                                                                \
            lsq_set_error("%s failed: %s (%s:%d)", #call, hipGetErrorString(e_), __FILE__, __LINE__); \
            return (e_ == hipErrorOutOfMemory) ? LSQ_ENOMEM : LSQ_EHIP;                        \
        }                                                                                      \
    } while (0)

#define LSQ_TRY(expr)                  \
    do {                               \
        int rc_ = (expr);              \
        if (rc_ != LSQ_OK) return rc_; \
    } while (0)

struct DevBuf {
    void *p = nullptr;
    size_t cap = 0;
    bool view = false;
    int ensure(size_t bytes) {
        if (bytes <= cap) return LSQ_OK;
        if (view) { p = nullptr; cap = 0; view = false; }
        if (p) { LSQ_HIP(hipFree(p)); p = nullptr; cap = 0; }
        if (bytes == 0) return LSQ_OK;
        LSQ_HIP(hipMalloc(&p, bytes));
        cap = bytes;
        return LSQ_OK;
    }
    void release() { if (p && !view) (void)hipFree(p); p = nullptr; cap = 0; view = false; }
    void window(void *base, size_t off, size_t bytes) { release(); p = static_cast<char *>(base) + off; cap = bytes; view = true; }
    template <class T> T *as() const { return reinterpret_cast<T *>(p); }
};

enum { LSQ_DOM_PERTURB = 1, LSQ_DOM_PERM = 2, LSQ_DOM_INIT = 3, LSQ_DOM_DATA = 4, LSQ_DOM_CODEBOOK = 5 };

struct lsq_u32x4 { uint32_t v[4]; };

__host__ __device__ inline lsq_u32x4 lsq_philox4x32_10(uint32_t c0, uint32_t c1, uint32_t c2, uint32_t c3,
                                                       uint32_t k0, uint32_t k1) {
#pragma unroll
    for (int r = 0; r < 10; ++r) {
        const uint64_t p0 = (uint64_t)0xD2511F53u * c0;
        const uint64_t p1 = (uint64_t)0xCD9E8D57u * c2;
        const uint32_t n0 = (uint32_t)(p1 >> 32) ^ c1 ^ k0;
        const uint32_t n1 = (uint32_t)p1;
        const uint32_t n2 = (uint32_t)(p0 >> 32) ^ c3 ^ k1;
        const uint32_t n3 = (uint32_t)p0;
        c0 = n0; c1 = n1; c2 = n2; c3 = n3;
        k0 += 0x9E3779B9u; k1 += 0xBB67AE85u;
    }
    lsq_u32x4 o;
    o.v[0] = c0; o.v[1] = c1; o.v[2] = c2; o.v[3] = c3;
    return o;
}

__host__ __device__ inline lsq_u32x4 lsq_rng_block(uint64_t seed, uint64_t idx, uint32_t it, uint32_t domain, uint32_t block) {
    return lsq_philox4x32_10((uint32_t)idx, (uint32_t)(idx >> 32), it, (domain << 16) | block,
                             (uint32_t)seed, (uint32_t)(seed >> 32));
}

__host__ __device__ inline uint32_t lsq_rng_word(uint64_t seed, uint64_t idx, uint32_t it, uint32_t domain, uint32_t w) {
    return lsq_rng_block(seed, idx, it, domain, w >> 2).v[w & 3];
}

__host__ __device__ inline uint32_t lsq_mulhi32(uint32_t a, uint32_t b) { return (uint32_t)(((uint64_t)a * b) >> 32); }

struct lsq_q16_node {
    float loU, invD, D;
    float hiq;
    int window;
    double slack;
};
struct lsq_q16_params {
    int ok;
    int oor;
    int nflag;
    lsq_q16_node node[LSQ_MAX_M];
};

const void *lsq_probe_kernel_gemm();
const void *lsq_probe_kernel_icm();
const void *lsq_probe_kernel_icmq();


struct lsq_gemm_q16 {
    uint16_t *Dq = nullptr; int slice_q = 0;
    lsq_q16_params *qp = nullptr;
    unsigned short *qflag = nullptr;
    const float *sigma = nullptr, *colshift = nullptr;
    unsigned *qrange = nullptr; int rts = 1;
};
int lsq_launch_chain_gemm(hipStream_t s, const float *A, const float *Bm, const float *addv, float alpha,
                          int64_t M, int N, int Kd, int h, int64_t plane_stride, int64_t row_stride, float *D, int slice,
                          int64_t Mtot, int64_t rbase, const lsq_gemm_q16 *q = nullptr);
int lsq_launch_chain_gemm(hipStream_t s, const uint8_t *A, const float *Bm, const float *addv, float alpha,
                          int64_t M, int N, int Kd, int h, int64_t plane_stride, int64_t row_stride, float *D, int slice,
                          int64_t Mtot, int64_t rbase, const lsq_gemm_q16 *q = nullptr);
int lsq_launch_sqnorms(hipStream_t s, const float *Kb, int rows, int d, float *sci);

static inline int lsq_code_stride(int m) { return m <= 8 ? 8 : 16; }

int lsq_launch_codes_expand(hipStream_t s, const uint8_t *tight, int64_t n, int m, uint8_t *rec);
int lsq_launch_codes_compact(hipStream_t s, const uint8_t *rec, int64_t n, int m, uint8_t *tight);
int lsq_launch_codes_from_i16(hipStream_t s, const int16_t *B, int64_t n, int m, int h, uint8_t *rec, int *bad_flag);
int lsq_launch_codes_to_i16(hipStream_t s, const uint8_t *rec, int64_t n, int m, int16_t *B);

int lsq_launch_perturb(hipStream_t s, const uint8_t *src, uint8_t *dst, int64_t n, int m, int npert,
                       uint64_t seed, uint32_t it, uint64_t global_offset, const unsigned short *vsrc, unsigned short *vdst);
constexpr int lsq_walk_slice_width(int m) { return m <= 8 ? 16 : 8; }
constexpr int lsq_q16_slice_width(int m) { return 2 * lsq_walk_slice_width(m); }
int lsq_launch_tables_to_slices(hipStream_t s, const float *T, float *Ts, int m, int sl);
constexpr int lsq_walk_pp(int M, int SL) {
    const int avail = 160 * 1024 - 256 - (M - 1) * LSQ_H * (SL / 4) * 16;
    const int pp = avail / 10 / 64 * 64;
    return pp > 4096 ? 4096 : pp;
}
inline void lsq_walk_geometry(int64_t n, int pp, int *per_pass, int *npass) {
    const int64_t rounds = (n + 256 * (int64_t)pp - 1) / (256 * (int64_t)pp);
    int64_t per = rounds > 0 ? (n + 256 * rounds - 1) / (256 * rounds) : 1;
    per = per > pp ? pp : (per < 1 ? 1 : per);
    *per_pass = (int)per;
    *npass = (int)((n + per - 1) / per);
}
int lsq_launch_icm_wave(hipStream_t s, const float *U, const float *T, uint8_t *rec, unsigned short *valid, int64_t n, int m, const int32_t *order,
                        int nnodes, int pos0, int max_per, int use_skip, unsigned long long *active_total, const uint8_t *ref_rec,
                        const unsigned short *ref_valid, int *launched);
int lsq_launch_icm_walk(hipStream_t s, const float *U, const float *Ts, const float *T, uint8_t *rec, unsigned short *valid, int64_t n, int m,
                        const int32_t *order, int nnodes, int pos0, int max_per, int use_skip, unsigned long long *active_total, int ablation, int light,
                        const uint8_t *ref_rec, const unsigned short *ref_valid, const int *idle_if_set, int *launched);
struct lsq_q16_work {
    enum { Q_NONFINITE = 2 * LSQ_MAX_M,
           Q_SIGMAX,
           Q_SIGBOUND,
           Q_PANEL_SINK,
           Q_WORDS };
    uint16_t *Tq = nullptr, *Uq = nullptr;
    int *bad = nullptr;
    float *trange = nullptr;
    unsigned *qrange = nullptr;
    unsigned short *qflag = nullptr;
    lsq_q16_params *P = nullptr;
    float *rowmin = nullptr, *colmean = nullptr, *colshift = nullptr, *means = nullptr, *sigma = nullptr;
    const void *Xsample = nullptr;
    int64_t nsample_rows = 0;
    float *sigma_sample = nullptr;
};
template <class XT>
int lsq_launch_q16_prepare(hipStream_t s, const XT *X, int64_t n, int d, const float *K, const float *sci, const float *T, int m, const lsq_q16_work &w,
                           int tables_changed);
int lsq_q16_sample_rows(int64_t n, int d, int64_t *rts_out);
template <class XT>
int lsq_launch_unary_shift_panel(hipStream_t s, const XT *Xp, int64_t rows, int d, int m, const lsq_q16_work &w, int64_t row0);
int lsq_launch_icm_walkq(hipStream_t s, const float *U, const uint16_t *Uq, const uint16_t *Tq, const float *T, uint8_t *rec, unsigned short *valid,
                         int64_t n, int m, const int32_t *order, int nnodes, int pos0, int max_per, int use_skip, unsigned long long *active_total, int light,
                         const uint8_t *ref_rec, const unsigned short *ref_valid, const lsq_q16_params *P, const unsigned short *qflag,
                         const unsigned *gate, int *launched);
int lsq_launch_q16_road(hipStream_t s, const lsq_q16_params *P, unsigned *road, int64_t pairs, int64_t fallback_div);
int lsq_launch_q16_probe(hipStream_t s, const unsigned long long *probe, unsigned long long *totals, unsigned *road, int64_t probe_div);
struct lsq_perturb_next { int on; int m, npert; uint32_t it; uint64_t seed, goff; uint8_t *dst; unsigned short *vdst; int abl; };
int lsq_launch_cost(hipStream_t s, const float *X, const float *K, const uint8_t *rec, uint8_t *cur, float *prev,
                    unsigned long long *counters, int64_t n, int d, int m, int mode,
                    const unsigned short *vnew, unsigned short *vcur,
                    const lsq_perturb_next *next = nullptr);
int lsq_launch_cost(hipStream_t s, const uint8_t *X, const float *K, const uint8_t *rec, uint8_t *cur, float *prev,
                    unsigned long long *counters, int64_t n, int d, int m, int mode,
                    const unsigned short *vnew, unsigned short *vcur,
                    const lsq_perturb_next *next = nullptr);
int lsq_launch_sum_f64(hipStream_t s, const float *v, int64_t n, double *sum);

int lsq_launch_synth_data_u8(hipStream_t s, uint64_t seed, uint64_t global_offset, int64_t n, int d, float *X);
int lsq_launch_randinit(hipStream_t s, uint64_t seed, uint64_t global_offset, int64_t n, int m, int h, uint8_t *tight);
int lsq_launch_synth_codebooks(hipStream_t s, uint64_t seed, int m, int h, int d, float *K);

int lsq_launch_viterbi(hipStream_t s, const float *U, const float *T, int64_t n, int m, uint8_t *codes);
int lsq_launch_unary_argmin(hipStream_t s, const float *U, int64_t n, int m, uint8_t *codes, float *minval);

__device__ inline uint32_t lsq_adc_key(float v) {
    if (v != v) return 0xffffffffu;
    const uint32_t b = __float_as_uint(v);
    return b ^ ((uint32_t)((int32_t)b >> 31) | 0x80000000u);
}
__device__ inline float lsq_adc_unkey(uint32_t k) {
    if (k == 0xffffffffu) return __uint_as_float(0x7fc00000u);
    return __uint_as_float((k & 0x80000000u) ? (k ^ 0x80000000u) : ~k);
}
struct lsq_adc_state;
void lsq_adc_free(lsq_adc_state *st);
enum lsq_search_kind { LSQ_SEARCH_LSQ, LSQ_SEARCH_PQ, LSQ_SEARCH_EXACT };
struct lsq_search_input {
    lsq_search_kind kind;
    const uint8_t *codes; int cstride;
    const void *Q; int qstride;
    const float *K;
    const float *dbnorms;
    int n, m, d;
    const void *base; int bstride;
    int base_u8 = 0, q_u8 = 0;
    const uint32_t *xnorms = nullptr, *qnorms = nullptr;
    int id_base = 0;
    int query_width() const { return kind == LSQ_SEARCH_PQ ? m * d : d; }
    int id_sub() const { return kind == LSQ_SEARCH_LSQ ? 0 : 1 - id_base; }
    size_t base_elem() const { return base_u8 ? 1 : sizeof(float); }
    size_t query_elem() const { return q_u8 ? 1 : sizeof(float); }
};
struct lsq_search_opts {
    int force_exhaustive = 0, rank_override = 0;
    lsq_linscan_stats *stats = nullptr;
    int timed = 0;
};
int lsq_adc_search(hipStream_t s, lsq_adc_state **st, float *dists, int *idx, const lsq_search_input &in, int nq, int nn, const lsq_search_opts &opt);
int lsq_adc_search_host(hipStream_t s, lsq_adc_state **st, float *dists, int *idx, const lsq_search_input &in, int nq, int nn, const lsq_search_opts &opt);
int lsq_knn_launch_scan(hipStream_t s, int mode, const lsq_search_input &in, const int *qsel, int q0, int nqb, int stride, int ns, const uint32_t *tau,
                        unsigned *count, int cap, uint64_t *out, int idbits);
int lsq_knn_launch_norms_u8(hipStream_t s, const uint8_t *X, int64_t ld, int n, int d, uint32_t *out);
int lsq_knn_exact_check(const char *fn, const void *dists, const void *ids, const void *base, const void *queries, int n, int nq, int d, int ldb,
                        int ldq, int nn);

int lsq_rerank_launch(hipStream_t s, const void *base, int base_u8, int64_t ldb, int64_t n, const float *Q, int64_t ldq, const int *cand, int q0, int nqb,
                      int L, int d, int id_base, uint64_t *out, int idbits, unsigned long long *invalid);
int lsq_rerank_check(const char *fn, const void *dists, const void *ids, const void *base, const void *queries, const void *cand, int64_t n, int nq, int d,
                     int64_t ldb, int64_t ldq, int L, int nn, int id_base);
int lsq_adc_idbits(int64_t n);
int lsq_adc_select(lsq_adc_state **st, hipStream_t s, const uint64_t *recs, uint64_t *sorted, int *seg, const unsigned *count, int *fail, const int *qsel,
                   int q0, int nqb, int cap, int nn, float *dists, int *idx, int idbits, int end_bit, int id_sub);

int lsq_linscan_pq_check(const char *fn, const void *dists, const void *res, const void *codes, const void *centers, const void *queries, int N,
                         uint32_t NQ, int B, int K, int dim1codes, int dim1queries, int subdim);

int lsq_launch_quantize_norms(hipStream_t s, const uint8_t *codes, int stride, const float *K, const float *cb, int ncb, int64_t n, int d, int m,
                              uint8_t *idx0, int16_t *idx1, float *dbnorms, float *norms);

struct lsq_lsqr_state;
void lsq_lsqr_free(lsq_lsqr_state *st);
int lsq_lsqr_update_codebooks(hipStream_t s, lsq_lsqr_state **st, const float *dX, const uint8_t *dcodes, const uint8_t *cover, int d, int64_t n, int m,
                              float *dK, int *iters_out);
int lsq_sort_rows_by_code(hipStream_t s, DevBuf &buf, const uint8_t *dcodes, int64_t n, int m, const uint64_t **sorted, const int64_t **seg);

struct lsq_kmeans_state;
void lsq_kmeans_free(lsq_kmeans_state *st);
int lsq_kmeans_update_centers(hipStream_t s, lsq_kmeans_state **st, const float *dX, const uint8_t *dcodes, const uint8_t *cover, const float *dKprev, int d,
                              int64_t n, int m, float *dK, int *dcounts);
int lsq_kmeans_seed(hipStream_t s, lsq_kmeans_state **st, const float *dX, const uint8_t *cover, const double *u, int d, int64_t n, int m, float *dK,
                    int64_t *didx, float *dd2);
int lsq_kmeans_fill_i64(hipStream_t s, int64_t *p, int64_t count, int64_t v);

struct lsq_spgl1_state;
void lsq_spgl1_free(lsq_spgl1_state *st);
int lsq_spgl1_update_codebooks(hipStream_t s, lsq_spgl1_state **st, const float *dX, const uint8_t *dcodes, int d, int64_t n, int m, double tau,
                               const float *dK0, int64_t S, double opt_tol, int64_t max_iter, float *dK, lsq_spgl1_info *info);
```

Baseline: 21.46 million.

## Overlap table prep and initial cost on an auxiliary stream; add streaming shift kernel

```diff
diff --git a/local-search-quantization_amd/csrc/lsq_api.hip b/local-search-quantization_amd/csrc/lsq_api.hip
--- a/local-search-quantization_amd/csrc/lsq_api.hip
+++ b/local-search-quantization_amd/csrc/lsq_api.hip
@@ -7,6 +7,7 @@
 #include <atomic>
 #include <chrono>
 #include <string>
+#include <functional>
 #include <thread>
 #include <vector>
 
@@ -100,6 +101,11 @@
     int64_t pipeline_min_bytes = 64ll << 20;
     hipStream_t copy_stream = nullptr;
     hipEvent_t copy_done = nullptr;
+    hipStream_t aux_stream = nullptr;
+    hipEvent_t aux_fork = nullptr, aux_k = nullptr, aux_cost = nullptr;
+    int aux_on = 1;
+    bool aux_failed = false;
+    bool k_forked = false;
     double cat_ms[CAT_COUNT] = {0, 0, 0, 0, 0, 0};
     int64_t icm_launches = 0, icm_node_updates = 0, staged_blocks = 0, light_blocks = 0, filtered_blocks = 0, filter_refined = 0, filter_exact = 0, filter_f32 = 0;
     int64_t trace[LSQ_WALK_TRACE] = {0};
@@ -121,13 +127,41 @@
     return LSQ_OK;
 }
 
+static hipStream_t aux_ready(lsq_ctx *c) {
+    if (!c->aux_on || c->aux_failed) return nullptr;
+    hipStreamCaptureStatus cap = hipStreamCaptureStatusNone;
+    if (hipStreamIsCapturing(c->stream, &cap) != hipSuccess || cap != hipStreamCaptureStatusNone) { (void)hipGetLastError(); return nullptr; }
+    if (!c->aux_stream) {
+        if (hipStreamCreateWithFlags(&c->aux_stream, hipStreamNonBlocking) != hipSuccess || hipEventCreateWithFlags(&c->aux_fork, hipEventDisableTiming) != hipSuccess ||
+            hipEventCreateWithFlags(&c->aux_k, hipEventDisableTiming) != hipSuccess || hipEventCreateWithFlags(&c->aux_cost, hipEventDisableTiming) != hipSuccess) {
+            (void)hipGetLastError();
+            c->aux_failed = true;
+            return nullptr;
+        }
+    }
+    return c->aux_stream;
+}
+static hipStream_t fork_aux(lsq_ctx *c) {
+    if (!aux_ready(c)) return nullptr;
+    if (hipEventRecord(c->aux_fork, c->stream) != hipSuccess || hipStreamWaitEvent(c->aux_stream, c->aux_fork, 0) != hipSuccess) { (void)hipGetLastError(); return nullptr; }
+    return c->aux_stream;
+}
+static int join_k(lsq_ctx *c) {
+    if (!c->k_forked) return LSQ_OK;
+    c->k_forked = false;
+    LSQ_HIP(hipEventRecord(c->aux_k, c->aux_stream));
+    LSQ_HIP(hipStreamWaitEvent(c->stream, c->aux_k, 0));
+    return LSQ_OK;
+}
+
 struct Timer {
-    lsq_ctx *c; int cat; hipEvent_t a = nullptr, b = nullptr; bool on;
-    Timer(lsq_ctx *ctx, int category) : c(ctx), cat(category), on(ctx->profile != 0) {
+    lsq_ctx *c; int cat; hipEvent_t a = nullptr, b = nullptr; bool on; hipStream_t s;
+    Timer(lsq_ctx *ctx, int category) : Timer(ctx, category, ctx->stream, true) {}
+    Timer(lsq_ctx *ctx, int category, hipStream_t stream, bool enabled) : c(ctx), cat(category), on(enabled && ctx->profile != 0), s(stream) {
         if (!on) return;
         a = grab(); b = grab();
         if (!a || !b) { on = false; return; }
-        (void)hipEventRecord(a, c->stream);
+        (void)hipEventRecord(a, s);
     }
     hipEvent_t grab() {
         if (!c->pool.empty()) { hipEvent_t e = c->pool.back(); c->pool.pop_back(); return e; }
@@ -137,7 +171,7 @@
     }
     ~Timer() {
         if (!on) return;
-        (void)hipEventRecord(b, c->stream);
+        (void)hipEventRecord(b, s);
         c->pending.push_back({a, b, cat});
     }
 };
@@ -225,6 +259,8 @@
     if (c->own_stream) (void)hipStreamDestroy(c->own_stream);
     if (c->copy_stream) (void)hipStreamDestroy(c->copy_stream);
     if (c->copy_done) (void)hipEventDestroy(c->copy_done);
+    if (c->aux_stream) { (void)hipStreamSynchronize(c->aux_stream); (void)hipStreamDestroy(c->aux_stream); }
+    for (hipEvent_t e : {c->aux_fork, c->aux_k, c->aux_cost}) if (e) (void)hipEventDestroy(e);
     delete c;
     return LSQ_OK;
 }
@@ -253,6 +289,7 @@
     else if (!strcmp(key, "q16_min")) c->q16_min = value;
     else if (!strcmp(key, "async")) c->async_mode = value != 0;
     else if (!strcmp(key, "per_node")) c->per_node = value != 0;
+    else if (!strcmp(key, "aux_stream")) c->aux_on = value != 0;
     else if (!strcmp(key, "upload_panel_bytes")) {
         if (value < 1) { lsq_set_error("upload_panel_bytes must be >= 1"); return LSQ_EINVAL; }
         c->panel_bytes = value;
@@ -837,7 +874,7 @@
     return LSQ_OK;
 }
 
-static int prepare_tables(lsq_ctx *c, const float *dK, int d, int m) {
+static int prepare_tables(lsq_ctx *c, const float *dK, int d, int m, bool fork = false) {
     Timer t(c, CAT_TABLES);
     c->tables_changed = 1;
     c->chunk_road.resident = false;
@@ -845,12 +882,18 @@
     const int mh = m * LSQ_H;
     LSQ_TRY(c->sci.ensure(sizeof(float) * (size_t)mh));
     LSQ_TRY(c->T.ensure(sizeof(float) * (size_t)mh * mh));
-    LSQ_TRY(lsq_launch_sqnorms(c->stream, dK, mh, d, c->sci.as<float>()));
-    LSQ_TRY(lsq_launch_chain_gemm(c->stream, dK, dK, nullptr, 2.0f, mh, mh, d, LSQ_H, (int64_t)m * LSQ_H * LSQ_H, LSQ_H, c->T.as<float>(), 0, mh, 0));
-    if (c->schedule >= 3 && m > 1) {
-        LSQ_TRY(c->Ts.ensure(sizeof(float) * (size_t)m * (m - 1) * LSQ_H * LSQ_H));
-        LSQ_TRY(lsq_launch_tables_to_slices(c->stream, c->T.as<float>(), c->Ts.as<float>(), m, lsq_walk_slice_width(m)));
-    }
+    if (c->schedule >= 3 && m > 1) LSQ_TRY(c->Ts.ensure(sizeof(float) * (size_t)m * (m - 1) * LSQ_H * LSQ_H));
+    LSQ_TRY(join_k(c));
+    hipStream_t ks = c->stream;
+    if (fork) {
+        hipStream_t aux = fork_aux(c);
+        if (aux) { ks = aux; c->k_forked = true; }
+    }
+    Timer tk(c, CAT_TABLES, ks, ks != c->stream);
+    LSQ_TRY(lsq_launch_sqnorms(ks, dK, mh, d, c->sci.as<float>()));
+    LSQ_TRY(lsq_launch_chain_gemm(ks, dK, dK, nullptr, 2.0f, mh, mh, d, LSQ_H, (int64_t)m * LSQ_H * LSQ_H, LSQ_H, c->T.as<float>(), 0, mh, 0));
+    if (c->schedule >= 3 && m > 1)
+        LSQ_TRY(lsq_launch_tables_to_slices(ks, c->T.as<float>(), c->Ts.as<float>(), m, lsq_walk_slice_width(m)));
     return LSQ_OK;
 }
 
@@ -896,7 +939,10 @@
     Timer t(c, CAT_TABLES);
     LSQ_TRY(q16_map(c, d, cn, m, Xsample ? nsample_rows : 0));
     if (Xsample) { c->qw.Xsample = Xsample; c->qw.nsample_rows = nsample_rows; c->qw.sigma_sample = c->sSigmaS.as<float>(); }
-    LSQ_TRY(lsq_launch_q16_prepare(c->stream, dX, cn, d, dK, c->sci.as<float>(), c->T.as<float>(), m, c->qw, c->tables_changed));
+    const bool forked = c->k_forked;
+    c->k_forked = false;
+    LSQ_TRY(lsq_launch_q16_prepare(c->stream, dX, cn, d, dK, c->sci.as<float>(), c->T.as<float>(), m, c->qw, c->tables_changed, forked ? c->aux_stream : nullptr,
+                                   forked ? c->aux_k : nullptr));
     c->tables_changed = 0;
     return LSQ_OK;
 }
@@ -915,14 +961,17 @@
 static int q16_verdict(lsq_ctx *c, bool q16, int64_t cn, int m);
 
 template <class XT>
-static int build_unaries(lsq_ctx *c, const XT *dX, const float *dK, int d, int64_t cn, int m, int slice, int64_t r0, int64_t rows) {
+static int build_unaries(lsq_ctx *c, const XT *dX, const float *dK, int d, int64_t cn, int m, int slice, int64_t r0, int64_t rows,
+                         const std::function<int()> &after_gemm = {}) {
     const bool q16 = start_chunk(c, cn, slice) && r0 == 0 && rows == cn;
     if (q16) LSQ_TRY(q16_prepare_chunk(c, dX, dK, d, cn, m));
+    LSQ_TRY(join_k(c));
     {
         Timer t(c, CAT_UNARIES);
         LSQ_TRY(c->U.ensure(sizeof(float) * (size_t)m * (size_t)cn * LSQ_H));
         LSQ_TRY(unary_gemm(c, dX, dK, d, cn, m, slice, r0, rows, q16));
     }
+    if (after_gemm) LSQ_TRY(after_gemm());
     return q16_verdict(c, q16, cn, m);
 }
 
@@ -974,6 +1023,7 @@
         LSQ_HIP(hipMemcpyAsync(c->sSample.p, sample, (size_t)ns * row_bytes, hipMemcpyHostToDevice, c->stream));
         LSQ_TRY(q16_prepare_chunk<XT>(c, dXc, dK, d, cn, m, c->sSample.as<XT>(), ns));
     }
+    LSQ_TRY(join_k(c));
     LSQ_TRY(c->U.ensure(sizeof(float) * (size_t)m * (size_t)cn * LSQ_H));
     std::atomic<int> landed{0};
     hipError_t herr = hipSuccess;
@@ -1065,7 +1115,6 @@
 static int encode_chunk(lsq_ctx *c, const XT *dXc, const float *dK, int64_t cn, uint64_t goff, const EncodeParams &P, int64_t I, Snap snap,
                         bool unaries_ready = false) {
     const int cs = lsq_code_stride(P.m);
-    if (!unaries_ready) LSQ_TRY(build_unaries(c, dXc, dK, P.d, cn, P.m, lsq_walk_slice_width(P.m), 0, cn));
     LSQ_TRY(c->recNew.ensure((size_t)cn * cs));
     LSQ_TRY(c->prev.ensure(sizeof(float) * (size_t)cn));
     LSQ_TRY(c->vCur.ensure(sizeof(unsigned short) * (size_t)(cn + 8)));
@@ -1078,11 +1127,23 @@
     unsigned long long *totals = c->active.as<unsigned long long>(), *probed = nullptr;
     lsq_perturb_next pn;
     pn.on = 1; pn.m = P.m; pn.npert = P.npert; pn.seed = P.seed; pn.goff = goff; pn.dst = nw; pn.vdst = vnew;
-    {
-        Timer t(c, CAT_COST);
+    hipStream_t cost_stream = unaries_ready ? nullptr : aux_ready(c);
+    if (cost_stream && hipEventRecord(c->aux_fork, c->stream) != hipSuccess) { (void)hipGetLastError(); cost_stream = nullptr; }
+    auto initial_cost = [&](hipStream_t s) -> int {
+        Timer t(c, CAT_COST, s, true);
         pn.it = P.it0;
-        LSQ_TRY(lsq_launch_cost(c->stream, dXc, dK, cur, cur, prev, counters, cn, P.d, P.m, 0, nullptr, vcur, I > 0 ? &pn : nullptr));
-    }
+        return lsq_launch_cost(s, dXc, dK, cur, cur, prev, counters, cn, P.d, P.m, 0, nullptr, vcur, I > 0 ? &pn : nullptr);
+    };
+    std::function<int()> early_cost;
+    if (cost_stream) early_cost = [&]() -> int {
+        LSQ_HIP(hipStreamWaitEvent(cost_stream, c->aux_fork, 0));
+        LSQ_TRY(initial_cost(cost_stream));
+        LSQ_HIP(hipEventRecord(c->aux_cost, cost_stream));
+        return LSQ_OK;
+    };
+    if (!unaries_ready) LSQ_TRY(build_unaries(c, dXc, dK, P.d, cn, P.m, lsq_walk_slice_width(P.m), 0, cn, early_cost));
+    if (cost_stream) LSQ_HIP(hipStreamWaitEvent(c->stream, c->aux_cost, 0));
+    else LSQ_TRY(initial_cost(c->stream));
     for (int64_t it = 0; it < I; ++it) {
         int32_t order[LSQ_MAX_M];
         LSQ_TRY(lsq_node_order(P.seed, P.it0 + (uint32_t)it, P.m, P.randord, order));
@@ -1137,6 +1198,7 @@
 }
 
 static int begin_call(lsq_ctx *c, int64_t I, int nr) {
+    LSQ_TRY(join_k(c));
     c->call_row0 = 0;
     c->chunk_road.resident = false;
     LSQ_TRY(c->counters.ensure(sizeof(unsigned long long) * 2 * (size_t)std::max<int64_t>(I, 1)));
@@ -1228,7 +1290,7 @@
     LSQ_TRY(validate_encode(fn, d, n, m, h, ilsiters, nr, icmiter, npert, &I));
     if (!dK || !obj_sums || (n > 0 && (!dX || !dB0 || !dBs))) { lsq_set_error("%s: null pointer", fn); return LSQ_EINVAL; }
     LSQ_TRY(begin_call(c, I, nr));
-    LSQ_TRY(prepare_tables(c, dK, d, m));
+    LSQ_TRY(prepare_tables(c, dK, d, m, true));
     const EncodeParams P{d, m, ilsiters, nr, icmiter, npert, randord, seed, 0u};
     const int cs = lsq_code_stride(m);
     for (int64_t off = 0; off < n; off += c->chunk) {
@@ -1267,14 +1329,15 @@
     return LSQ_OK;
 }
 
-static int host_codebooks(lsq_ctx *c, const float *K, int d, int m) {
+static int host_codebooks(lsq_ctx *c, const float *K, int d, int m, bool fork = false) {
     const size_t count = (size_t)m * LSQ_H * d, kbytes = sizeof(float) * count;
+    LSQ_TRY(join_k(c));
     if (c->tables_valid && c->hostK_d == d && c->hostK_m == m && c->hostK.size() == count && memcmp(c->hostK.data(), K, kbytes) == 0) {
         c->table_reuses += 1;
         return LSQ_OK;
     }
     LSQ_TRY(claim_sK(c, d, m, K));
-    LSQ_TRY(prepare_tables(c, c->sK.as<float>(), d, m));
+    LSQ_TRY(prepare_tables(c, c->sK.as<float>(), d, m, fork));
     c->hostK.assign(K, K + count);
     c->hostK_d = d; c->hostK_m = m;
     c->tables_valid = true;
@@ -1294,11 +1357,12 @@
     if (!K || (!objs && !place) || (n > 0 && (!X || !B || !Bs))) { lsq_set_error("%s: null pointer", fn); return LSQ_EINVAL; }
     const int64_t ntot = place ? place->ntot : n, row0 = place ? place->row0 : 0;
     LSQ_TRY(begin_call(c, I, nr));
-    LSQ_TRY(host_codebooks(c, K, d, m));
+    LSQ_TRY(host_codebooks(c, K, d, m, true));
     const float *dK = c->sK.as<float>();
     {
         const int rc = check_codes_host(fn, B, n, m, h);
         if (rc != LSQ_OK) {
+            (void)join_k(c);
             (void)hipStreamSynchronize(c->stream);
             return rc;
         }
diff --git a/local-search-quantization_amd/csrc/lsq_icmq.hip b/local-search-quantization_amd/csrc/lsq_icmq.hip
--- a/local-search-quantization_amd/csrc/lsq_icmq.hip
+++ b/local-search-quantization_amd/csrc/lsq_icmq.hip
@@ -91,6 +91,8 @@
     const int64_t nrows = (int64_t)gridDim.x * 16;
     const bool vec = std::is_same<XT, float>::value ? (d & 3) == 0 && ((((uintptr_t)X | (uintptr_t)R) & 15) == 0)
                                                     : (d & 3) == 0 && (((uintptr_t)X & 3) == 0) && (((uintptr_t)R & 15) == 0);
+    const bool quads = (d & 3) == 0 && (((uintptr_t)R & 15) == 0);
+    auto ld4_any = [&](const XT *p) -> f32x4 { return vec ? lsq_ld4(p) : (f32x4){(float)p[0], (float)p[1], (float)p[2], (float)p[3]}; };
     float amax = 0.0f;
     const int64_t first = ((int64_t)blockIdx.x * 256 + (threadIdx.x & ~63)) >> 4;
     const float bnd = bound ? __uint_as_float(*bound) : __builtin_inff();
@@ -108,11 +110,11 @@
         float rmax = 0.0f;
         bool rnan = false;
         const XT *x = X + (live ? i : 0) * (int64_t)d;
-        if (!LONGV && vec && d <= 256) {
+        if (!LONGV && quads && d <= 256) {
             f32x4 xr[4];
 #pragma unroll
             for (int t = 0; t < 4; ++t)
-                xr[t] = 4 * lp + 64 * t < d ? lsq_ld4(x + 4 * lp + 64 * t) : (f32x4){0.0f, 0.0f, 0.0f, 0.0f};
+                xr[t] = 4 * lp + 64 * t < d ? ld4_any(x + 4 * lp + 64 * t) : (f32x4){0.0f, 0.0f, 0.0f, 0.0f};
             for (int j = 0; j < m; ++j) {
                 const float *r = R + (int64_t)j * d + 4 * lp;
                 float acc = 0.0f;
@@ -197,14 +199,92 @@
     if (lane == 0 && __float_as_uint(amax) > __hip_atomic_load(sigmax, __ATOMIC_RELAXED, __HIP_MEMORY_SCOPE_AGENT)) atomicMax(sigmax, __float_as_uint(amax));
 }
 
+constexpr int SHIFT_STREAM_ROWS = 32;
+template <int MJ>
+__global__ __launch_bounds__(256) void unary_shift_stream_kernel(const float *__restrict__ X, const float *__restrict__ R, int64_t n, int d, int m,
+                                                                 float *__restrict__ sigma, unsigned *__restrict__ sigmax,
+                                                                 const unsigned *__restrict__ bound, unsigned short *__restrict__ qflag,
+                                                                 int64_t flag_row0, lsq_q16_params *__restrict__ P) {
+    const int lane = threadIdx.x & 63, lp = lane & 15;
+    const int64_t nrows = (int64_t)gridDim.x * SHIFT_STREAM_ROWS;
+    const bool on[2] = {4 * lp < d, 4 * lp + 64 < d};
+    f32x4 rr[MJ][2];
+#pragma unroll
+    for (int j = 0; j < MJ; ++j)
+#pragma unroll
+        for (int t = 0; t < 2; ++t)
+            rr[j][t] = (j < m && on[t]) ? *reinterpret_cast<const f32x4 *>(R + (int64_t)j * d + 4 * lp + 64 * t) : (f32x4){0.0f, 0.0f, 0.0f, 0.0f};
+    float amax = 0.0f;
+    const float bnd = bound ? __uint_as_float(*bound) : __builtin_inff();
+    const int64_t first = (int64_t)blockIdx.x * SHIFT_STREAM_ROWS + (threadIdx.x >> 6) * 8;
+    for (int64_t base = first; base < n; base += nrows) {
+        f32x4 xr[2][2];
+#pragma unroll
+        for (int g = 0; g < 2; ++g) {
+            const int64_t i = base + 4 * g + (lane >> 4);
+            const float *x = X + (i < n ? i : 0) * (int64_t)d;
+#pragma unroll
+            for (int t = 0; t < 2; ++t) xr[g][t] = on[t] ? lsq_ld4(x + 4 * lp + 64 * t) : (f32x4){0.0f, 0.0f, 0.0f, 0.0f};
+        }
+#pragma unroll
+        for (int g = 0; g < 2; ++g) {
+            const int64_t i = base + 4 * g + (lane >> 4);
+            const bool live = i < n;
+            float rmax = 0.0f;
+            bool rnan = false;
+#pragma unroll
+            for (int j = 0; j < MJ; ++j) {
+                if (j < m) {
+                    float acc = 0.0f;
+#pragma unroll
+                    for (int t = 0; t < 2; ++t)
+                        if (on[t]) acc = fmaf(xr[g][t].w, rr[j][t].w, fmaf(xr[g][t].z, rr[j][t].z, fmaf(xr[g][t].y, rr[j][t].y, fmaf(xr[g][t].x, rr[j][t].x, acc))));
+                    acc = acc + dpp_self<DPP_XOR1, 0xf>(acc);
+                    acc = acc + dpp_self<DPP_XOR2, 0xf>(acc);
+                    acc = acc + dpp_self<DPP_HALF_MIRROR, 0xf>(acc);
+                    acc = acc + dpp_self<DPP_MIRROR, 0xf>(acc);
+                    const float sg = 2.0f * acc;
+                    if (live && lp == 0) sigma[i * m + j] = sg;
+                    if (live) { amax = fmaxf(amax, fabsf(sg)); rmax = fmaxf(rmax, fabsf(sg)); if (!(sg == sg)) rnan = true; }
+                }
+            }
+            if (qflag && live && lp == 0 && (rmax > bnd || rnan)) {
+                const int64_t gi = flag_row0 + i;
+                const unsigned bits = ((1u << m) - 1u) << (16 * (int)(gi & 1));
+                const unsigned old = atomicOr(reinterpret_cast<unsigned *>(qflag + (gi & ~(int64_t)1)), bits);
+                const int fresh = __popc(bits & ~old);
+                if (P && fresh) atomicAdd(&P->nflag, fresh);
+            }
+        }
+    }
+#pragma unroll
+    for (int off = 32; off > 0; off >>= 1) amax = fmaxf(amax, __shfl_xor(amax, off, 64));
+    if (lane == 0 && __float_as_uint(amax) > __hip_atomic_load(sigmax, __ATOMIC_RELAXED, __HIP_MEMORY_SCOPE_AGENT)) atomicMax(sigmax, __float_as_uint(amax));
+}
+
 __global__ __launch_bounds__(64) void q16_range_init_kernel(unsigned *__restrict__ qrange, int m) {
     const int t = threadIdx.x;
     if (t < 2 * LSQ_MAX_M + 4) qrange[t] = (t < 2 * m && !(t & 1)) ? 0xffffffffu : 0u;
 }
 
+static bool shift_streams(const float *X, const float *R, int d, int m) {
+    return d <= 128 && (d & 3) == 0 && ((((uintptr_t)X | (uintptr_t)R) & 15) == 0) && m <= 16;
+}
+static bool shift_streams(const uint8_t *, const float *, int, int) { return false; }
+static void launch_shift_stream(hipStream_t s, const float *X, const float *R, int64_t n, int d, int m, float *sigma, unsigned *sigmax,
+                                const unsigned *bound, unsigned short *qflag, int64_t flag_row0, lsq_q16_params *P) {
+    const int64_t blocks = (n + SHIFT_STREAM_ROWS - 1) / SHIFT_STREAM_ROWS;
+    const dim3 grid((unsigned)(blocks < 1024 ? blocks : 1024));
+    if (m <= 8) hipLaunchKernelGGL((unary_shift_stream_kernel<8>), grid, dim3(256), 0, s, X, R, n, d, m, sigma, sigmax, bound, qflag, flag_row0, P);
+    else hipLaunchKernelGGL((unary_shift_stream_kernel<16>), grid, dim3(256), 0, s, X, R, n, d, m, sigma, sigmax, bound, qflag, flag_row0, P);
+}
+static void launch_shift_stream(hipStream_t, const uint8_t *, const float *, int64_t, int, int, float *, unsigned *, const unsigned *, unsigned short *, int64_t,
+                                lsq_q16_params *) {}
+
 template <class XT>
 static void launch_unary_shift(dim3 grid, hipStream_t s, const XT *X, const float *R, int64_t n, int d, int m, float *sigma, unsigned *sigmax,
                                const unsigned *bound = nullptr, unsigned short *qflag = nullptr, int64_t flag_row0 = 0, lsq_q16_params *P = nullptr) {
+    if (shift_streams(X, R, d, m)) { launch_shift_stream(s, X, R, n, d, m, sigma, sigmax, bound, qflag, flag_row0, P); return; }
     if (d > 256) hipLaunchKernelGGL((unary_shift_kernel<true, XT>), grid, dim3(256), 0, s, X, R, n, d, m, sigma, sigmax, bound, qflag, flag_row0, P);
     else hipLaunchKernelGGL((unary_shift_kernel<false, XT>), grid, dim3(256), 0, s, X, R, n, d, m, sigma, sigmax, bound, qflag, flag_row0, P);
 }
@@ -1018,18 +1098,22 @@
 
 template <class XT>
 int lsq_launch_q16_prepare(hipStream_t s, const XT *X, int64_t n, int d, const float *K, const float *sci, const float *T, int m, const lsq_q16_work &w,
-                           int tables_changed) {
+                           int tables_changed, hipStream_t ks, hipEvent_t k_done) {
     using W = lsq_q16_work;
+    const bool forked = ks != nullptr && k_done != nullptr && ks != s;
+    if (!forked) ks = s;
     const XT *Xsample = static_cast<const XT *>(w.Xsample);
     unsigned *sigmax = &w.qrange[W::Q_SIGMAX];
     static_assert(W::Q_SIGBOUND == W::Q_SIGMAX + 1 && W::Q_WORDS == 2 * LSQ_MAX_M + 4, "q16_params_kernel's sigrange[0 .. 1], q16_range_init_kernel's fill");
     if (tables_changed) {
-        LSQ_HIP(hipMemsetAsync(w.bad, 0, sizeof(int), s));
-        hipLaunchKernelGGL(table_colmean_kernel, dim3((unsigned)(m * m)), dim3(256), 0, s, T, m, w.colmean);
-        hipLaunchKernelGGL(unary_colshift_kernel, dim3((unsigned)m), dim3(256), 0, s, w.colmean, m, w.colshift);
-        if (m > 1) hipLaunchKernelGGL(table_range_kernel, dim3((unsigned)(m * m)), dim3(256), 0, s, T, m, w.colmean, w.trange, w.rowmin, w.bad);
         hipLaunchKernelGGL(codebook_means_kernel, dim3((unsigned)((d + 63) / 64), (unsigned)m), dim3(256), 0, s, K, m, d, w.means);
-    }
+        LSQ_HIP(hipMemsetAsync(w.bad, 0, sizeof(int), ks));
+        hipLaunchKernelGGL(table_colmean_kernel, dim3((unsigned)(m * m)), dim3(256), 0, ks, T, m, w.colmean);
+        hipLaunchKernelGGL(unary_colshift_kernel, dim3((unsigned)m), dim3(256), 0, ks, w.colmean, m, w.colshift);
+        if (m > 1) hipLaunchKernelGGL(table_range_kernel, dim3((unsigned)(m * m)), dim3(256), 0, ks, T, m, w.colmean, w.trange, w.rowmin, w.bad);
+    }
+    if (forked) LSQ_HIP(hipEventRecord(k_done, ks));
+    auto join = [&]() -> int { if (forked) LSQ_HIP(hipStreamWaitEvent(s, k_done, 0)); return LSQ_OK; };
     hipLaunchKernelGGL(q16_range_init_kernel, dim3(1), dim3(64), 0, s, w.qrange, m);
     lsq_gemm_q16 range;
     range.qrange = w.qrange; range.colshift = w.colshift;
@@ -1037,6 +1121,7 @@
         const int64_t shift_blocks = (w.nsample_rows * 16 + 255) / 256;
         LSQ_SHIFT_LAUNCH(d, dim3((unsigned)(shift_blocks < 2048 ? shift_blocks : 2048)), s, Xsample, w.means, w.nsample_rows, d, m, w.sigma_sample, sigmax);
         range.sigma = w.sigma_sample;
+        LSQ_TRY(join());
         LSQ_TRY(lsq_launch_chain_gemm(s, Xsample, K, sci, -2.0f, w.nsample_rows, m * LSQ_H, d, LSQ_H, 0, 0, nullptr, 0, w.nsample_rows, 0, &range));
         LSQ_HIP(hipMemsetAsync(w.qflag, 0, sizeof(unsigned short) * (size_t)((n + 1) & ~(int64_t)1), s));
     } else if (n > 0) {
@@ -1045,9 +1130,11 @@
         int64_t rts64 = 1;
         (void)lsq_q16_sample_rows(n, d, &rts64);
         range.rts = (int)rts64; range.sigma = w.sigma;
+        LSQ_TRY(join());
         LSQ_TRY(lsq_launch_chain_gemm(s, X, K, sci, -2.0f, n, m * LSQ_H, d, LSQ_H, 0, 0, nullptr, 0, n, 0, &range));
         LSQ_HIP(hipMemsetAsync(w.qflag, 0, sizeof(unsigned short) * (size_t)((n + 1) & ~(int64_t)1), s));
     }
+    LSQ_TRY(join());
     hipLaunchKernelGGL(q16_params_kernel, dim3(1), dim3(64), 0, s, w.trange, w.bad, w.qrange, m, w.P, sigmax, Xsample ? 2.0f : 1.0f);
     if (m > 1) {
         const int slq = lsq_q16_slice_width(m);
@@ -1060,8 +1147,8 @@
     return LSQ_OK;
 }
 
-template int lsq_launch_q16_prepare(hipStream_t, const float *, int64_t, int, const float *, const float *, const float *, int, const lsq_q16_work &, int);
-template int lsq_launch_q16_prepare(hipStream_t, const uint8_t *, int64_t, int, const float *, const float *, const float *, int, const lsq_q16_work &, int);
+template int lsq_launch_q16_prepare(hipStream_t, const float *, int64_t, int, const float *, const float *, const float *, int, const lsq_q16_work &, int, hipStream_t, hipEvent_t);
+template int lsq_launch_q16_prepare(hipStream_t, const uint8_t *, int64_t, int, const float *, const float *, const float *, int, const lsq_q16_work &, int, hipStream_t, hipEvent_t);
 
 template <int M>
 static int launch_walkq_t(hipStream_t s, const float *U, const uint16_t *Uq, const uint16_t *Tq, const float *T, uint8_t *rec, unsigned short *valid,
diff --git a/local-search-quantization_amd/csrc/lsq_internal.h b/local-search-quantization_amd/csrc/lsq_internal.h
--- a/local-search-quantization_amd/csrc/lsq_internal.h
+++ b/local-search-quantization_amd/csrc/lsq_internal.h
@@ -168,7 +168,7 @@
 };
 template <class XT>
 int lsq_launch_q16_prepare(hipStream_t s, const XT *X, int64_t n, int d, const float *K, const float *sci, const float *T, int m, const lsq_q16_work &w,
-                           int tables_changed);
+                           int tables_changed, hipStream_t ks = nullptr, hipEvent_t k_done = nullptr);
 int lsq_q16_sample_rows(int64_t n, int d, int64_t *rts_out);
 template <class XT>
 int lsq_launch_unary_shift_panel(hipStream_t s, const XT *Xp, int64_t rows, int d, int m, const lsq_q16_work &w, int64_t row0);
```

Result: no change. 21.59 million, median of 6 (+0.6%).
